# marionmari/pyGPs

Measured on AMD Instinct MI355X. Metric: GP fits/sec (nlZ+grad, RBF, N=8192 d=16), higher is better.
Workload: dtype f64; 1 GPU; GPR+RBF, N=8192 d=16 fp64 synthetic (SURVEY 8d recipe, seed 0), infExact nlZ + dnlZ (BASELINE configs[1]); x,y resident in HBM, hyp changes every step; outputs nlZ, dnlZ(4), alpha(N) to host per step; fits_per_rank=313, fit_streams_per_gpu=2, sched=1

## Files before the change

### pygps_amd/csrc/capi.hip

```cpp
#include <algorithm>
#include <atomic>
#include <cmath>
#include <cstdio>
#include <cstdlib>
#include <cstring>
#include <map>
#include <string>
#include <mutex>
#include <vector>

#include "ctx.h"

static thread_local char g_err[512] = "";
void pgp_set_last_hip_error(hipError_t e, const char* what, const char* file, int line) {
    snprintf(g_err, sizeof(g_err), "HIP error %d (%s) in %s at %s:%d", (int)e, hipGetErrorString(e), what, file, line);
    (void)hipGetLastError();
}

static void ctx_register(pgp_ctx* c);
static void ctx_unregister(pgp_ctx* c);

void prof_collect(pgp_ctx* c) {
    if (c->recs.empty()) return;
    (void)hipStreamSynchronize(c->st);
    for (auto& r : c->recs) {
        float ms = 0.f;
        (void)hipEventElapsedTime(&ms, r.e0, r.e1);
        c->pc_ms[r.cls] += ms; c->pc_flops[r.cls] += r.flops; c->pc_bytes[r.cls] += r.bytes; c->pc_launch[r.cls]++;
        if (r.shadow >= 0) { c->pc_ms[r.shadow] += ms; c->pc_flops[r.shadow] += r.flops; c->pc_launch[r.shadow]++; }
        if (getenv("PGP_PROF_DUMP"))
            fprintf(stderr, "prof %-34s %8.4f ms %10.3f GF %7.2f TF\n", kProfNames[r.cls], ms, r.flops * 1e-9,
                    ms > 0 ? r.flops / (ms * 1e-3) * 1e-12 : 0.0);
        c->ev_pool.push_back(r.e0); c->ev_pool.push_back(r.e1);
    }
    c->recs.clear();
}

DeviceGate& device_gate(int device) {
    static DeviceGate gates[64];
    return gates[(unsigned)device % 64u];
}
int& device_gate_depth(int device) {
    static thread_local int depth[64] = {0};
    return depth[(unsigned)device % 64u];
}

extern "C" {

const char* pgp_version(void) { return "pygps_amd 0.1 (gfx950)"; }
int pgp_device_count(void) {
    int n = 0;
    if (hipGetDeviceCount(&n) != hipSuccess) { (void)hipGetLastError(); return 0; }
    return n;
}

const char* pgp_strerror(int status) {
    if (status == 0) return "ok";
    if (status > 0) return "kernel matrix not positive definite";
    if (status <= PGP_ERR_HIP) return g_err[0] ? g_err : "HIP runtime failure";
    return "bad argument";
}

__global__ void pgp_noop_kernel() {}
static int alloc_result_buffer(pgp_ctx* c, long np);

static unsigned* yield_table(int device) {
    static std::mutex mu;
    static unsigned* tab[64] = {nullptr};
    std::lock_guard<std::mutex> lk(mu);
    if (device < 0 || device >= 64) return nullptr;
    if (!tab[device]) {
        if (hipMalloc((void**)&tab[device], 4096 * sizeof(unsigned)) != hipSuccess) { (void)hipGetLastError(); tab[device] = nullptr; return nullptr; }
        (void)hipMemset(tab[device], 0, 4096 * sizeof(unsigned));
    }
    return tab[device];
}

int pgp_init(int device, pgp_ctx** ctx_out) { GateShared device_gate_hold(device);
    if (!ctx_out) return -2;
    HIP_TRY(hipSetDevice(device));
    {
        static std::mutex mu;
        static bool primed[64] = {false};
        std::lock_guard<std::mutex> lk(mu);
        if (device >= 0 && device < 64 && !primed[device]) {
            hipLaunchKernelGGL(pgp_noop_kernel, dim3(1), dim3(64), 0, 0);
            HIP_TRY(hipDeviceSynchronize());
            primed[device] = true;
        }
    }
    pgp_ctx* c = new pgp_ctx();
    c->device = device;
    if (const char* e = getenv("PYGPS_AMD_PREDICT_INVERSE")) { const int v = atoi(e); if (v >= 0 && v <= 2) c->predict_inverse = v; }
    if (const char* e = getenv("PYGPS_AMD_KEEP_INVERSE")) c->keep_inverse = atoi(e) != 0;
    HIP_TRY(hipGetDeviceProperties(&c->prop, device));
    HIP_TRY(hipStreamCreateWithFlags(&c->st, hipStreamNonBlocking));
    {
        int lo = 0, hi = 0;
        (void)hipDeviceGetStreamPriorityRange(&lo, &hi);
        HIP_TRY(hipStreamCreateWithPriority(&c->st2, hipStreamNonBlocking, hi));
        if (lo == hi) c->ep_block = 0;
    }
    for (auto& e : c->ev) HIP_TRY(hipEventCreate(&e));
    memset(c->last_ms, 0, sizeof(c->last_ms));
    memset(c->pc_ms, 0, sizeof(c->pc_ms)); memset(c->pc_flops, 0, sizeof(c->pc_flops));
    memset(c->pc_bytes, 0, sizeof(c->pc_bytes)); memset(c->pc_launch, 0, sizeof(c->pc_launch));
    CHK(alloc_result_buffer(c, 0));
    c->yield_flags = yield_table(device);
    HIP_TRY(hipMalloc((void**)&c->Dk, (size_t)2048 * 1024 * sizeof(double)));
    HIP_TRY(hipMalloc((void**)&c->dpack, (size_t)8 * PACK_DOUBLES * sizeof(double)));
    HIP_TRY(hipMemset(c->Dk, 0, (size_t)2048 * 1024 * sizeof(double)));
    ctx_register(c);
    *ctx_out = c;
    return PGP_OK;
}

constexpr long RES_HEAD = 272, RES_INFO = 264;
static int alloc_result_buffer(pgp_ctx* c, long np) {
    const size_t bytes = (size_t)(RES_HEAD + np) * sizeof(double);
    if (c->res_dev) (void)hipFree(c->res_dev);
    if (c->res_host) (void)hipHostFree(c->res_host);
    c->res_dev = c->res_host = c->res_host_dev = nullptr; c->scal = c->alpha_dev = nullptr; c->info_dev = nullptr; c->res_cap = 0;
    HIP_TRY(hipMalloc((void**)&c->res_dev, bytes));
    HIP_TRY(hipMemset(c->res_dev, 0, bytes));
    HIP_TRY(hipHostMalloc((void**)&c->res_host, bytes, hipHostMallocMapped | hipHostMallocCoherent));
    c->res_host_dev = nullptr;
    if (hipHostGetDevicePointer((void**)&c->res_host_dev, c->res_host, 0) != hipSuccess) { (void)hipGetLastError(); c->res_host_dev = nullptr; }
    c->scal = c->res_dev; c->info_dev = (int*)(c->res_dev + RES_INFO); c->alpha_dev = c->res_dev + RES_HEAD;
    c->res_cap = bytes;
    return PGP_OK;
}

void pgp_destroy(pgp_ctx* c) { if (!c) return; GateShared device_gate_hold(c);
    if (!c) return;
    ctx_unregister(c);
    (void)hipSetDevice(c->device);
    (void)hipStreamSynchronize(c->st);
    if (c->st2) (void)hipStreamSynchronize(c->st2);
    for (auto& kv : c->pool) (void)hipFree(kv.second);
    for (auto& kv : c->spool) (void)hipFree(kv.second);
    for (auto& kv : c->orders) (void)hipFree(kv.second.first);
    void* bufs[] = {c->x_dev, c->y_dev, c->XsT, c->scale_dev, c->W, c->T, c->Binv, c->inv16, c->m_dev,
                    c->rvec, c->zvec, c->partial, c->Dk, c->dpack, c->Xs, c->res_dev, c->prep, c->pre2, c->pre1t, c->pre1s};
    for (void* b : bufs) if (b) (void)hipFree(b);
    if (c->res_host) (void)hipHostFree(c->res_host);
    if (c->in_host) (void)hipHostFree(c->in_host);
    if (c->pred_host) (void)hipHostFree(c->pred_host);
    if (c->gemm_trace) (void)hipFree(c->gemm_trace);
    for (auto& e : c->ev) (void)hipEventDestroy(e);
    for (auto& e : c->ev_pool) (void)hipEventDestroy(e);
    for (auto& r : c->recs) { (void)hipEventDestroy(r.e0); (void)hipEventDestroy(r.e1); }
    for (auto& e : c->la_ev) (void)hipEventDestroy(e);
    for (auto& e : c->tm_ev) (void)hipEventDestroy(e);
    for (auto& e : c->fill_ev) (void)hipEventDestroy(e);
    for (auto& e : c->ep_ev) (void)hipEventDestroy(e);
    (void)hipStreamDestroy(c->st);
    if (c->st2) (void)hipStreamDestroy(c->st2);
    delete c;
}

int pgp_device_info(pgp_ctx* c, int* n_cu, int* sclk_mhz, double* hbm_gib, char* name, int name_len) {
    if (!c) return -1;
    if (n_cu) *n_cu = c->prop.multiProcessorCount;
    if (sclk_mhz) *sclk_mhz = c->prop.clockRate / 1000;
    if (hbm_gib) *hbm_gib = (double)c->prop.totalGlobalMem / (1024.0 * 1024.0 * 1024.0);
    if (name && name_len > 0) { strncpy(name, c->prop.name, name_len - 1); name[name_len - 1] = 0; }
    return PGP_OK;
}

int pgp_set_option(pgp_ctx* c, const char* name, int value) {
    if (!c || !name) return -1;
    if (!strcmp(name, "nb_outer")) { if (value < 0) return -3; c->nb_outer = value; return PGP_OK; }
    if (!strcmp(name, "small_tile_below")) { c->small_tile_below = value; return PGP_OK; }
    if (!strcmp(name, "trtri_small_tile_below")) { c->trtri_small_tile_below = value; return PGP_OK; }
    if (!strcmp(name, "xcd_order")) { c->xcd_order = value; return PGP_OK; }
    if (!strcmp(name, "gemm_dbg")) { if (value & ~(64 | 256 | 512)) return -2; c->gemm_dbg = value; return PGP_OK; }
    if (!strcmp(name, "tile_ring")) { if (value < 0 || value > 1) return -2; c->tile_ring = value; return PGP_OK; }
    if (!strcmp(name, "lookahead")) { c->lookahead = value; return PGP_OK; }
    if (!strcmp(name, "leaf_first")) { c->leaf_first = value; return PGP_OK; }
    if (!strcmp(name, "leaf_pivot")) { if (value < 0 || value > 2) return -2; c->leaf_pivot = value; return PGP_OK; }
    if (!strcmp(name, "sched")) { if (value < -1 || value > 2) return -2; c->sched = value < 0 ? PGP_SCHED_DEFAULT : value; c->sched_explicit = value >= 0; return PGP_OK; }
    if (!strcmp(name, "concurrent_streams")) { c->concurrent_streams = value != 0; return PGP_OK; }
    if (!strcmp(name, "tud_tile")) { if (value != 64 && value != 128) return -2; c->tud_tile = value; return PGP_OK; }
    if (!strcmp(name, "tur_tile")) { if (value != 0 && value != 64 && value != 128 && value != 1264) return -2; c->tur_tile = value; return PGP_OK; }
    if (!strcmp(name, "s_pan")) { if (value < -1 || value > 2) return -2; c->s_pan = value; return PGP_OK; }
    if (!strcmp(name, "s_pan_direct")) { c->s_pan_direct = value != 0; return PGP_OK; }
    if (!strcmp(name, "s_pan_out")) { c->s_pan_out = value != 0; return PGP_OK; }
    if (!strcmp(name, "skip_zeros")) { c->skip_zeros = value != 0; return PGP_OK; }
    if (!strcmp(name, "tud_mark")) { c->tud_mark = value != 0; return PGP_OK; }
    if (!strcmp(name, "sched2_wide")) { c->sched2_wide = value != 0; return PGP_OK; }
    if (!strcmp(name, "gram_assembly")) { if (value < 0 || value > 2) return -2; c->gram_assembly = value; return PGP_OK; }
    if (!strcmp(name, "yield")) { c->yield = value; return PGP_OK; }
    if (!strcmp(name, "ep_fused")) { c->ep_fused = value; return PGP_OK; }
    if (!strcmp(name, "ep_tol_exp")) { if (value < 1 || value > 16) return -3; c->ep_tol_exp = value; return PGP_OK; }
    if (!strcmp(name, "ep_max_sweep")) { if (value < 2 || value > 1000) return -3; c->ep_max_sweep = value; return PGP_OK; }
    if (!strcmp(name, "laplace_tol_exp")) { if (value < 1 || value > 16) return -3; c->laplace_tol_exp = value; return PGP_OK; }
    if (!strcmp(name, "ep_r_direct")) { c->ep_r_direct = value; return PGP_OK; }
    if (!strcmp(name, "ep_alpha_direct")) { c->ep_alpha_direct = value; return PGP_OK; }
    if (!strcmp(name, "ep_sym")) { c->ep_sym = value; return PGP_OK; }
    if (!strcmp(name, "ep_wait_kernel")) { c->ep_wait_kernel = value; return PGP_OK; }
    if (!strcmp(name, "ep_sigma_under")) { c->ep_sigma_under = value; return PGP_OK; }
    if (!strcmp(name, "ep_recompute")) { c->ep_recompute = value; return PGP_OK; }
    if (!strcmp(name, "ep_final_rebuild")) { c->ep_final_rebuild = value; return PGP_OK; }
    if (!strcmp(name, "ep_block")) { c->ep_block = value; return PGP_OK; }
    if (!strcmp(name, "xcd_max_k")) { c->xcd_max_k = value; return PGP_OK; }
    if (!strcmp(name, "xcd_min_tiles")) { c->xcd_min_tiles = value; return PGP_OK; }
    if (!strcmp(name, "xcd_super")) { c->xcd_super = value; return PGP_OK; }
    if (!strcmp(name, "solve_outer")) { if (value < 1) return -2; c->solve_outer = value; return PGP_OK; }
    if (!strcmp(name, "keep_inverse")) { c->keep_inverse = value != 0; return PGP_OK; }
    if (!strcmp(name, "predict_inverse")) { if (value < 0 || value > 2) return -2; c->predict_inverse = value; return PGP_OK; }
    if (!strcmp(name, "predict_batch")) { if (value < 128 || value % 128) return -2; c->predict_batch = value; return PGP_OK; }
    if (!strcmp(name, "s_tile")) { if (value != 0 && value != 64 && value != 128) return -2; c->s_tile = value; return PGP_OK; }
    if (!strcmp(name, "eet_overlap")) { if (value != 0 && value != 2 && value != 3) return -2; c->eet_overlap = value; return PGP_OK; }
    if (!strcmp(name, "eet_max_panels")) { c->eet_max_panels = value; return PGP_OK; }
    if (!strcmp(name, "eet_first")) { if (value < -1) return -2; c->eet_first = value; return PGP_OK; }
    if (!strcmp(name, "eet_tile")) { if (value != 64 && value != 128) return -2; c->eet_tile = value; return PGP_OK; }
    if (!strcmp(name, "fused_inverse")) { c->fused_inverse = value; return PGP_OK; }
    if (!strcmp(name, "trsm_lean")) { if (value < 0 || value > 2) return -2; c->trsm_lean = value; return PGP_OK; }
    if (!strcmp(name, "ep_merge12")) { c->ep_merge12 = value != 0; return PGP_OK; }
    if (!strcmp(name, "publish")) { c->publish = value != 0; return PGP_OK; }
    if (!strcmp(name, "fused_value_max_np")) { c->fused_value_max_np = value; return PGP_OK; }
    if (!strcmp(name, "asm_grid")) { c->asm_grid = value; return PGP_OK; }
    if (!strcmp(name, "gram_fast")) { if (value < 0 || value > 2) return -2; c->gram_fast = value; return PGP_OK; }
    if (!strcmp(name, "gram_grid")) { if (value < 0) return -2; c->gram_grid = value; return PGP_OK; }
    if (!strcmp(name, "asm_nt")) { c->asm_nt = value; return PGP_OK; }
    if (!strcmp(name, "pair_launch")) { c->pair_launch = value != 0; return PGP_OK; }
    if (!strcmp(name, "gemm_trace")) {
        GateShared device_gate_hold(c);
        HIP_TRY(hipSetDevice(c->device));
        HIP_TRY(hipDeviceSynchronize());
        if (c->gemm_trace) { (void)hipFree(c->gemm_trace); c->gemm_trace = nullptr; }
        c->gemm_trace_cap = 0; c->gemm_trace_pos = 0;
        if (value > 0) {
            const long cap = (long)value * 1024;
            HIP_TRY(hipMalloc((void**)&c->gemm_trace, (size_t)cap * 64));
            HIP_TRY(hipMemset(c->gemm_trace, 0, (size_t)cap * 64));
            c->gemm_trace_cap = cap;
        }
        return PGP_OK;
    }
    if (!strcmp(name, "ard_grad_form")) { if (value < 0 || value > 2) return -3; c->ard_grad_form = value; return PGP_OK; }
    return -2;
}

int pgp_last_timings(pgp_ctx* c, double* ms_out) {
    if (!c || !ms_out) return -1;
    memcpy(ms_out, c->last_ms, sizeof(c->last_ms));
    return PGP_OK;
}
int pgp_set_profiling(pgp_ctx* c, int on) { if (!c) return -1; c->prof = on != 0; return PGP_OK; }
int pgp_profile_classes(void) { return PC_COUNT; }
const char* pgp_profile_class_name(int cls) { return (cls >= 0 && cls < PC_COUNT) ? kProfNames[cls] : "?"; }
int pgp_profile_read(pgp_ctx* c, int cls, int64_t* launches, double* ms, double* flops, double* bytes) {
    if (!c || cls < 0 || cls >= PC_COUNT) return -1;
    prof_collect(c);
    if (launches) *launches = c->pc_launch[cls];
    if (ms) *ms = c->pc_ms[cls];
    if (flops) *flops = c->pc_flops[cls];
    if (bytes) *bytes = c->pc_bytes[cls];
    return PGP_OK;
}
int pgp_profile_reset(pgp_ctx* c) {
    if (!c) return -1;
    prof_collect(c);
    memset(c->pc_ms, 0, sizeof(c->pc_ms)); memset(c->pc_flops, 0, sizeof(c->pc_flops));
    memset(c->pc_bytes, 0, sizeof(c->pc_bytes)); memset(c->pc_launch, 0, sizeof(c->pc_launch));
    return PGP_OK;
}

}


static int matern_d(int para) { return (para == 1 || para == 3 || para == 5 || para == 7) ? para : 3; }

static int leaf_nhyp(int kind, long d) {
    switch (kind) {
        case PGP_COV_RBF: case PGP_COV_MATERN: case PGP_COV_PIECEPOLY: case PGP_COV_GABOR: return 2;
        case PGP_COV_RBFARD: return (int)d + 1;
        case PGP_COV_RQARD: return (int)d + 2;
        case PGP_COV_RBFUNIT: case PGP_COV_NOISE: case PGP_COV_CONST: return 1;
        case PGP_COV_RQ: case PGP_COV_PERIODIC: return 3;
        case PGP_COV_PRE: return 0;
        default: return -1;
    }
}

static int make_leaf(int kind, const double* hyp, int nhyp, int para, int flags, long d, CovParams& cp, double& iso) {
    const int want = leaf_nhyp(kind, d);
    if (want < 0) return -2;
    if (nhyp != want) return -11;
    cp = CovParams{};
    cp.kind = kind; cp.der = -1; cp.md = matern_d(para); cp.D = (int)d; cp.train = 1;
    cp.ref_der = (flags & PGP_FLAG_MATERN_REFERENCE_DER) ? 1 : 0;
    cp.sf2 = 1.0; cp.alpha = 1.0; cp.ppv = 0; cp.ppj = 1.0; cp.ga = 0.0; cp.gb = 0.0;
    iso = 1.0;
    switch (kind) {
        case PGP_COV_RBF: iso = 1.0 / exp(hyp[0]); cp.sf2 = exp(2.0 * hyp[1]); break;
        case PGP_COV_RBFARD: cp.sf2 = exp(2.0 * hyp[d]); break;
        case PGP_COV_MATERN: iso = sqrt((double)cp.md) / exp(hyp[0]); cp.sf2 = exp(2.0 * hyp[1]); break;
        case PGP_COV_RBFUNIT: iso = 1.0 / exp(hyp[0]); break;
        case PGP_COV_RQ: iso = 1.0 / exp(hyp[0]); cp.sf2 = exp(2.0 * hyp[1]); cp.alpha = exp(hyp[2]); break;
        case PGP_COV_PIECEPOLY:
            if (para < 0 || para > 3) return -12;
            iso = 1.0 / exp(hyp[0]); cp.sf2 = exp(2.0 * hyp[1]);
            cp.ppv = para; cp.ppj = floor(0.5 * (double)d) + para + 1.0;
            break;
        case PGP_COV_RQARD: cp.sf2 = exp(2.0 * hyp[d]); cp.alpha = exp(hyp[d + 1]); cp.gb = 1.0; break;
        case PGP_COV_GABOR: {
            const double ell = exp(hyp[0]), p = exp(2.0 * hyp[1]);
            iso = 1.0 / ell; cp.ga = 2.0 * M_PI * ell / p;
            break;
        }
        case PGP_COV_PERIODIC:
            if (d != 1) return -12;
            cp.gb = 1.0 / exp(hyp[0]); cp.ga = M_PI / exp(hyp[1]); cp.sf2 = exp(2.0 * hyp[2]);
            break;
        case PGP_COV_NOISE: cp.sf2 = exp(2.0 * hyp[0]); break;
        case PGP_COV_CONST: cp.sf2 = exp(hyp[0]); break;
    }
    return PGP_OK;
}

static int bind_pre(pgp_ctx* c, CovSpec& cs) {
    if (cs.pg.pre_leaf < 0) return PGP_OK;
    if (!c || !c->pre2 || c->pre_n != c->n || c->n <= 0) return -14;
    cs.pre_train = c->pre2; cs.pre_ld = c->pre_ld; cs.pre_rows = c->pre_ld;
    return PGP_OK;
}

int make_spec(pgp_ctx* c, int kind, const double* hyp, int nhyp, int para, int flags, int der, long d, CovSpec& cs) {
    cs = CovSpec{};
    if (c) { cs.asm_grid = c->asm_grid; cs.asm_nt = c->asm_nt; cs.gram_fast = c->gram_fast; cs.gram_grid = c->gram_grid; }
    if (!hyp && nhyp > 0) return -10;
    if (kind == PGP_COV_SM) {
        const long Q = para;
        if (Q < 1) return -12;
        if (d > SM_MAXD || Q * (1 + 2 * d) > SM_MAXHYP) return -13;
        if ((long)nhyp != Q * (1 + 2 * d)) return -11;
        if (der >= nhyp) return -4;
        CovSM& P = cs.smp;
        P = CovSM{};
        P.Q = (int)Q; P.D = (int)d; P.dt = -1; P.dj = -1; P.dq = 0;
        const long double pi = 3.14159265358979323846264338327950288L;
        long double sw = 0.0L;
        for (long q = 0; q < Q; ++q) { P.h[q] = (double)expl((long double)hyp[q]); sw += expl((long double)hyp[q]); }
        for (long i = 0; i < d * Q; ++i) {
            P.h[Q + i] = (double)(2.0L * pi * expl((long double)hyp[Q + i]));
            P.h[Q + d * Q + i] = (double)(2.0L * pi * pi * expl(2.0L * (long double)hyp[Q + d * Q + i]));
        }
        cs.sm = true; cs.scale.assign(d, 1.0); cs.ncov = nhyp; cs.nder = nhyp;
        cs.cp = CovParams{};
        cs.cp.kind = kind; cs.cp.der = der; cs.cp.D = (int)d; cs.cp.train = 1; cs.cp.sf2 = (double)sw;
        return PGP_OK;
    }
    if (kind >= PGP_COV_GABOR && kind < PGP_COV_NKIND) {
        CovProgram& P = cs.pg;
        P = CovProgram{};
        double iso;
        CHK(make_leaf(kind, hyp, nhyp, para, flags, d, P.leaf[0], iso));
        if (der >= nhyp) return -4;
        P.nleaf = 1; P.nterm = 1; P.nscale = 0; P.is2[0] = iso * iso; P.hyp0[0] = 0; P.nh[0] = nhyp; P.ard_leaf = -1; P.ard_leaf2 = -1;
        P.pre_leaf = kind == PGP_COV_PRE ? 0 : -1;
        P.coef[0] = 1.0; P.tl[0] = 1u; P.ts[0] = 0u;
        P.der = der; P.der_leaf = der >= 0 ? 0 : -1; P.der_j = der; P.der_scale = -1;
        cs.prog = true; cs.scale.assign(d, 1.0); cs.ncov = nhyp; cs.nder = nhyp;
        return bind_pre(c, cs);
    }
    if (kind != PGP_COV_COMPOSITE) {
        double iso;
        CHK(make_leaf(kind, hyp, nhyp, para, flags, d, cs.cp, iso));
        cs.scale.assign(d, iso);
        if (kind == PGP_COV_RBFARD || kind == PGP_COV_RQARD) {
            for (long k = 0; k < d; ++k) cs.scale[k] = 1.0 / exp(hyp[k]);
            double bound = 0.0;
            if (c && (long)c->xdev2.size() == d)
                for (long k = 0; k < d; ++k) bound += cs.scale[k] * cs.scale[k] * c->xdev2[k];
            cs.ard_grad_diff = !(bound <= ARD_GRAM_GRAD_BOUND) || (c && c->ard_grad_form == 2);
            if (c && c->ard_grad_form == 1) cs.ard_grad_diff = false;
        }
        cs.ncov = nhyp;
        cs.nder = (kind == PGP_COV_MATERN || kind == PGP_COV_PIECEPOLY) ? 3 : nhyp;
        if (der >= cs.nder) return -4;
        cs.cp.der = der;
        cs.ell4 = (kind == PGP_COV_RQARD && cs.cp.ref_der && der >= 0 && der < d) ? exp(4.0 * hyp[der]) : 1.0;
        return PGP_OK;
    }
    const std::vector<int>& tok = c->composite;
    if (tok.empty()) return -2;
    struct Term { unsigned leaves, scales; };
    std::vector<std::vector<Term>> stack;
    CovProgram& P = cs.pg;
    P = CovProgram{};
    P.der = der; P.der_leaf = P.der_j = P.der_scale = -1;
    P.ard_leaf = -1; P.ard_leaf2 = -1; P.pre_leaf = -1;
    int used = 0;
    for (size_t i = 0; i < tok.size();) {
        const int op = tok[i];
        if (op == PGP_PROG_LEAF) {
            if (i + 5 > tok.size()) return -2;
            const int lk = tok[i + 1], lpara = tok[i + 2], lflags = tok[i + 3], h0 = tok[i + 4];
            i += 5;
            const bool ard = lk == PGP_COV_RBFARD || lk == PGP_COV_RQARD;
            if (ard && (P.ard_leaf2 >= 0 || d > CP_MAXARD)) return -13;
            const int nh = leaf_nhyp(lk, d);
            if (nh < 0) return -2;
            if (h0 < 0 || h0 + nh > nhyp) return -11;
            if (P.nleaf >= CP_MAXLEAF) return -13;
            if (lk == PGP_COV_PRE) {
                if (P.pre_leaf >= 0) return -13;
                P.pre_leaf = P.nleaf;
            }
            double iso;
            CHK(make_leaf(lk, hyp + h0, nh, lpara, lflags, d, P.leaf[P.nleaf], iso));
            P.is2[P.nleaf] = iso * iso; P.hyp0[P.nleaf] = h0; P.nh[P.nleaf] = nh;
            if (ard) {
                double* aw = P.ard_leaf < 0 ? P.ardw : P.ardw2;
                (P.ard_leaf < 0 ? P.ard_leaf : P.ard_leaf2) = P.nleaf;
                for (long k = 0; k < d; ++k) aw[k] = exp(-2.0 * hyp[h0 + k]);
                if (lk == PGP_COV_RQARD && P.leaf[P.nleaf].ref_der && der >= h0 && der < h0 + d) cs.ell4 = exp(4.0 * hyp[der]);
            }
            if (der >= h0 && der < h0 + nh) { P.der_leaf = P.nleaf; P.der_j = der - h0; }
            stack.push_back({Term{1u << P.nleaf, 0u}});
            ++P.nleaf; used += nh;
        } else if (op == PGP_PROG_SUM || op == PGP_PROG_PRODUCT) {
            ++i;
            if (stack.size() < 2) return -2;
            std::vector<Term> b = stack.back(); stack.pop_back();
            std::vector<Term> a = stack.back(); stack.pop_back();
            std::vector<Term> r;
            if (op == PGP_PROG_SUM) { r = a; r.insert(r.end(), b.begin(), b.end()); }
            else for (const Term& x : a) for (const Term& y : b) r.push_back(Term{x.leaves | y.leaves, x.scales | y.scales});
            if (r.size() > (size_t)CP_MAXTERM) return -13;
            stack.push_back(r);
        } else if (op == PGP_PROG_SCALE) {
            if (i + 1 >= tok.size()) return -2;
            const int h = tok[i + 1];
            i += 2;
            if (stack.empty()) return -2;
            if (h < 0 || h >= nhyp) return -11;
            if (P.nscale >= CP_MAXSCALE) return -13;
            for (Term& t : stack.back()) t.scales |= 1u << P.nscale;
            P.shyp[P.nscale] = h;
            if (der == h) P.der_scale = P.nscale;
            ++P.nscale; ++used;
        } else {
            return -2;
        }
    }
    if (stack.size() != 1 || used != nhyp) return -11;
    P.nterm = (int)stack[0].size();
    for (int t = 0; t < P.nterm; ++t) {
        P.tl[t] = stack[0][t].leaves; P.ts[t] = stack[0][t].scales;
        double cf = 1.0;
        for (int k = 0; k < P.nscale; ++k)
            if ((P.ts[t] >> k) & 1u) cf *= exp(hyp[P.shyp[k]]);
        P.coef[t] = cf;
    }
    if (der >= nhyp) return -4;
    cs.prog = true;
    cs.scale.assign(d, 1.0);
    cs.ncov = nhyp; cs.nder = nhyp;
    cs.cp = CovParams{};
    if (P.ard_leaf >= 0 && c && (long)c->xdev2.size() == d) {
        double b1 = 0.0, b2 = 0.0;
        for (long k = 0; k < d && k < CP_MAXARD; ++k) { b1 += P.ardw[k] * c->xdev2[k]; if (P.ard_leaf2 >= 0) b2 += P.ardw2[k] * c->xdev2[k]; }
        cs.ard_grad_diff = !(std::max(b1, b2) <= ARD_GRAM_GRAD_BOUND);
    }
    if (c && P.ard_leaf >= 0 && c->ard_grad_form) cs.ard_grad_diff = c->ard_grad_form == 2;
    return bind_pre(c, cs);
}

int cov_point_value(pgp_ctx* c, const CovSpec& cs, int train, double* out) {
    if (cs.has_pre()) { *out = 0.0; return PGP_OK; }
    if (!cs.prog && cs.cp.der < 0) {
        (void)train;
        *out = cs.cp.sf2;
        return PGP_OK;
    }
    double* dv = c->scal + 6;
    CHK(cov_self_launch(cs, train, dv, c->st));
    HIP_TRY(hipMemcpyAsync(out, dv, sizeof(double), hipMemcpyDeviceToHost, c->st));
    HIP_TRY(hipStreamSynchronize(c->st));
    return PGP_OK;
}

int upload_scaled(pgp_ctx* c, const double* x_dev, long n, long d, const std::vector<double>& sc, double* XsT,
                         long ldp, int dpad, double* scale_dev) {
    HIP_TRY(hipMemcpyAsync(scale_dev, sc.data(), d * sizeof(double), hipMemcpyHostToDevice, c->st));
    return scale_transpose_launch(x_dev, n, (int)d, scale_dev, XsT, ldp, dpad, c->st);
}

static int tile_order(pgp_ctx* c, int mt, int nt, int tri, int off_tiles, const int** out, int* n) {
    std::vector<int> key = {mt, nt, tri ? 1 : 0, off_tiles, c->xcd_super};
    auto it = c->orders.find(key);
    if (it != c->orders.end()) { *out = it->second.first; *n = it->second.second; return PGP_OK; }
    const int S = c->xcd_super > 0 ? c->xcd_super : 8;
    std::vector<std::vector<int>> sts;
    for (int SI = 0; SI * S < mt; ++SI)
        for (int SJ = 0; SJ * S < nt; ++SJ) {
            std::vector<int> st;
            for (int ti = SI * S; ti < std::min(mt, SI * S + S); ++ti)
                for (int tj = SJ * S; tj < std::min(nt, SJ * S + S); ++tj)
                    if (!tri || ti + off_tiles >= tj) { st.push_back(ti); st.push_back(tj); }
            if (!st.empty()) sts.push_back(std::move(st));
        }
    std::stable_sort(sts.begin(), sts.end(), [](const std::vector<int>& a, const std::vector<int>& b) { return a.size() > b.size(); });
    std::vector<std::vector<int>> seq(8);
    for (auto& st : sts) {
        int best = 0;
        for (int x = 1; x < 8; ++x) if (seq[x].size() < seq[best].size()) best = x;
        seq[best].insert(seq[best].end(), st.begin(), st.end());
    }
    for (;;) {
        int lo = 0, hi = 0;
        for (int x = 1; x < 8; ++x) { if (seq[x].size() < seq[lo].size()) lo = x; if (seq[x].size() > seq[hi].size()) hi = x; }
        if (seq[hi].size() < seq[lo].size() + 4) break;
        const int tj = seq[hi].back(); seq[hi].pop_back();
        const int ti = seq[hi].back(); seq[hi].pop_back();
        seq[lo].push_back(ti); seq[lo].push_back(tj);
    }
    size_t maxlen = 0;
    for (auto& q : seq) maxlen = std::max(maxlen, q.size() / 2);
    const int nb = (int)maxlen * 8;
    std::vector<int> ord(2 * (size_t)nb, -1);
    for (int b = 0; b < nb; ++b) {
        const int x = b % 8, idx = b / 8;
        if ((size_t)idx < seq[x].size() / 2) { ord[2 * b] = seq[x][2 * idx]; ord[2 * b + 1] = seq[x][2 * idx + 1]; }
    }
    int* dev = nullptr;
    HIP_TRY(hipMalloc((void**)&dev, ord.size() * sizeof(int)));
    HIP_TRY(hipMemcpyAsync(dev, ord.data(), ord.size() * sizeof(int), hipMemcpyHostToDevice, c->st));
    HIP_TRY(hipStreamSynchronize(c->st));
    c->orders[key] = {dev, nb};
    *out = dev; *n = nb;
    return PGP_OK;
}

static int tri_tile_list(pgp_ctx* c, int mt, int nt, int off_tiles, const int** out, int* n) {
    std::vector<int> key = {mt, nt, 2, off_tiles};
    auto it = c->orders.find(key);
    if (it != c->orders.end()) { *out = it->second.first; *n = it->second.second; return PGP_OK; }
    std::vector<int> ord;
    for (int tj = 0; tj < nt; ++tj)
        for (int ti = 0; ti < mt; ++ti)
            if (ti + off_tiles >= tj) { ord.push_back(ti); ord.push_back(tj); }
    int* dev = nullptr;
    HIP_TRY(hipMalloc((void**)&dev, ord.size() * sizeof(int)));
    HIP_TRY(hipMemcpyAsync(dev, ord.data(), ord.size() * sizeof(int), hipMemcpyHostToDevice, c->st));
    HIP_TRY(hipStreamSynchronize(c->st));
    c->orders[key] = {dev, (int)ord.size() / 2};
    *out = dev; *n = (int)ord.size() / 2;
    return PGP_OK;
}

int batch_tile_list(pgp_ctx* c, int mt0, int nt, int nb, int dmt, const int** out, int* n) {
    std::vector<int> key = {mt0, nt, nb, dmt, 7777};
    auto it = c->orders.find(key);
    if (it != c->orders.end()) { *out = it->second.first; *n = it->second.second; return PGP_OK; }
    std::vector<int> ord;
    for (int z = 0; z < nb; ++z)
        for (int tj = 0; tj < nt; ++tj)
            for (int ti = tj; ti < mt0 - z * dmt; ++ti) { ord.push_back(ti | (z << 16)); ord.push_back(tj); }
    if (ord.empty()) { ord.push_back(-1); ord.push_back(-1); }
    int* dev = nullptr;
    HIP_TRY(hipMalloc((void**)&dev, ord.size() * sizeof(int)));
    HIP_TRY(hipMemcpyAsync(dev, ord.data(), ord.size() * sizeof(int), hipMemcpyHostToDevice, c->st));
    HIP_TRY(hipStreamSynchronize(c->st));
    c->orders[key] = {dev, (int)ord.size() / 2};
    *out = dev; *n = (int)ord.size() / 2;
    return PGP_OK;
}

bool gram_assembly_applies(pgp_ctx* c, const CovSpec& cs) {
    if (!c->gram_assembly || !cov_gram_applies(cs, c->dpad) || (long)c->xdev2.size() != c->d || (long)cs.scale.size() < c->d) return false;
    if (c->gram_assembly == 2) return true;
    double bound = 0.0;
    for (long k = 0; k < c->d; ++k) bound += cs.scale[k] * cs.scale[k] * c->xdev2[k];
    return bound <= 64.0;
}

static int gemm_prepare(pgp_ctx* c, GemmArgs& g) {
    if (g.batch < 1) g.batch = 1;
    g.dbg |= c->gemm_dbg;
    bool xcd = false;
    if (c->xcd_order && !g.order && g.tile != 64 && g.tile != 1264 && g.batch == 1 && g.K <= c->xcd_max_k) {
        const long mt = g.M / 128, nt = g.N / 128;
        const long tiles = g.tri == 2 ? mt * (mt + 1) / 2 : (g.tri == 1 ? mt * nt - nt * (nt - 1) / 2 : mt * nt);
        xcd = tiles >= c->xcd_min_tiles;
    }
    if (g.tri == 1 && !g.order && !xcd) {
        const int T = g.tile == 64 ? 64 : 128;
        CHK(tri_tile_list(c, g.M / T, g.N / T, g.tri_off / T, &g.order, &g.norder));
    }
    if (xcd) CHK(tile_order(c, g.M / 128, g.N / 128, g.tri, g.tri ? g.tri_off / 128 : 0, &g.order, &g.norder));
    if (c->yield && c->yield_flags) {
        g.yield_flags = c->yield_flags;
        if (g.yield_role != 2) g.yield_role = gemm_f64_uses_dma(g) ? 1 : 0;
    } else g.yield_role = 0;
    g.ring = c->tile_ring && gemm_f64_uses_dma(g) ? 1 : 0;
    if (c->gemm_trace && gemm_f64_uses_dma128(g) && g.batch == 1) {
        const long mt = g.M / 128, nt = g.N / 128;
        const long nb = g.order ? g.norder : (g.tri == 2 ? mt * (mt + 1) / 2 : mt * nt);
        if (c->gemm_trace_pos + nb <= c->gemm_trace_cap) { g.trace = c->gemm_trace + 8 * c->gemm_trace_pos; c->gemm_trace_pos += nb; }
    }
    return PGP_OK;
}

int gemm_prof(pgp_ctx* c, int cls, GemmArgs g, hipStream_t st) {
    if (!st) st = c->st;
    CHK(gemm_prepare(c, g));
    ProfScope ps(c, cls, g.flops, 0.0, st, gemm_f64_uses_dma128(g) ? PC_KERNEL_DMA128 : -1);
    return gemm_f64_launch(g, st);
}

int gemm_prof_pair(pgp_ctx* c, int cls_a, GemmArgs a, int cls_b, GemmArgs b, hipStream_t st) {
    if (!st) st = c->st;
    CHK(gemm_prepare(c, a));
    CHK(gemm_prepare(c, b));
    if (c->pair_launch && gemm_f64_pair_ok(a, b)) {
        ProfScope ps(c, cls_a, a.flops + b.flops, 0.0, st, PC_KERNEL_DMA128);
        return gemm_f64_launch_pair(a, b, st);
    }
    { ProfScope ps(c, cls_a, a.flops, 0.0, st, gemm_f64_uses_dma128(a) ? PC_KERNEL_DMA128 : -1);
      CHK(gemm_f64_launch(a, st)); }
    ProfScope ps(c, cls_b, b.flops, 0.0, st, gemm_f64_uses_dma128(b) ? PC_KERNEL_DMA128 : -1);
    return gemm_f64_launch(b, st);
}

struct TriNode { int lo, mid, hi, depth; };
static void tri_nodes(int lo, int hi, int depth, std::vector<TriNode>& out) {
    if (hi - lo <= 1) return;
    int half = 1;
    while (half * 2 < hi - lo) half *= 2;
    const int mid = lo + half;
    out.push_back({lo, mid, hi, depth});
    tri_nodes(lo, mid, depth + 1, out);
    tri_nodes(mid, hi, depth + 1, out);
}

int trtri_lower(pgp_ctx* c, const double* L, long ldl, double* W, long ldw, double* T, long np) {
    const int nblk = (int)(np / 128);
    {
        ProfScope ps(c, PC_LEAFINV, (double)nblk * 128.0 * 128.0 * 128.0 / 3.0, 0.0);
        CHK(leaf_inv_launch(L, ldl, W, ldw, 128L * (1 + ldw), nblk, c->st));
    }
    std::vector<TriNode> nodes;
    tri_nodes(0, nblk, 0, nodes);
    int maxd = -1;
    for (auto& nd : nodes) maxd = std::max(maxd, nd.depth);
    for (int dep = maxd; dep >= 0; --dep) {
        std::vector<TriNode> lv;
        for (auto& nd : nodes) if (nd.depth == dep) lv.push_back(nd);
        if (lv.empty()) continue;
        std::sort(lv.begin(), lv.end(), [](const TriNode& a, const TriNode& b) { return a.lo < b.lo; });
        bool uniform = true;
        const int h1 = lv[0].mid - lv[0].lo, h2 = lv[0].hi - lv[0].mid;
        const int step = lv.size() > 1 ? lv[1].lo - lv[0].lo : 0;
        for (size_t i = 0; i < lv.size(); ++i)
            if (lv[i].mid - lv[i].lo != h1 || lv[i].hi - lv[i].mid != h2 || lv[i].lo != lv[0].lo + (int)i * step)
                uniform = false;
        const size_t ngroups = uniform ? 1 : lv.size();
        for (size_t gi = 0; gi < ngroups; ++gi) {
            const TriNode& nd = lv[gi];
            const int a1 = (nd.mid - nd.lo) * 128, a2 = (nd.hi - nd.mid) * 128;
            const long o1 = (long)nd.lo * 128, o2 = (long)nd.mid * 128;
            const int batch = uniform ? (int)lv.size() : 1;
            const long bstep = (long)step * 128;
            const long t128 = (long)(a2 / 128) * (a1 / 128) * batch;
            GemmArgs g{};
            g.A = L + o2 + o1 * ldl; g.lda = ldl; g.a_kc = 0;
            g.B = W + o1 + o1 * ldw; g.ldb = ldw; g.b_kc = 1;
            g.C = T; g.ldc = a2;
            g.M = a2; g.N = a1; g.K = a1; g.alpha = 1.0; g.beta = 0.0;
            g.kmode = KM_GE_J; g.koff = 0;
            g.batch = batch; g.sA = bstep * (1 + ldl); g.sB = bstep * (1 + ldw); g.sC = (long)a1 * a2;
            g.tile = t128 < c->trtri_small_tile_below ? 64 : 128;
            g.flops = (double)batch * (double)a2 * a1 * a1;
            CHK(gemm_prof(c, PC_GEMM_TRTRI, g));
            GemmArgs h{};
            h.A = W + o2 + o2 * ldw; h.lda = ldw; h.a_kc = 0;
            h.B = T; h.ldb = a2; h.b_kc = 1;
            h.C = W + o2 + o1 * ldw; h.ldc = ldw;
            h.M = a2; h.N = a1; h.K = a2; h.alpha = -1.0; h.beta = 0.0;
            h.kmode = KM_LT_I; h.koff = 0;
            h.batch = batch; h.sA = bstep * (1 + ldw); h.sB = (long)a1 * a2; h.sC = bstep * (1 + ldw);
            h.tile = g.tile;
            h.flops = (double)batch * (double)a2 * a2 * a1;
            CHK(gemm_prof(c, PC_GEMM_TRTRI, h));
        }
    }
    return PGP_OK;
}

int lauum_lower(pgp_ctx* c, const double* W, long ldw, double* Binv, long ldb, long np) {
    GemmArgs g{};
    g.A = W; g.lda = ldw; g.a_kc = 1;
    g.B = W; g.ldb = ldw; g.b_kc = 1;
    g.C = Binv; g.ldc = ldb;
    g.M = (int)np; g.N = (int)np; g.K = (int)np; g.alpha = 1.0; g.beta = 0.0;
    g.tri = 2; g.mask_diag = 1; g.kmode = KM_GE_I; g.koff = 0;
    const long t128 = (np / 128) * (np / 128 + 1) / 2;
    g.tile = t128 < c->small_tile_below ? 64 : 128;
    g.flops = (double)np * np * np / 3.0;
    return gemm_prof(c, PC_GEMM_LAUUM, g);
}

int eet_lower(pgp_ctx* c, const double* E, long lde, double* Binv, long ldb, long np) {
    GemmArgs g{};
    g.A = E; g.lda = lde; g.a_kc = 0;
    g.B = E; g.ldb = lde; g.b_kc = 0;
    g.C = Binv; g.ldc = ldb;
    g.M = (int)np; g.N = (int)np; g.K = (int)np; g.alpha = 1.0; g.beta = 0.0;
    g.tri = 2; g.mask_diag = 1; g.kmode = KM_GE_I; g.koff = 0;
    const long t128 = (np / 128) * (np / 128 + 1) / 2;
    g.tile = t128 < c->small_tile_below ? 64 : 128;
    g.flops = (double)np * np * np / 3.0;
    return gemm_prof(c, PC_GEMM_LAUUM, g);
}

int ensure_workspace(pgp_ctx* c, long np) {
    if (c->ws_np == np) return PGP_OK;
    (void)hipStreamSynchronize(c->st);
    void* olds[] = {c->W, c->T, c->Binv, c->inv16, c->m_dev, c->rvec, c->zvec, c->prep};
    for (void* b : olds) if (b) (void)hipFree(b);
    c->W = c->T = c->Binv = c->inv16 = c->m_dev = c->rvec = c->zvec = c->prep = nullptr;
    if (c->in_host) { (void)hipHostFree(c->in_host); c->in_host = nullptr; c->in_cap = 0; }
    c->ws_np = 0;
    c->dense_ready = false;
    const size_t nn = (size_t)np * np * sizeof(double);
    HIP_TRY(hipMalloc((void**)&c->W, nn));
    HIP_TRY(hipMemsetAsync(c->W, 0, nn, c->st));
    HIP_TRY(hipMalloc((void**)&c->Binv, nn));
    HIP_TRY(hipMemsetAsync(c->Binv, 0, nn, c->st));
    HIP_TRY(hipMalloc((void**)&c->T, std::max<size_t>(nn / 4, 128 * 128 * sizeof(double))));
    HIP_TRY(hipMalloc((void**)&c->inv16, (size_t)(np / 128) * PACK_DOUBLES * sizeof(double)));
    CHK(alloc_result_buffer(c, np));
    HIP_TRY(hipMalloc((void**)&c->m_dev, np * sizeof(double)));
    HIP_TRY(hipMalloc((void**)&c->rvec, np * sizeof(double)));
    HIP_TRY(hipMalloc((void**)&c->zvec, np * sizeof(double)));
    HIP_TRY(hipMalloc((void**)&c->prep, (size_t)hadamard_prep_count(np) * sizeof(double)));
    HIP_TRY(hipMemsetAsync(c->rvec, 0, np * sizeof(double), c->st));
    c->in_cap = (size_t)(np + 1024) * sizeof(double);
    HIP_TRY(hipHostMalloc((void**)&c->in_host, c->in_cap, hipHostMallocDefault));
    c->ws_np = np;
    return PGP_OK;
}

int alloc_factor_buffer(pgp_ctx* c, long np, long ldf, double** F) {
    const size_t bytes = (size_t)ldf * np * sizeof(double);
    bool fresh = false;
    CHK(pool_alloc(c, bytes, (void**)F, &fresh));
    if (fresh) HIP_TRY(hipMemsetAsync(*F, 0, bytes, c->st));
    return PGP_OK;
}

static std::mutex g_ctx_mu;
static std::vector<pgp_ctx*> g_ctxs;
int pgp_ctx_count_on_device(int device) {
    std::lock_guard<std::mutex> lk(g_ctx_mu);
    int n = 0;
    for (pgp_ctx* c : g_ctxs) n += c->device == device;
    return n;
}
void pgp_drop_idle_pools(int device) { GateShared device_gate_hold(device);
    std::lock_guard<std::mutex> lk(g_ctx_mu);
    for (pgp_ctx* c : g_ctxs) {
        if (c->device != device) continue;
        std::lock_guard<std::mutex> lp(c->pool_mu);
        for (auto& kv : c->pool) (void)hipFree(kv.second);
        for (auto& kv : c->spool) (void)hipFree(kv.second);
        c->pool.clear(); c->pool_bytes = 0;
        c->spool.clear(); c->spool_bytes = 0;
    }
}
static void ctx_register(pgp_ctx* c) { std::lock_guard<std::mutex> lk(g_ctx_mu); g_ctxs.push_back(c); }
static void ctx_unregister(pgp_ctx* c) {
    std::lock_guard<std::mutex> lk(g_ctx_mu);
    g_ctxs.erase(std::remove(g_ctxs.begin(), g_ctxs.end(), c), g_ctxs.end());
}

extern "C" {

int pgp_set_composite(pgp_ctx* c, const int32_t* prog, int nprog) { if (!c) return -1; GateShared device_gate_hold(c);
    if (!c) return -1;
    if (nprog < 0 || (nprog > 0 && !prog)) return -2;
    c->composite.assign(prog, prog + nprog);
    return PGP_OK;
}

int pgp_set_pre(pgp_ctx* c, const double* M2, int64_t n, const double* M1, int64_t ns) { if (!c) return -1; GateShared device_gate_hold(c);
    if (!c) return -1;
    if (n <= 0) return -3;
    if (M1 && ns <= 0) return -5;
    HIP_TRY(hipSetDevice(c->device));
    (void)hipStreamSynchronize(c->st);
    const long np = round_up(n, 128);
    if (M2) {
        if (c->pre2) (void)hipFree(c->pre2);
        c->pre2 = nullptr; c->pre_n = 0;
        if (c->pre1t) (void)hipFree(c->pre1t);
        if (c->pre1s) (void)hipFree(c->pre1s);
        c->pre1t = c->pre1s = nullptr; c->pre_ns = 0;
        HIP_TRY(hipMalloc((void**)&c->pre2, (size_t)np * np * sizeof(double)));
        HIP_TRY(hipMemsetAsync(c->pre2, 0, (size_t)np * np * sizeof(double), c->st));
        HIP_TRY(hipMemcpy2DAsync(c->pre2, np * sizeof(double), M2, n * sizeof(double), n * sizeof(double), n, hipMemcpyHostToDevice, c->st));
        HIP_TRY(hipStreamSynchronize(c->st));
        c->pre_n = n; c->pre_ld = np;
    }
    if (M1) {
        if (!c->pre2 || c->pre_n != n) return -2;
        if (c->pre1t) (void)hipFree(c->pre1t);
        if (c->pre1s) (void)hipFree(c->pre1s);
        c->pre1t = c->pre1s = nullptr; c->pre_ns = 0;
        const long nsp = round_up(ns, 128);
        HIP_TRY(hipMalloc((void**)&c->pre1t, (size_t)nsp * np * sizeof(double)));
        HIP_TRY(hipMalloc((void**)&c->pre1s, (size_t)nsp * sizeof(double)));
        HIP_TRY(hipMemsetAsync(c->pre1t, 0, (size_t)nsp * np * sizeof(double), c->st));
        HIP_TRY(hipMemsetAsync(c->pre1s, 0, (size_t)nsp * sizeof(double), c->st));
        std::vector<double> blk;
        for (int64_t a = 0; a < ns; a += 1024) {
            const int64_t nb = std::min<int64_t>(1024, ns - a);
            blk.resize((size_t)nb * n);
            for (int64_t i = 0; i < n; ++i)
                for (int64_t j = 0; j < nb; ++j) blk[(size_t)j * n + i] = M1[(size_t)i * ns + a + j];
            HIP_TRY(hipMemcpy2DAsync(c->pre1t + a * np, np * sizeof(double), blk.data(), n * sizeof(double), n * sizeof(double), nb,
                                     hipMemcpyHostToDevice, c->st));
            HIP_TRY(hipStreamSynchronize(c->st));
        }
        HIP_TRY(hipMemcpyAsync(c->pre1s, M1 + (size_t)n * ns, ns * sizeof(double), hipMemcpyHostToDevice, c->st));
        HIP_TRY(hipStreamSynchronize(c->st));
        c->pre_ns = ns; c->pre_nsp = nsp;
    }
    return PGP_OK;
}

int pgp_set_data(pgp_ctx* c, const double* x, int64_t n, int64_t d, const double* y) { if (!c) return -1; GateShared device_gate_hold(c);
    if (!c) return -1;
    if (!x) return -2;
    if (n <= 0) return -3;
    if (d <= 0) return -4;
    HIP_TRY(hipSetDevice(c->device));
    (void)hipStreamSynchronize(c->st);
    void* olds[] = {c->x_dev, c->y_dev, c->XsT, c->scale_dev};
    for (void* b : olds) if (b) (void)hipFree(b);
    c->x_dev = c->y_dev = c->XsT = c->scale_dev = nullptr;
    c->n = 0;
    const long np = round_up(n, 128);
    const int dpad = (int)round_up(d, SKC);
    HIP_TRY(hipMalloc((void**)&c->x_dev, n * d * sizeof(double)));
    HIP_TRY(hipMalloc((void**)&c->y_dev, np * sizeof(double)));
    HIP_TRY(hipMalloc((void**)&c->XsT, (size_t)dpad * np * sizeof(double)));
    HIP_TRY(hipMalloc((void**)&c->scale_dev, dpad * sizeof(double)));
    HIP_TRY(hipMemcpyAsync(c->x_dev, x, n * d * sizeof(double), hipMemcpyHostToDevice, c->st));
    HIP_TRY(hipMemsetAsync(c->y_dev, 0, np * sizeof(double), c->st));
    if (y) HIP_TRY(hipMemcpyAsync(c->y_dev, y, n * sizeof(double), hipMemcpyHostToDevice, c->st));
    HIP_TRY(hipStreamSynchronize(c->st));
    {
        std::vector<double> mean((size_t)d, 0.0);
        for (int64_t p = 0; p < n; ++p) for (int64_t k = 0; k < d; ++k) mean[k] += x[p * d + k];
        for (int64_t k = 0; k < d; ++k) mean[k] /= (double)n;
        c->xdev2.assign((size_t)d, 0.0);
        for (int64_t p = 0; p < n; ++p)
            for (int64_t k = 0; k < d; ++k) { const double v = x[p * d + k] - mean[k]; if (v * v > c->xdev2[k]) c->xdev2[k] = v * v; }
    }
    c->n = n; c->d = d; c->np = np; c->ldf = np + 128;
    c->dpad = dpad;
    return PGP_OK;
}

int pgp_exact_fit(pgp_ctx* c, int kind, const double* covhyp, int ncov, int para, int flags, double log_sn,
                  const double* mvec, const double* dm, int nmean, int want, double* alpha_out, double* nlZ_out,
                  double* dnlZ_out, pgp_factor** factor_out) {
    if (!c) return -1;
    GateShared device_gate_hold(c);
    if (!c) return -1;
    if (c->n <= 0) return -1;
    if (!covhyp) return -3;
    if (want < 1 || want > 3) return -11;
    if (ncov < 0 || 8 + ncov + 1 > RES_INFO) return -4;
    HIP_TRY(hipSetDevice(c->device));
    c->dense_ready = false;
    const long n = c->n, d = c->d, np = c->np;
    bool fused = c->fused_inverse != 0;
    if (want < 3 && fused && c->fused_value_max_np >= 0 && np > c->fused_value_max_np) fused = false;
    const long ldf = c->ldf;
    CovSpec cp;
    { const int rc = make_spec(c, kind, covhyp, ncov, para, flags, -1, d, cp); if (rc != PGP_OK) return rc == -11 ? -10 : rc; }
    const std::vector<double>& sc = cp.scale;
    CHK(ensure_workspace(c, np));
    double kss = 0.0;
    if (factor_out) CHK(cov_point_value(c, cp, 2, &kss));
    const long need = std::max(hadamard_partial_count(np, ncov), 32L * np);
    if ((want >= 3 || fused) && c->partial_cap < need) {
        if (c->partial) (void)hipFree(c->partial);
        c->partial = nullptr; c->partial_cap = 0;
        HIP_TRY(hipMalloc((void**)&c->partial, need * sizeof(double)));
        c->partial_cap = need;
    }
    const double sn2 = exp(2.0 * log_sn);
    double* F = nullptr;
    CHK(alloc_factor_buffer(c, np, ldf, &F));
    FactorGuard fguard(c, F, (size_t)ldf * np * sizeof(double), true);
    PoolScratch pscr(c);
    double* E = nullptr;
    const long lde = np;
    if (fused) {
        const int erc = pscr.alloc(&E, (size_t)np * np * sizeof(double));
        if (erc != PGP_OK) {
            if (want >= 3) return erc;
            (void)hipGetLastError(); fused = false; E = nullptr;
        }
    }
    hipStream_t st = c->st;
    HIP_TRY(hipMemsetAsync(c->info_dev, 0, sizeof(int), st));
    if (mvec) {
        memcpy(c->in_host, mvec, n * sizeof(double));
        HIP_TRY(hipMemcpyAsync(c->m_dev, c->in_host, n * sizeof(double), hipMemcpyHostToDevice, st));
    } else HIP_TRY(hipMemsetAsync(c->m_dev, 0, n * sizeof(double), st));

    HIP_TRY(hipEventRecord(c->ev[0], st));
    CHK(upload_scaled(c, c->x_dev, n, d, sc, c->XsT, np, c->dpad, c->scale_dev));
    const bool gram = gram_assembly_applies(c, cp);
    if (gram) CHK(hadamard_prepare_launch(c->XsT, np, n, np, c->dpad, cp, c->prep, st, true));
    {
        ProfScope ps(c, PC_ASSEMBLE, 0.0, 8.0 * (double)np * (np + 1) / 2.0 + 8.0 * (double)n * d);
        if (gram) CHK(cov_factor_gram_launch(c->XsT, np, n, np, c->dpad, cp, 1.0 / sn2, F, ldf, c->prep, st));
        else CHK(cov_factor_launch(c->XsT, np, n, np, c->dpad, cp, 1.0 / sn2, F, ldf, st));
    }
    CHK(aug_rhs_launch(c->y_dev, c->m_dev, n, F, ldf, np, c->rvec, st));
    HIP_TRY(hipEventRecord(c->ev[1], st));
    SweepJob job{F, ldf, np, np + 128, fused, E, lde};
    if (fused && want >= 3) { job.eet_out = c->Binv; job.eet_ld = np; }
    const int prc = potrf_blocked(c, job);
    if (prc != PGP_OK) (void)hipDeviceSynchronize();
    CHK(prc);
    HIP_TRY(hipEventRecord(c->ev[2], st));
    CHK(logdet_ztz_launch(F, ldf, n, F + np, ldf, c->scal, st));
    CHK(gather_strided_launch(F + np, ldf, np, c->zvec, st));
    if (fused) {
        HIP_TRY(hipEventRecord(c->ev[3], st));
        { ProfScope ps(c, PC_SMALL, 0.0, 4.0 * (double)np * np);
          CHK(upper_matvec_launch(E, lde, np, c->zvec, 1.0 / sn2, c->partial, c->alpha_dev, st)); }
    } else if (want >= 3) {
        CHK(trtri_lower(c, F, ldf, c->W, np, c->T, np));
        HIP_TRY(hipEventRecord(c->ev[3], st));
        { ProfScope ps(c, PC_SMALL, 0.0, 4.0 * (double)np * np);
          CHK(col_dot_launch(c->W, np, np, c->zvec, 1, 1.0 / sn2, c->alpha_dev, st)); }
    } else {
        { ProfScope ps(c, PC_LEAFINV, 0.0, 0.0);
          CHK(leaf_inv_launch(F, ldf, c->W, np, 128L * (1 + np), (int)(np / 128), st)); }
        HIP_TRY(hipEventRecord(c->ev[3], st));
        { ProfScope ps(c, PC_SMALL, 0.0, 4.0 * (double)np * np);
          CHK(trsv_bwd_launch(F, ldf, c->W, np, c->zvec, c->alpha_dev, (int)(np / 128), st)); }
    }
    HIP_TRY(hipEventRecord(c->ev[4], st));
    if (want >= 3) {
        if (fused && job.join) HIP_TRY(hipStreamWaitEvent(st, job.join, 0));
        else if (fused) CHK(eet_lower(c, E, lde, c->Binv, np, np));
        else CHK(lauum_lower(c, c->W, np, c->Binv, np, np));
        HIP_TRY(hipEventRecord(c->ev[5], st));
        { ProfScope ps(c, PC_HADAMARD, 0.0, 8.0 * (double)np * (np + 1) / 2.0 + 8.0 * (double)n * d);
          CHK(hadamard_reduce_launch(c->XsT, np, n, np, c->dpad, cp, ncov, sn2, c->Binv, np, c->alpha_dev, c->partial,
                                     c->scal + 8, st, nullptr, gram ? c->prep : nullptr)); }
    } else {
        HIP_TRY(hipEventRecord(c->ev[5], st));
    }
    HIP_TRY(hipEventRecord(c->ev[6], st));
    if (c->publish && c->res_host_dev) CHK(publish_launch(c->res_dev, c->res_host_dev, RES_HEAD + n, st));
    else HIP_TRY(hipMemcpyAsync(c->res_host, c->res_dev, (size_t)(RES_HEAD + n) * sizeof(double), hipMemcpyDeviceToHost, st));
    HIP_TRY(hipStreamSynchronize(st));
    const double* sc_host = c->res_host;
    double* alpha_h = c->res_host + RES_HEAD;
    int info = 0;
    memcpy(&info, c->res_host + RES_INFO, sizeof(int));
    if (want < 3 && !fused) for (long j = 0; j < n; ++j) alpha_h[j] /= sn2;
    {
        float ms;
        const int map[6][2] = {{0, 1}, {1, 2}, {3, 4}, {2, 3}, {4, 5}, {5, 6}};
        for (int i = 0; i < 6; ++i) { (void)hipEventElapsedTime(&ms, c->ev[map[i][0]], c->ev[map[i][1]]); c->last_ms[i] = ms; }
        (void)hipEventElapsedTime(&ms, c->ev[0], c->ev[6]); c->last_ms[PGP_STAGE_TOTAL] = ms;
    }
    if (c->prof) prof_collect(c);
    if (info != 0) return info > (int)n ? (int)n : info;
    if (alpha_out) memcpy(alpha_out, alpha_h, n * sizeof(double));
    if (want >= 2 && nlZ_out) {
        const double logdet = sc_host[0], ztz = sc_host[1];
        *nlZ_out = 0.5 * ztz / sn2 + logdet + 0.5 * (double)n * log(2.0 * M_PI * sn2);
    }
    if (want >= 3 && dnlZ_out) {
        for (int i = 0; i < nmean; ++i) {
            double s = 0.0;
            for (long j = 0; j < n; ++j) s += dm[(long)i * n + j] * alpha_h[j];
            dnlZ_out[i] = -s;
        }
        for (int h = 0; h < ncov; ++h) dnlZ_out[nmean + h] = 0.5 * sc_host[8 + h];
        dnlZ_out[nmean + ncov] = sc_host[8 + ncov];
    }
    if (factor_out) {
        FactorHandleGuard hg(c, new pgp_factor());
        pgp_factor* f = hg.f;
        f->n = n; f->np = np; f->ldf = ldf; f->F = fguard.release(); f->dpad = c->dpad; f->d = (int)d; f->cs = cp; f->kss = kss;
        f->sn2 = sn2; f->sw = 1.0 / sqrt(sn2); f->Wd = nullptr;
        CHK(spool_take(c, np * sizeof(double), (void**)&f->alpha));
        HIP_TRY(hipMemsetAsync(f->alpha, 0, np * sizeof(double), st));
        HIP_TRY(hipMemcpyAsync(f->alpha, alpha_h, n * sizeof(double), hipMemcpyHostToDevice, st));
        CHK(spool_take(c, (size_t)c->dpad * np * sizeof(double), (void**)&f->XsT));
        HIP_TRY(hipMemcpyAsync(f->XsT, c->XsT, (size_t)c->dpad * np * sizeof(double), hipMemcpyDeviceToDevice, st));
        HIP_TRY(hipStreamSynchronize(st));
        if (fused && E && c->keep_inverse && np <= 16384) {
            const size_t eb = pscr.release(E);
            if (eb) { f->Eraw = E; f->Eraw_bytes = eb; }
        }
        *factor_out = hg.release();
    }
    fguard.scrub = false;
    return PGP_OK;
}

int64_t pgp_factor_n(pgp_factor* f) { return f ? f->n : 0; }

int pgp_factor_to_host(pgp_ctx* c, pgp_factor* f, double* L_out) {
    if (!c) return -1;
    GateShared device_gate_hold(c);
    if (!c || !f) return -1;
    if (!L_out) return -3;
    HIP_TRY(hipSetDevice(c->device));
    HIP_TRY(hipMemcpy2DAsync(L_out, f->n * sizeof(double), f->F, f->ldf * sizeof(double), f->n * sizeof(double), f->n,
                             hipMemcpyDeviceToHost, c->st));
    HIP_TRY(hipStreamSynchronize(c->st));
    return PGP_OK;
}

void pgp_factor_free(pgp_ctx* c, pgp_factor* f) { GateShared device_gate_hold(c);
    if (!f) return;
    if (c) {
        (void)hipSetDevice(c->device);
        pool_free(c, (size_t)f->ldf * f->np * sizeof(double), f->F);
        if (f->Linv) pool_free(c, (size_t)f->ldf * f->np * sizeof(double), f->Linv);
    }
    spool_give(c, (size_t)f->np * sizeof(double), f->alpha);
    spool_give(c, (size_t)f->dpad * f->np * sizeof(double), f->XsT);
    spool_give(c, (size_t)128 * f->np * sizeof(double), f->Wd);
    spool_give(c, (size_t)f->np * sizeof(double), f->sWv);
    if (f->Eraw) spool_give(c, f->Eraw_bytes, f->Eraw);
    delete f;
}

int pgp_cov(pgp_ctx* c, int kind, int mode, int der, const double* x, int64_t n, const double* z, int64_t m,
            int64_t d, const double* hyp, int nhyp, int para, int flags, double* out) {
    if (!c) return -1;
    GateShared device_gate_hold(c);
    if (!c) return -1;
    if (mode < 0 || mode > 2) return -3;
    if (!hyp) return -10;
    if (!out) return -14;
    if (mode != PGP_MODE_SELF_TEST && !x) return -5;
    if (mode != PGP_MODE_TRAIN && !z) return -7;
    if (d <= 0) return -9;
    HIP_TRY(hipSetDevice(c->device));
    hipStream_t st = c->st;
    CovSpec cp;
    CHK(make_spec(c, kind, hyp, nhyp, para, flags, der, d, cp));
    if (cp.has_pre()) return -13;
    if (mode == PGP_MODE_SELF_TEST) {
        double val = 0.0;
        CHK(cov_point_value(c, cp, 2, &val));
        for (int64_t i = 0; i < m; ++i) out[i] = val;
        return PGP_OK;
    }
    const std::vector<double>& sc = cp.scale;
    const int dpad = (int)round_up(d, SKC);
    const long ldr = round_up(n, 128), ldc = (mode == PGP_MODE_CROSS) ? round_up(m, 128) : 0;
    const long mm = (mode == PGP_MODE_CROSS) ? m : n;
    PoolScratch tmp(c);
    double *xd = nullptr, *zd = nullptr, *XrT = nullptr, *XcT = nullptr, *scd = nullptr, *od = nullptr;
    CHK(tmp.alloc(&xd, n * d * sizeof(double)));
    CHK(tmp.alloc(&XrT, (size_t)dpad * ldr * sizeof(double)));
    CHK(tmp.alloc(&scd, dpad * sizeof(double)));
    CHK(tmp.alloc(&od, (size_t)n * mm * sizeof(double)));
    HIP_TRY(hipMemcpyAsync(xd, x, n * d * sizeof(double), hipMemcpyHostToDevice, st));
    CHK(upload_scaled(c, xd, n, d, sc, XrT, ldr, dpad, scd));
    if (mode == PGP_MODE_CROSS) {
        CHK(tmp.alloc(&zd, m * d * sizeof(double)));
        CHK(tmp.alloc(&XcT, (size_t)dpad * ldc * sizeof(double)));
        HIP_TRY(hipMemcpyAsync(zd, z, m * d * sizeof(double), hipMemcpyHostToDevice, st));
        CHK(scale_transpose_launch(zd, m, (int)d, scd, XcT, ldc, dpad, st));
    }
    {
        ProfScope ps(c, PC_ASSEMBLE, 0.0, 8.0 * (double)n * mm + 8.0 * (double)(n + (mode == PGP_MODE_CROSS ? m : 0)) * d);
        bool gram = false;
        if (mode == PGP_MODE_TRAIN && der < 0 && n >= 4096 && c->gram_assembly && cov_gram_applies(cp, dpad) && (long)sc.size() >= d) {
            gram = c->gram_assembly == 2;
            if (!gram) {
                double bound = 0.0;
                for (int64_t k = 0; k < d; ++k) {
                    double mean = 0.0, dev = 0.0;
                    for (int64_t p = 0; p < n; ++p) mean += x[p * d + k];
                    mean /= (double)n;
                    for (int64_t p = 0; p < n; ++p) dev = std::max(dev, fabs(x[p * d + k] - mean));
                    bound += sc[k] * sc[k] * dev * dev;
                }
                gram = bound <= 64.0;
            }
        }
        if (gram) {
            double* prep = nullptr;
            CHK(tmp.alloc(&prep, (size_t)hadamard_prep_count(ldr) * sizeof(double)));
            CHK(hadamard_prepare_launch(XrT, ldr, n, ldr, dpad, cp, prep, st, true));
            CHK(cov_sym_gram_launch(XrT, ldr, n, dpad, cp, od, n, prep, st));
        } else if (mode == PGP_MODE_TRAIN) CHK(cov_sym_launch(XrT, ldr, n, dpad, cp, od, st));
        else CHK(cov_rect_launch(XrT, ldr, n, XcT, ldc, m, dpad, cp, od, m, st));
    }
    HIP_TRY(hipMemcpyAsync(out, od, (size_t)n * mm * sizeof(double), hipMemcpyDeviceToHost, st));
    HIP_TRY(hipStreamSynchronize(st));
    if (c->prof) prof_collect(c);
    return PGP_OK;
}

int pgp_potrf(pgp_ctx* c, const double* A, int64_t n, double* L_out) {
    if (!c) return -1;
    GateShared device_gate_hold(c);
    if (!c) return -1;
    if (!A) return -2;
    if (n <= 0) return -3;
    if (!L_out) return -4;
    HIP_TRY(hipSetDevice(c->device));
    const long np = round_up(n, 128);
    hipStream_t st = c->st;
    PoolScratch tmp(c);
    double *F = nullptr, *pack = nullptr;
    CHK(tmp.alloc(&F, (size_t)np * np * sizeof(double)));
    CHK(tmp.alloc(&pack, (size_t)(np / 128) * PACK_DOUBLES * sizeof(double)));
    HIP_TRY(hipMemsetAsync(F, 0, (size_t)np * np * sizeof(double), st));
    HIP_TRY(hipMemcpy2DAsync(F, np * sizeof(double), A, n * sizeof(double), n * sizeof(double), n, hipMemcpyHostToDevice, st));
    std::vector<double> ones(np - n + 1, 1.0);
    if (np > n)
        HIP_TRY(hipMemcpy2DAsync(F + n + n * np, (np + 1) * sizeof(double), ones.data(), sizeof(double), sizeof(double),
                                 np - n, hipMemcpyHostToDevice, st));
    HIP_TRY(hipMemsetAsync(c->info_dev, 0, sizeof(int), st));
    double* pack_save = c->inv16;
    c->inv16 = pack;
    SweepJob job{F, np, np, np};
    const int rc = potrf_blocked(c, job);
    c->inv16 = pack_save;
    CHK(rc);
    int info = 0;
    HIP_TRY(hipMemcpyAsync(&info, c->info_dev, sizeof(int), hipMemcpyDeviceToHost, st));
    HIP_TRY(hipStreamSynchronize(st));
    if (c->prof) prof_collect(c);
    if (info != 0) return info > (int)n ? (int)n : info;
    std::vector<double> host((size_t)n * n);
    HIP_TRY(hipMemcpy2D(host.data(), n * sizeof(double), F, np * sizeof(double), n * sizeof(double), n,
                        hipMemcpyDeviceToHost));
    for (int64_t i = 0; i < n; ++i)
        for (int64_t j = 0; j < n; ++j) L_out[i * n + j] = (j <= i) ? host[(size_t)j * n + i] : 0.0;
    return PGP_OK;
}

}
```

### pygps_amd/csrc/common.h

```cpp
#pragma once
#include <hip/hip_runtime.h>
#include <cstdint>
#include <cstdio>

#define PGP_OK 0
#define PGP_ERR_HIP (-100)
#define PGP_ERR_ARG (-1)

#define HIP_TRY(expr)                                                                       \
    do {                                                                                    \
        hipError_t e__ = (expr);                                                            \
        if (e__ != hipSuccess) {                                                            \
            pgp_set_last_hip_error(e__, #expr, __FILE__, __LINE__);                         \
            return PGP_ERR_HIP;                                                             \
        }                                                                                   \
    } while (0)

void pgp_set_last_hip_error(hipError_t e, const char* what, const char* file, int line);

enum GemmKMode {
    KM_FULL = 0,
    KM_GE_I = 1,
    KM_GE_J = 2,
    KM_LT_I = 3,
    KM_LT_J = 4,
};

struct GemmArgs {
    const double* A; long lda; int a_kc;
    const double* B; long ldb; int b_kc;
    double* C; long ldc;
    int M, N, K;
    double alpha, beta;
    int tri;
    int tri_off;
    int mask_diag;
    int kmode; int koff;
    int batch; long sA, sB, sC;
    int tile;
    const int* order;
    int norder;
    int order_z;
    int dbg;
    int ring;
    double flops;
    const double* A2; long lda2; int a_split;
    double* C2; long ldc2; int c_split;
    const double* Cin; long ldcin; const double* Cin2; long ldcin2;
    int rev_cols;
    int rev_rows;
    int fold_rows;
    int zero_from;
    int zf_upper;
    int batch_dm;
    int batch_dk;
    int batch_dldc; long batch_sC2;
    unsigned* yield_flags; int yield_role;
    int skip_lo, skip_hi;
    unsigned* wait_flag; unsigned wait_target; unsigned* wait_err;
    long long* trace;
};

__device__ __forceinline__ unsigned pgp_cu_key() {
    const unsigned hw = __builtin_amdgcn_s_getreg((4 << 0) | (0 << 6) | (31 << 11));
    const unsigned xcc = __builtin_amdgcn_s_getreg((20 << 0) | (0 << 6) | (3 << 11)) & 15u;
    return (xcc << 8) | ((hw >> 8) & 0xffu);
}
__device__ __forceinline__ void pgp_yield_mark(unsigned* flags, int delta) {
    if (flags && threadIdx.x == 0) {
        if (delta > 0) __hip_atomic_fetch_add(flags + pgp_cu_key(), 1u, __ATOMIC_RELAXED, __HIP_MEMORY_SCOPE_AGENT);
        else __hip_atomic_fetch_sub(flags + pgp_cu_key(), 1u, __ATOMIC_RELAXED, __HIP_MEMORY_SCOPE_AGENT);
    }
}

int gemm_f64_launch(const GemmArgs& g, hipStream_t st);
bool gemm_f64_pair_ok(const GemmArgs& a, const GemmArgs& b);
int gemm_f64_launch_pair(const GemmArgs& a, const GemmArgs& b, hipStream_t st);
bool gemm_f64_uses_dma(const GemmArgs& g);
bool gemm_f64_uses_dma128(const GemmArgs& g);

void func_max_dynamic_lds(const void* fn, size_t bytes);
```

### pygps_amd/csrc/ctx.h

```cpp
#pragma once
#include <algorithm>
#include <chrono>
#include <condition_variable>
#include <cstdio>
#include <cstdlib>
#include <map>
#include <mutex>
#include <vector>

#include "../../include/pygps_amd.h"
#include "kernels.h"
#include "sqdist_tile.h"

enum ProfClass { PC_ASSEMBLE = 0, PC_GEMM_TRAIL, PC_GEMM_INNER, PC_LEAF, PC_TRSM, PC_LEAFINV, PC_GEMM_TRTRI,
                 PC_GEMM_LAUUM, PC_HADAMARD, PC_SMALL, PC_GEMM_SOLVE, PC_DIAG, PC_KERNEL_DMA128, PC_COUNT };
static const char* const kProfNames[PC_COUNT] = {
    "cov_tile_kernel(assemble)", "gemm_f64(potrf trailing syrk)", "gemm_f64(potrf inner update)",
    "leaf_potrf_kernel", "trsm_rows_kernel", "leaf_inv_kernel", "gemm_f64(trtri)", "gemm_f64(lauum W^T W)",
    "hadamard_reduce_kernel", "small/O(N) kernels", "gemm_f64(panel solve X E_D)", "diag_in/out staging",
    "kernel gemm_f64_kernel<128,128,false,false,true,*> + gemm_f64_pair_kernel (LDS-DMA 128-tile)"};

struct ProfRec { int cls; hipEvent_t e0, e1; double flops, bytes; int shadow; };

struct pgp_factor {
    long n, np, ldf;
    double* F;
    double* alpha;
    double* XsT;
    double* Wd;
    double* Linv = nullptr;
    double* Eraw = nullptr;
    size_t Eraw_bytes = 0;
    int dpad, d;
    CovSpec cs;
    double kss = 0.0;
    double sn2;
    double sw;
    double* sWv = nullptr;
};

constexpr int PGP_SCHED_DEFAULT = 2;

struct pgp_ctx {
    int device = 0;
    std::vector<int> composite;
    hipStream_t st = nullptr;
    hipStream_t st2 = nullptr;
    std::vector<hipEvent_t> fill_ev;
    std::vector<hipEvent_t> ep_ev;
    int eet_tile = 128;
    int eet_first = -1;
    int eet_overlap = 3;
    int eet_max_panels = 32;
    std::vector<hipEvent_t> la_ev;
    std::vector<hipEvent_t> tm_ev;
    int lookahead = 1;
    bool sched_explicit = false;
    bool concurrent_streams = false;
    int sched = PGP_SCHED_DEFAULT;
    int tur_tile = 0;
    int tud_tile = 64;
    int sched2_wide = 0;
    int s_pan = -1;
    int s_pan_direct = 1;
    int s_pan_out = 1;
    int skip_zeros = 1;
    int tud_mark = 1;
    int leaf_pivot = 2;
    int leaf_first = 0;
    int yield = 1;
    long long* gemm_trace = nullptr;
    long gemm_trace_cap = 0;
    long gemm_trace_pos = 0;
    unsigned* yield_flags = nullptr;
    int ep_fused = 2;
    int ep_r_direct = 1;
    int ep_alpha_direct = 1;
    int ep_recompute = 0;
    int ep_final_rebuild = 0;
    int ep_tol_exp = 4;
    int ep_max_sweep = 10;
    int laplace_tol_exp = 6;
    int ep_sigma_under = 1;
    int ep_wait_kernel = 1;
    int ep_sym = 1;
    int ep_block = 1;
    int fused_value_max_np = 12288;
    int fused_inverse = 1;
    hipDeviceProp_t prop;
    std::mutex pool_mu;
    std::multimap<size_t, void*> pool;
    size_t pool_bytes = 0;
    std::multimap<size_t, void*> spool;
    size_t spool_bytes = 0;
    long n = 0, d = 0, np = 0, ldf = 0;
    int dpad = 0;
    double *x_dev = nullptr, *y_dev = nullptr, *XsT = nullptr, *scale_dev = nullptr;
    double *pre2 = nullptr, *pre1t = nullptr, *pre1s = nullptr;
    long pre_n = 0, pre_ld = 0, pre_ns = 0, pre_nsp = 0;
    long ws_np = 0;
    double *W = nullptr, *T = nullptr, *Binv = nullptr, *inv16 = nullptr, *alpha_dev = nullptr, *m_dev = nullptr,
           *rvec = nullptr, *zvec = nullptr, *partial = nullptr, *scal = nullptr;
    long partial_cap = 0;
    double* prep = nullptr;
    int pair_launch = 1;
    int ard_grad_form = 0;
    std::vector<double> xdev2;
    int gram_assembly = 1;
    bool dense_ready = false;
    long dense_n = 0;
    int* info_dev = nullptr;
    double* res_dev = nullptr;
    double* res_host = nullptr;
    double* res_host_dev = nullptr;
    int ep_merge12 = 1;
    int trsm_lean = 0;
    int publish = 1;
    double* in_host = nullptr;
    double* pred_host = nullptr;
    size_t pred_cap = 0;
    size_t res_cap = 0, in_cap = 0;
    double *Dk = nullptr, *dpack = nullptr, *Xs = nullptr;
    int xcd_max_k = 512;
    int xcd_min_tiles = 256;
    int xcd_super = 8;
    int solve_outer = 8;
    int keep_inverse = 1;
    int predict_inverse = 1;
    int predict_batch = 65536;
    int s_tile = 0;
    int gram_fast = 2, gram_grid = 32768;
    int asm_grid = 4096, asm_nt = 0;
    size_t Xs_bytes = 0;
    hipEvent_t ev[PGP_NSTAGE + 2];
    double last_ms[PGP_NSTAGE];
    bool prof = false;
    std::vector<ProfRec> recs;
    std::vector<hipEvent_t> ev_pool;
    double pc_ms[PC_COUNT], pc_flops[PC_COUNT], pc_bytes[PC_COUNT];
    int64_t pc_launch[PC_COUNT];
    std::map<std::vector<int>, std::pair<int*, int>> orders;
    int gemm_dbg = 64 | 256 | 512;
    int tile_ring = 1;
    int xcd_order = 0;
    int nb_outer = 0;
    int trtri_small_tile_below = 2049;
    int small_tile_below = 200;
};

#define CHK(x)                      \
    do {                            \
        int rc__ = (x);             \
        if (rc__ != PGP_OK) return rc__; \
    } while (0)

int pgp_ctx_count_on_device(int device);
void pgp_drop_idle_pools(int device);

static inline bool pool_trace_on() { static const bool on = getenv("PGP_POOL_TRACE") != nullptr; return on; }
static inline hipError_t pool_hip_malloc(void** out, size_t bytes, const char* who) {
    if (!pool_trace_on()) return hipMalloc(out, bytes);
    const auto t0 = std::chrono::steady_clock::now();
    const hipError_t e = hipMalloc(out, bytes);
    fprintf(stderr, "[pool] hipMalloc %8.1f MiB  %8.3f ms  (%s)%s\n", bytes / 1048576.0,
            std::chrono::duration<double, std::milli>(std::chrono::steady_clock::now() - t0).count(), who, e == hipSuccess ? "" : " FAILED");
    return e;
}
static inline void pool_hip_free(void* p, size_t bytes, const char* who) {
    if (!pool_trace_on()) { (void)hipFree(p); return; }
    const auto t0 = std::chrono::steady_clock::now();
    (void)hipFree(p);
    fprintf(stderr, "[pool] hipFree   %8.1f MiB  %8.3f ms  (%s)\n", bytes / 1048576.0,
            std::chrono::duration<double, std::milli>(std::chrono::steady_clock::now() - t0).count(), who);
}

static inline size_t pool_idle_cap(pgp_ctx* c) {
    return (size_t)c->prop.totalGlobalMem / 3 / (size_t)std::max(1, pgp_ctx_count_on_device(c->device));
}

static inline int pool_alloc(pgp_ctx* c, size_t bytes, void** out, bool* fresh = nullptr) {
    if (fresh) *fresh = false;
    {
        std::lock_guard<std::mutex> lk(c->pool_mu);
        auto it = c->pool.find(bytes);
        if (it != c->pool.end()) {
            *out = it->second;
            c->pool.erase(it);
            c->pool_bytes -= bytes;
            return PGP_OK;
        }
    }
    if (fresh) *fresh = true;
    if (pool_hip_malloc(out, bytes, "factor pool") != hipSuccess) {
        (void)hipGetLastError();
        pgp_drop_idle_pools(c->device);
        HIP_TRY(pool_hip_malloc(out, bytes, "factor pool, retry"));
    }
    return PGP_OK;
}
static inline void pool_free(pgp_ctx* c, size_t bytes, void* p) {
    if (!p) return;
    const size_t cap = pool_idle_cap(c);
    std::lock_guard<std::mutex> lk(c->pool_mu);
    if (c->pool_bytes + bytes > cap) { pool_hip_free(p, bytes, "factor pool over its cap"); return; }
    c->pool.insert({bytes, p});
    c->pool_bytes += bytes;
}

static inline int spool_take(pgp_ctx* c, size_t bytes, void** out) {
    {
        std::lock_guard<std::mutex> lk(c->pool_mu);
        auto it = c->spool.find(bytes);
        if (it != c->spool.end()) {
            *out = it->second;
            c->spool.erase(it);
            c->spool_bytes -= bytes;
            return PGP_OK;
        }
    }
    hipError_t e = pool_hip_malloc(out, bytes ? bytes : 8, "handle buffer");
    if (e != hipSuccess) { pgp_set_last_hip_error(e, "hipMalloc(handle buffer)", __FILE__, __LINE__); return PGP_ERR_HIP; }
    return PGP_OK;
}
static inline void spool_give(pgp_ctx* c, size_t bytes, void* p) {
    if (!p) return;
    if (!c) { (void)hipFree(p); return; }
    const size_t cap = pool_idle_cap(c);
    std::lock_guard<std::mutex> lk(c->pool_mu);
    if (c->spool_bytes + bytes > cap) { pool_hip_free(p, bytes, "scratch pool over its cap (handle buffer)"); return; }
    c->spool.insert({bytes, p});
    c->spool_bytes += bytes;
}

struct ProfScope {
    pgp_ctx* c; int cls; double flops, bytes; hipEvent_t e0 = nullptr, e1 = nullptr; hipStream_t s; int shadow;
    ProfScope(pgp_ctx* c_, int cls_, double f, double b, hipStream_t s_ = nullptr, int shadow_ = -1)
        : c(c_), cls(cls_), flops(f), bytes(b), s(s_ ? s_ : c_->st), shadow(shadow_) {
        if (!c->prof) return;
        auto get = [&]() {
            hipEvent_t e;
            if (!c->ev_pool.empty()) { e = c->ev_pool.back(); c->ev_pool.pop_back(); }
            else (void)hipEventCreate(&e);
            return e;
        };
        e0 = get(); e1 = get();
        (void)hipEventRecord(e0, s);
    }
    ~ProfScope() {
        if (!c->prof) return;
        (void)hipEventRecord(e1, s);
        c->recs.push_back({cls, e0, e1, flops, bytes, shadow});
    }
};


struct DevScratch {
    std::vector<void*> ptrs;
    ~DevScratch() { for (void* p : ptrs) if (p) (void)hipFree(p); }
    template <typename T>
    int alloc(T** out, size_t bytes) {
        void* p = nullptr;
        hipError_t e = hipMalloc(&p, bytes ? bytes : 8);
        if (e != hipSuccess) { pgp_set_last_hip_error(e, "hipMalloc(scratch)", __FILE__, __LINE__); return PGP_ERR_HIP; }
        ptrs.push_back(p);
        *out = (T*)p;
        return PGP_OK;
    }
};

struct PoolScratch {
    pgp_ctx* c;
    std::vector<std::pair<size_t, void*>> held;
    explicit PoolScratch(pgp_ctx* c_) : c(c_) {}
    ~PoolScratch() {
        const size_t cap = pool_idle_cap(c);
        std::lock_guard<std::mutex> lk(c->pool_mu);
        for (auto& h : held) {
            if (c->spool_bytes + h.first > cap) { pool_hip_free(h.second, h.first, "scratch pool over its cap"); continue; }
            c->spool.insert({h.first, h.second});
            c->spool_bytes += h.first;
        }
    }
    template <typename T>
    int alloc(T** out, size_t bytes) {
        void* p = nullptr;
        if (!bytes) bytes = 8;
        {
            std::lock_guard<std::mutex> lk(c->pool_mu);
            auto it = c->spool.find(bytes);
            if (it != c->spool.end()) { p = it->second; c->spool.erase(it); c->spool_bytes -= bytes; }
        }
        if (!p && pool_hip_malloc(&p, bytes, "scratch pool") != hipSuccess) {
            (void)hipGetLastError();
            pgp_drop_idle_pools(c->device);
            hipError_t e = pool_hip_malloc(&p, bytes, "scratch pool, retry");
            if (e != hipSuccess) { pgp_set_last_hip_error(e, "hipMalloc(pool scratch)", __FILE__, __LINE__); return PGP_ERR_HIP; }
        }
        held.push_back({bytes, p});
        *out = (T*)p;
        return PGP_OK;
    }
    size_t release(void* p) {
        for (size_t i = 0; i < held.size(); ++i)
            if (held[i].second == p) { const size_t b = held[i].first; held.erase(held.begin() + (long)i); return b; }
        return 0;
    }
};

struct FactorGuard {
    pgp_ctx* c; double* F; size_t bytes; bool scrub;
    FactorGuard(pgp_ctx* c_, double* F_, size_t b, bool scrub_ = false) : c(c_), F(F_), bytes(b), scrub(scrub_) {}
    ~FactorGuard() {
        if (!F) return;
        if (scrub) { (void)hipMemsetAsync(F, 0, bytes, c->st); (void)hipStreamSynchronize(c->st); }
        pool_free(c, bytes, F);
    }
    double* release() { double* p = F; F = nullptr; return p; }
};

struct FactorHandleGuard {
    pgp_ctx* c; pgp_factor* f;
    FactorHandleGuard(pgp_ctx* c_, pgp_factor* f_) : c(c_), f(f_) {}
    ~FactorHandleGuard() { if (f) pgp_factor_free(c, f); }
    pgp_factor* release() { pgp_factor* p = f; f = nullptr; return p; }
};

void prof_collect(pgp_ctx* c);
static inline long round_up(long v, long m) { return (v + m - 1) / m * m; }
int make_spec(pgp_ctx* c, int kind, const double* hyp, int nhyp, int para, int flags, int der, long d, CovSpec& cs);
int cov_point_value(pgp_ctx* c, const CovSpec& cs, int train, double* out);
struct SweepJob {
    double* F; long ldf, np, mrows;
    bool inverse = false;
    double* E = nullptr; long lde = 0;
    double* R = nullptr; long ldr = 0, nrhs2 = 0;
    double* eet_out = nullptr; long eet_ld = 0;
    double* rhs_C = nullptr;  long rhs_ld = 0;
    hipEvent_t join = nullptr;
};
int potrf_blocked(pgp_ctx* c, SweepJob& job);
static inline int ensure_events(std::vector<hipEvent_t>& ev, size_t n) {
    for (hipEvent_t e; ev.size() < n; ev.push_back(e)) HIP_TRY(hipEventCreateWithFlags(&e, hipEventDisableTiming));
    return PGP_OK;
}
int gemm_prof(pgp_ctx* c, int cls, GemmArgs g, hipStream_t st = nullptr);
int gemm_prof_pair(pgp_ctx* c, int cls_a, GemmArgs a, int cls_b, GemmArgs b, hipStream_t st = nullptr);
int batch_tile_list(pgp_ctx* c, int mt0, int nt, int nb, int dmt, const int** out, int* n);
inline long predict_batch_points(int option, long ns, long np) {
    const long cap = std::max<long>(16384, ((long)1 << 34) / (8 * std::max<long>(np, 1)) / 128 * 128);
    const long want = std::min<long>(option, (ns + 127) / 128 * 128);
    return std::max<long>(128, std::min<long>(want, cap));
}
struct DeviceGate {
    std::mutex m;
    std::condition_variable cv;
    int readers = 0, writers_waiting = 0;
    bool writer = false;
    void lock_shared() { std::unique_lock<std::mutex> l(m); cv.wait(l, [&] { return !writer && writers_waiting == 0; }); ++readers; }
    void unlock_shared() { std::lock_guard<std::mutex> l(m); if (--readers == 0) cv.notify_all(); }
    void lock() { std::unique_lock<std::mutex> l(m); ++writers_waiting; cv.wait(l, [&] { return !writer && readers == 0; }); --writers_waiting; writer = true; }
    void unlock() { std::lock_guard<std::mutex> l(m); writer = false; cv.notify_all(); }
};
DeviceGate& device_gate(int device);
int& device_gate_depth(int device);
struct GateShared {
    DeviceGate& g; int& depth; int state = 1;
    explicit GateShared(pgp_ctx* c) : GateShared(c ? c->device : 0) {}
    explicit GateShared(int device) : g(device_gate(device)), depth(device_gate_depth(device)) {
        if (depth++ > 0) state = 0; else g.lock_shared();
    }
    void exclusive() { if (state == 1) { g.unlock_shared(); g.lock(); state = 2; } }
    void shared_again() { if (state == 2) { g.unlock(); g.lock_shared(); state = 1; } }
    ~GateShared() { --depth; if (state == 1) g.unlock_shared(); else if (state == 2) g.unlock(); }
    GateShared(const GateShared&) = delete;
    GateShared& operator=(const GateShared&) = delete;
};
constexpr double ARD_GRAM_GRAD_BOUND = 1.0e6;
bool gram_assembly_applies(pgp_ctx* c, const CovSpec& cs);
int diag_block_factor(pgp_ctx* c, const double* src, long lds, int w, double* Fd, long ldf, double* Ed, long lde,
                      int info_base, hipStream_t st, hipEvent_t staged = nullptr);
int trtri_lower(pgp_ctx* c, const double* L, long ldl, double* W, long ldw, double* T, long np);
int lauum_lower(pgp_ctx* c, const double* W, long ldw, double* Binv, long ldb, long np);
int upload_scaled(pgp_ctx* c, const double* x_dev, long n, long d, const std::vector<double>& sc, double* XsT, long ldp,
                  int dpad, double* scale_dev);
int alloc_factor_buffer(pgp_ctx* c, long np, long ldf, double** F);
int ensure_workspace(pgp_ctx* c, long np);
int solve_lower_multi(pgp_ctx* c, const double* L, long ldl, const double* Wd, double* Y, long ldy, long np, int nrhs,
                      bool trans);
int eet_lower(pgp_ctx* c, const double* E, long lde, double* Binv, long ldb, long np);

struct GatherSrc {
    long n = 0;
    long n_pos = 0;
    const double* K_all = nullptr;
    long ld = 0;
    const int* idx = nullptr;
    const double* m_all = nullptr;
    double* y = nullptr;
    double* m = nullptr;
};
int gather_sym_launch(const GatherSrc& g, double* Kd, long np, hipStream_t st);
int ep_fit_gathered(pgp_ctx* c, const GatherSrc& g, double* nlZ_out, int* sweeps_out, pgp_factor** factor_out);
int laplace_fit_gathered(pgp_ctx* c, const GatherSrc& g, double* nlZ_out, int* steps_out, pgp_factor** factor_out);
int predict_dense_block(pgp_ctx* c, pgp_factor* f, double* Ks, long nb, int nrhs, const double* msd, double* o1, double* o2);
```

### pygps_amd/csrc/gemm_f64.hip

```cpp
#include <algorithm>
#include <atomic>

#include "gemm_tile.h"

void func_max_dynamic_lds(const void* fn, size_t bytes) {
    constexpr int MAXF = 64, MAXD = 16;
    static std::atomic<const void*> fns[MAXF];
    static std::atomic<size_t> done[MAXF][MAXD];
    int dev = 0;
    if (hipGetDevice(&dev) != hipSuccess || dev < 0 || dev >= MAXD) { (void)hipFuncSetAttribute(fn, hipFuncAttributeMaxDynamicSharedMemorySize, (int)bytes); return; }
    int slot = -1;
    for (int i = 0; i < MAXF; ++i) {
        const void* cur = fns[i].load(std::memory_order_acquire);
        if (cur == fn) { slot = i; break; }
        if (cur == nullptr) {
            const void* expect = nullptr;
            if (fns[i].compare_exchange_strong(expect, fn, std::memory_order_acq_rel) || expect == fn) { slot = i; break; }
        }
    }
    if (slot < 0) { (void)hipFuncSetAttribute(fn, hipFuncAttributeMaxDynamicSharedMemorySize, (int)bytes); return; }
    if (done[slot][dev].load(std::memory_order_acquire) >= bytes) return;
    (void)hipFuncSetAttribute(fn, hipFuncAttributeMaxDynamicSharedMemorySize, (int)bytes);
    size_t prev = done[slot][dev].load(std::memory_order_relaxed);
    while (prev < bytes && !done[slot][dev].compare_exchange_weak(prev, bytes, std::memory_order_release)) {}
}


namespace {

using gemm_tile_ns::BK;

__device__ __forceinline__ bool decode_tile(const GemmArgs& g, int b, int T, int TNc, int& ti, int& tj) {
    if (g.order) {
        ti = g.order[2 * b];
        tj = g.order[2 * b + 1];
        return ti >= 0;
    }
    if (g.tri == 2) {
        int r = (int)((sqrt(8.0 * (double)b + 1.0) - 1.0) * 0.5);
        while ((long)(r + 1) * (r + 2) / 2 <= b) ++r;
        while ((long)r * (r + 1) / 2 > b) --r;
        ti = r;
        tj = b - r * (r + 1) / 2;
        return true;
    }
    const int mt = g.M / T;
    ti = b % mt;
    tj = b / mt;
    if (g.rev_cols) tj = g.N / TNc - 1 - tj;
    if (g.rev_rows) ti = mt - 1 - ti;
    return true;
}

template <int TM, int TN, bool AKC, bool BKC, bool DMA = false, bool YIELD = false, bool RING = false>
__global__ __launch_bounds__(256, 2) void gemm_f64_kernel(GemmArgs g) {
    extern __shared__ __attribute__((aligned(16))) double smem[];
    if (g.trace) {
        long long* tr0 = g.trace + 8L * (blockIdx.x + (long)gridDim.x * blockIdx.z);
        tr0[0] = (long long)wall_clock64();
        tr0[6] = (long long)__builtin_readcyclecounter();
    }
    int ti, tj;
    if (!decode_tile(g, (int)blockIdx.x, TM, TN, ti, tj)) return;
    long bz = blockIdx.z;
    if (g.order_z) { bz = ti >> 16; ti &= 0xffff; }
    if (g.wait_flag) {
        if (threadIdx.x == 0) {
            for (unsigned it = 0; (int)(__hip_atomic_load(g.wait_flag, __ATOMIC_ACQUIRE, __HIP_MEMORY_SCOPE_AGENT) - g.wait_target) < 0; ++it) {
                if (it > (1u << 22) || ((it & 1023u) == 1023u && __hip_atomic_load(g.wait_err, __ATOMIC_RELAXED, __HIP_MEMORY_SCOPE_AGENT))) {
                    __hip_atomic_store(g.wait_err, 1u, __ATOMIC_RELAXED, __HIP_MEMORY_SCOPE_AGENT);
                    break;
                }
                __builtin_amdgcn_s_sleep(8);
            }
        }
        __syncthreads();
    }
    if (!YIELD && g.yield_role == 2) {
        pgp_yield_mark(g.yield_flags, +1);
        gemm_tile_ns::gemm_tile<TM, TN, AKC, BKC, DMA, false, RING>(g, ti, tj, bz, smem, (int)(blockIdx.x + gridDim.x * blockIdx.z));
        __syncthreads();
        pgp_yield_mark(g.yield_flags, -1);
        return;
    }
    gemm_tile_ns::gemm_tile<TM, TN, AKC, BKC, DMA, YIELD, RING>(g, ti, tj, bz, smem, (int)(blockIdx.x + gridDim.x * blockIdx.z));
}

template <bool YIELD, bool RING = false>
__global__ __launch_bounds__(256, 2) void gemm_f64_pair_kernel(GemmArgs a, GemmArgs b, int na) {
    extern __shared__ __attribute__((aligned(16))) double smem[];
    auto run = [&](const GemmArgs& g, int bid) {
        if (g.trace) {
            long long* tr0 = g.trace + 8L * bid;
            tr0[0] = (long long)wall_clock64();
            tr0[6] = (long long)__builtin_readcyclecounter();
        }
        int ti, tj;
        if (!decode_tile(g, bid, 128, 128, ti, tj)) return;
        gemm_tile_ns::gemm_tile<128, 128, false, false, true, YIELD, RING>(g, ti, tj, 0, smem, bid);
    };
    if ((int)blockIdx.x < na) run(a, (int)blockIdx.x);
    else run(b, (int)blockIdx.x - na);
}

template <bool YIELD, bool RING = false>
__global__ __launch_bounds__(256, 2) void gemm_f64_fold_kernel(GemmArgs g) {
    extern __shared__ __attribute__((aligned(16))) double smem[];
    const int mt = g.M / 128, half = (mt + 1) / 2;
    const int r = (int)blockIdx.x % half, tj = (int)blockIdx.x / half;
    const int hi = mt - 1 - r;
    const long bz = blockIdx.z;
    gemm_tile_ns::gemm_tile<128, 128, false, false, true, YIELD, RING>(g, hi, tj, bz, smem, 0);
    if (hi != r) {
        __syncthreads();
        gemm_tile_ns::gemm_tile<128, 128, false, false, true, YIELD, RING>(g, r, tj, bz, smem, 0);
    }
}

constexpr size_t DMA_SPARE = 16;

template <int T, bool AKC, bool BKC, bool DMA = false, bool YIELD = false, bool RING = false>
int launch_t(const GemmArgs& g, hipStream_t st) {
    constexpr int SK = BK + 2;
    constexpr int ASZ = AKC ? T * SK : BK * (T + 16);
    constexpr int BSZ = BKC ? T * SK : BK * (T + 16);
    const size_t shm = 2 * (ASZ + BSZ) * sizeof(double) + (DMA ? DMA_SPARE : 0);
    const int mt = g.M / T, nt = g.N / T;
    unsigned nblk = (g.tri == 2) ? (unsigned)((long)mt * (mt + 1) / 2) : (unsigned)(mt * nt);
    if (g.order) nblk = (unsigned)g.norder;
    dim3 grid(nblk, 1, (g.batch > 0 && !g.order_z) ? g.batch : 1);
    func_max_dynamic_lds((const void*)gemm_f64_kernel<T, T, AKC, BKC, DMA, YIELD, RING>, shm);
    hipLaunchKernelGGL((gemm_f64_kernel<T, T, AKC, BKC, DMA, YIELD, RING>), grid, dim3(256), shm, st, g);
    return hipGetLastError() == hipSuccess ? PGP_OK : PGP_ERR_HIP;
}

static bool dma_ok(const GemmArgs& g);
static bool dma1264_ok(const GemmArgs& g) {
    return g.tile == 1264 && dma_ok(g) && !g.tri && !g.order && g.batch <= 1 && !g.order_z && (g.N % 64) == 0 && (g.M % 128) == 0 && g.kmode == KM_FULL;
}
template <bool YIELD, bool RING>
int launch_1264(const GemmArgs& g, hipStream_t st) {
    constexpr int SA_ = 128 + 16;
    const size_t shm = 2 * (BK * SA_ + (BK / 2) * SA_) * sizeof(double) + DMA_SPARE;
    dim3 grid((unsigned)((g.M / 128) * (g.N / 64)), 1, 1);
    func_max_dynamic_lds((const void*)gemm_f64_kernel<128, 64, false, false, true, YIELD, RING>, shm);
    hipLaunchKernelGGL((gemm_f64_kernel<128, 64, false, false, true, YIELD, RING>), grid, dim3(256), shm, st, g);
    return hipGetLastError() == hipSuccess ? PGP_OK : PGP_ERR_HIP;
}

static bool dma_ok(const GemmArgs& g) {
    return g.tile != 64 && (g.dbg & 64) && !g.a_kc && !g.b_kc && (g.K % 16) == 0 && (g.koff % 16) == 0 && (g.batch_dk % 16) == 0;
}

template <int T>
int launch_l(const GemmArgs& g, hipStream_t st) {
    if (!g.a_kc && !g.b_kc) return launch_t<T, false, false>(g, st);
    if (!g.a_kc && g.b_kc) return launch_t<T, false, true>(g, st);
    if (g.a_kc && !g.b_kc) return launch_t<T, true, false>(g, st);
    return launch_t<T, true, true>(g, st);
}

}

bool gemm_f64_uses_dma128(const GemmArgs& g) { return dma_ok(g) && !dma1264_ok(g); }
bool gemm_f64_uses_dma(const GemmArgs& g) { return dma_ok(g); }

static unsigned launch_blocks(const GemmArgs& g) {
    const int mt = g.M / 128, nt = g.N / 128;
    if (g.order) return (unsigned)g.norder;
    return (g.tri == 2) ? (unsigned)((long)mt * (mt + 1) / 2) : (unsigned)(mt * nt);
}
bool gemm_f64_pair_ok(const GemmArgs& a, const GemmArgs& b) {
    auto plain = [](const GemmArgs& g) {
        return g.M > 0 && g.N > 0 && g.tile != 64 && dma_ok(g) && g.batch <= 1 && !g.order_z && !g.wait_flag && g.yield_role != 2;
    };
    return plain(a) && plain(b) && (a.yield_role == 1 && a.yield_flags) == (b.yield_role == 1 && b.yield_flags) && !a.ring == !b.ring;
}
int gemm_f64_launch_pair(const GemmArgs& a, const GemmArgs& b, hipStream_t st) {
    if (!gemm_f64_pair_ok(a, b)) return -2;
    constexpr int SA_ = 128 + 16;
    const size_t shm = 2 * (2 * BK * SA_) * sizeof(double) + DMA_SPARE;
    const unsigned na = launch_blocks(a), nb = launch_blocks(b);
    const bool yield = a.yield_role == 1 && a.yield_flags;
    auto go = [&](auto kern) {
        func_max_dynamic_lds((const void*)kern, shm);
        hipLaunchKernelGGL(kern, dim3(na + nb), dim3(256), shm, st, a, b, (int)na);
    };
    if (a.ring) { if (yield) go(gemm_f64_pair_kernel<true, true>); else go(gemm_f64_pair_kernel<false, true>); }
    else { if (yield) go(gemm_f64_pair_kernel<true, false>); else go(gemm_f64_pair_kernel<false, false>); }
    return hipGetLastError() == hipSuccess ? PGP_OK : PGP_ERR_HIP;
}

static int launch_fold(const GemmArgs& g, hipStream_t st) {
    constexpr int SA_ = 128 + 16;
    const size_t shm = 2 * (2 * BK * SA_) * sizeof(double) + DMA_SPARE;
    const int mt = g.M / 128, nt = g.N / 128;
    dim3 grid((unsigned)(((mt + 1) / 2) * nt), 1, g.batch > 0 ? g.batch : 1);
    const bool yield = g.yield_role == 1 && g.yield_flags;
    auto go = [&](auto kern) {
        func_max_dynamic_lds((const void*)kern, shm);
        hipLaunchKernelGGL(kern, grid, dim3(256), shm, st, g);
    };
    if (g.ring) { if (yield) go(gemm_f64_fold_kernel<true, true>); else go(gemm_f64_fold_kernel<false, true>); }
    else { if (yield) go(gemm_f64_fold_kernel<true, false>); else go(gemm_f64_fold_kernel<false, false>); }
    return hipGetLastError() == hipSuccess ? PGP_OK : PGP_ERR_HIP;
}

int gemm_f64_launch(const GemmArgs& g, hipStream_t st) {
    if (g.M <= 0 || g.N <= 0) return PGP_OK;
    if (g.tile == 64) return launch_l<64>(g, st);
    if (g.fold_rows && g.tile == 128 && dma_ok(g) && !g.tri && !g.order && !g.order_z && !g.wait_flag && g.yield_role != 2 && !g.trace)
        return launch_fold(g, st);
    const bool yield = g.yield_role == 1 && g.yield_flags;
    if (dma1264_ok(g)) {
        if (g.ring) return yield ? launch_1264<true, true>(g, st) : launch_1264<false, true>(g, st);
        return yield ? launch_1264<true, false>(g, st) : launch_1264<false, false>(g, st);
    }
    if (dma_ok(g)) {
        if (g.ring) return yield ? launch_t<128, false, false, true, true, true>(g, st) : launch_t<128, false, false, true, false, true>(g, st);
        return yield ? launch_t<128, false, false, true, true>(g, st) : launch_t<128, false, false, true>(g, st);
    }
    return launch_l<128>(g, st);
}
```

### pygps_amd/csrc/gemm_tile.h

```cpp
#pragma once
#include "common.h"

typedef double double4_t __attribute__((ext_vector_type(4)));
typedef double double2_t __attribute__((ext_vector_type(2)));

namespace gemm_tile_ns {

constexpr int BK = 16;

template <int LDS_OFF>
__device__ __forceinline__ void lds_dma_1k_s(unsigned voff, const double* sbase, unsigned lds_wave_base) {
    asm volatile("s_add_u32 m0, %2, %3\n\ts_nop 0\n\tglobal_load_lds_dwordx4 %0, %1"
                 :: "v"(voff), "s"(sbase), "s"(lds_wave_base), "n"(LDS_OFF) : "memory", "scc");
}
__device__ __forceinline__ const double* uniform_ptr(const double* p) {
    const unsigned long a = (unsigned long)p;
    const unsigned lo = __builtin_amdgcn_readfirstlane((unsigned)a), hi = __builtin_amdgcn_readfirstlane((unsigned)(a >> 32));
    return (const double*)(((unsigned long)hi << 32) | lo);
}
template <int V> struct IC { static constexpr int value = V; };

template <int N>
__device__ __forceinline__ void ring_wait() { asm volatile("s_waitcnt vmcnt(%0)" :: "n"(N) : "memory"); }
template <int N>
__device__ __forceinline__ void ring_wait_barrier() {
    asm volatile("s_waitcnt vmcnt(%0) lgkmcnt(0)" :: "n"(N) : "memory");
    __builtin_amdgcn_s_barrier();
    asm volatile("" ::: "memory");
}
__device__ __forceinline__ void ring_load_f64(double& d, const double* p) {
    asm volatile("global_load_dwordx2 %0, %1, off" : "=v"(d) : "v"(p) : "memory");
}
__device__ __forceinline__ void ring_landed(double& d) { asm volatile("" : "+v"(d)); }
__device__ __forceinline__ void ring_landed(unsigned& d) { asm volatile("" : "+v"(d)); }

__device__ __forceinline__ double swap_adjacent(double v) {
    const int lo = __builtin_amdgcn_update_dpp(0, __double2loint(v), 0xB1, 0xF, 0xF, false);
    const int hi = __builtin_amdgcn_update_dpp(0, __double2hiint(v), 0xB1, 0xF, 0xF, false);
    return __hiloint2double(hi, lo);
}

__device__ __noinline__ void gemm_yield_wait(const unsigned* yf) {
    for (int i = 0; i < 400; ++i) {
        __builtin_amdgcn_s_sleep(32);
        if (__hip_atomic_load(yf, __ATOMIC_RELAXED, __HIP_MEMORY_SCOPE_AGENT) == 0u) break;
    }
}

template <int TM, int TN, bool AKC, bool BKC, bool DMA = false, bool YIELD = false, bool RING = false>
__device__ __forceinline__ void gemm_tile(const GemmArgs& g, int ti, int tj, long bz, double* __restrict__ smem, int wg = 0) {
    static_assert(!RING || DMA, "the staging ring is an LDS-DMA loop");
    static_assert(!DMA || (!AKC && !BKC && TM == 128 && (TN == 128 || TN == 64)), "LDS-DMA staging: M-contiguous operands, 128 x 128 or 128 x 64 tiles");
    constexpr bool BH = DMA && TN == 64;
    constexpr int SA = TM + 16, SB = BH ? TM + 16 : TN + 16, SK = BK + 2;
    constexpr int ASZ = AKC ? TM * SK : BK * SA;
    constexpr int BSZ = BKC ? TN * SK : (BH ? (BK / 2) * SB : BK * SB);
    constexpr int STAGE = ASZ + BSZ;
    constexpr int FM = TM / 32, FN = TN / 32;
    constexpr int AV = TM * BK / 2 / 256;
    constexpr int BV = TN * BK / 2 / 256;

    const int i0 = ti * TM, j0 = tj * TN;
    if (g.batch_dm && i0 >= g.M - (int)bz * g.batch_dm) return;
    const int zero_from = g.zero_from > 0 ? g.zero_from - (int)bz * g.batch_dm : 0;
    if (i0 < g.skip_hi && j0 < g.skip_hi && i0 >= g.skip_lo && j0 >= g.skip_lo) return;
    bool diag = false;
    if (g.tri) {
        if (i0 + g.tri_off < j0) return;
        diag = g.mask_diag && (i0 + g.tri_off == j0);
    }
    int k0 = 0, k1 = g.K;
    const int koff = g.koff + (int)bz * g.batch_dk;
    if (g.kmode == KM_GE_I) k0 = i0 + koff;
    else if (g.kmode == KM_GE_J) k0 = j0 + koff;
    else if (g.kmode == KM_LT_I) k1 = i0 + TM + koff;
    else if (g.kmode == KM_LT_J) k1 = j0 + TN + koff;
    if (g.zf_upper && zero_from > 0 && i0 >= zero_from && i0 - zero_from > k0) k0 = i0 - zero_from;
    if (k0 < 0) k0 = 0;
    if (k1 > g.K) k1 = g.K;
    k0 &= ~(BK - 1);

    const bool a_hi = g.a_split && i0 >= g.a_split;
    const bool c_hi = g.c_split && i0 >= g.c_split;
    const double* __restrict__ A = (a_hi ? g.A2 - g.a_split : g.A) + bz * g.sA;
    const long lda = a_hi ? g.lda2 : g.lda;
    const double* __restrict__ B = g.B + bz * g.sB;
    double* __restrict__ C = (c_hi ? g.C2 - g.c_split : g.C) + bz * g.sC - (bz * (bz - 1) / 2) * g.batch_sC2;
    const long ldc = (c_hi ? g.ldc2 : g.ldc) - bz * g.batch_dldc;
    const double* __restrict__ Cin = g.Cin ? (c_hi ? g.Cin2 - g.c_split : g.Cin) : C;
    const long ldcin = g.Cin ? (c_hi ? g.ldcin2 : g.ldcin) : ldc;

    const int t = threadIdx.x;
    const int lane = t & 63, wave = t >> 6;
    const int wm = (wave & 1) * (TM / 2), wn = (wave >> 1) * (TN / 2);
    const int l15 = lane & 15, l4 = lane >> 4;

    double4_t acc[FM][FN];
    const double ab = g.beta / g.alpha;
    const bool wantc = g.beta != 0.0 && !(zero_from > 0 && i0 >= zero_from);
    constexpr int LZ = 16;
    const bool lazyc = DMA && wantc && (g.dbg & 256) && (k1 - k0) >= (LZ + 2) * BK;
    const bool preload = wantc && !lazyc;
#pragma unroll
    for (int im = 0; im < FM; ++im)
#pragma unroll
        for (int in = 0; in < FN; ++in) {
            if (preload) {
                const double* cp = Cin + (long)(i0 + wm + im * 16 + l15) + (long)(j0 + wn + in * 16 + l4) * ldcin;
#pragma unroll
                for (int r = 0; r < 4; ++r) acc[im][in][r] = ab * cp[(long)(4 * r) * ldcin];
            } else {
#pragma unroll
                for (int r = 0; r < 4; ++r) acc[im][in][r] = 0.0;
            }
        }

    double2_t ra[AV], rb[BV];
    const double* pa[AV];
    const double* pb[BV];
    long astep, bstep;
    if (!AKC) {
        constexpr int VPR = TM / 2, RPP = 256 / VPR;
#pragma unroll
        for (int p = 0; p < AV; ++p) pa[p] = A + (long)(i0 + 2 * (t % VPR)) + (long)(k0 + t / VPR + p * RPP) * lda;
        astep = (long)BK * lda;
    } else {
#pragma unroll
        for (int p = 0; p < AV; ++p) pa[p] = A + (long)(k0 + 2 * (t & 7)) + (long)(i0 + (t >> 3) + p * 32) * lda;
        astep = BK;
    }
    if (!BKC) {
        constexpr int VPR = TN / 2, RPP = 256 / VPR;
#pragma unroll
        for (int p = 0; p < BV; ++p) pb[p] = B + (long)(j0 + 2 * (t % VPR)) + (long)(k0 + t / VPR + p * RPP) * g.ldb;
        bstep = (long)BK * g.ldb;
    } else {
#pragma unroll
        for (int p = 0; p < BV; ++p) pb[p] = B + (long)(k0 + 2 * (t & 7)) + (long)(j0 + (t >> 3) + p * 32) * g.ldb;
        bstep = BK;
    }
    const double* da[4];
    const double* db[4];
    unsigned lds_w = 0;
    const unsigned dvoff = (unsigned)lane * 16u;
    unsigned dvoff_b = dvoff;
    if constexpr (BH) dvoff_b = (unsigned)(lane & 31) * 16u + (unsigned)(lane >> 5) * (unsigned)(4L * g.ldb * 8L);
    const unsigned smem_lds = (unsigned)(unsigned long)(__attribute__((address_space(3))) void*)smem;
    if constexpr (DMA) {
        static_assert(SA == SB, "one LDS row stride for both operands");
#pragma unroll
        for (int p = 0; p < 4; ++p) {
            da[p] = uniform_ptr(A + (long)i0 + (long)(k0 + wave + 4 * p) * lda);
            db[p] = uniform_ptr(B + (long)j0 + (long)(k0 + wave + (BH ? 8 * (p & 1) : 4 * p)) * g.ldb);
        }
        lds_w = __builtin_amdgcn_readfirstlane(smem_lds + (unsigned)wave * (unsigned)(SA * 8));
    }
    const long dstep_a = (long)BK * lda, dstep_b = (long)BK * g.ldb;
    auto dma_stage = [&](auto bufc) {
        constexpr int O = decltype(bufc)::value * STAGE * 8;
        if constexpr (DMA && BH) {
            lds_dma_1k_s<O + 0 * SA * 8>(dvoff, da[0], lds_w);
            lds_dma_1k_s<O + ASZ * 8 + 0 * SB * 8>(dvoff_b, db[0], lds_w);
            lds_dma_1k_s<O + 4 * SA * 8>(dvoff, da[1], lds_w);
            lds_dma_1k_s<O + 8 * SA * 8>(dvoff, da[2], lds_w);
            lds_dma_1k_s<O + ASZ * 8 + 4 * SB * 8>(dvoff_b, db[1], lds_w);
            lds_dma_1k_s<O + 12 * SA * 8>(dvoff, da[3], lds_w);
#pragma unroll
            for (int p = 0; p < 4; ++p) da[p] += dstep_a;
            db[0] += dstep_b; db[1] += dstep_b;
        } else if constexpr (DMA) {
            lds_dma_1k_s<O + 0 * SA * 8>(dvoff, da[0], lds_w);
            lds_dma_1k_s<O + ASZ * 8 + 0 * SB * 8>(dvoff, db[0], lds_w);
            lds_dma_1k_s<O + 4 * SA * 8>(dvoff, da[1], lds_w);
            lds_dma_1k_s<O + ASZ * 8 + 4 * SB * 8>(dvoff, db[1], lds_w);
            lds_dma_1k_s<O + 8 * SA * 8>(dvoff, da[2], lds_w);
            lds_dma_1k_s<O + ASZ * 8 + 8 * SB * 8>(dvoff, db[2], lds_w);
            lds_dma_1k_s<O + 12 * SA * 8>(dvoff, da[3], lds_w);
            lds_dma_1k_s<O + ASZ * 8 + 12 * SB * 8>(dvoff, db[3], lds_w);
#pragma unroll
            for (int p = 0; p < 4; ++p) { da[p] += dstep_a; db[p] += dstep_b; }
        }
    };
    constexpr int P = BH ? 3 : 4;
    auto ring_piece = [&](auto bufc, auto halfc, auto jc) __attribute__((always_inline)) {
        constexpr int O = decltype(bufc)::value * STAGE * 8, hf = decltype(halfc)::value, j = decltype(jc)::value;
        if constexpr (DMA && BH) {
            if constexpr (j == 0) { lds_dma_1k_s<O + (8 * hf) * SA * 8>(dvoff, da[2 * hf], lds_w); da[2 * hf] += dstep_a; }
            if constexpr (j == 1) { lds_dma_1k_s<O + ASZ * 8 + (4 * hf) * SB * 8>(dvoff_b, db[hf], lds_w); db[hf] += dstep_b; }
            if constexpr (j == 2) { lds_dma_1k_s<O + (8 * hf + 4) * SA * 8>(dvoff, da[2 * hf + 1], lds_w); da[2 * hf + 1] += dstep_a; }
        } else if constexpr (DMA) {
            if constexpr (j == 0) { lds_dma_1k_s<O + (8 * hf) * SA * 8>(dvoff, da[2 * hf], lds_w); da[2 * hf] += dstep_a; }
            if constexpr (j == 1) { lds_dma_1k_s<O + ASZ * 8 + (8 * hf) * SB * 8>(dvoff, db[2 * hf], lds_w); db[2 * hf] += dstep_b; }
            if constexpr (j == 2) { lds_dma_1k_s<O + (8 * hf + 4) * SA * 8>(dvoff, da[2 * hf + 1], lds_w); da[2 * hf + 1] += dstep_a; }
            if constexpr (j == 3) { lds_dma_1k_s<O + ASZ * 8 + (8 * hf + 4) * SB * 8>(dvoff, db[2 * hf + 1], lds_w); db[2 * hf + 1] += dstep_b; }
        }
    };
    auto ring_issue = [&](auto bufc, auto halfc) __attribute__((always_inline)) {
        ring_piece(bufc, halfc, IC<0>{}); ring_piece(bufc, halfc, IC<1>{}); ring_piece(bufc, halfc, IC<2>{});
        if constexpr (P == 4) ring_piece(bufc, halfc, IC<3>{});
    };
    auto gload = [&](int) {
#pragma unroll
        for (int p = 0; p < AV; ++p) { ra[p] = *(const double2_t*)pa[p]; pa[p] += astep; }
#pragma unroll
        for (int p = 0; p < BV; ++p) { rb[p] = *(const double2_t*)pb[p]; pb[p] += bstep; }
    };
    auto sstore = [&](int buf) {
        double* sa = smem + buf * STAGE;
        double* sb = sa + ASZ;
        if (!AKC) {
            constexpr int VPR = TM / 2;
            constexpr int RPP = 256 / VPR;
#pragma unroll
            for (int p = 0; p < AV; ++p) {
                const int mv = t % VPR, kr = t / VPR + p * RPP;
                *(double2_t*)(sa + kr * SA + 2 * mv) = ra[p];
            }
        } else {
#pragma unroll
            for (int p = 0; p < AV; ++p) {
                const int kp = t & 7, m = (t >> 3) + p * 32;
                *(double2_t*)(sa + m * SK + 2 * kp) = ra[p];
            }
        }
        if (!BKC) {
            constexpr int VPR = TN / 2;
            constexpr int RPP = 256 / VPR;
#pragma unroll
            for (int p = 0; p < BV; ++p) {
                const int nv = t % VPR, kr = t / VPR + p * RPP;
                *(double2_t*)(sb + kr * SB + 2 * nv) = rb[p];
            }
        } else {
#pragma unroll
            for (int p = 0; p < BV; ++p) {
                const int kp = t & 7, n = (t >> 3) + p * 32;
                *(double2_t*)(sb + n * SK + 2 * kp) = rb[p];
            }
        }
    };

    double cr[8];
    const int ring_half = __builtin_amdgcn_readfirstlane(wave >> 1);
    auto ring_cact = [&](int fold_step) __attribute__((always_inline)) { return !BH || ring_half == (fold_step >> 3); };
    auto ring_cload = [&](int chunk) __attribute__((always_inline)) {
        const int in = chunk / (FM / 2), hf = chunk % (FM / 2);
#pragma unroll
        for (int q = 0; q < 2; ++q) {
            const double* cp = Cin + (long)(i0 + wm + (2 * hf + q) * 16 + l15) + (long)(j0 + wn + in * 16 + l4) * ldcin;
#pragma unroll
            for (int r = 0; r < 4; ++r) ring_load_f64(cr[4 * q + r], cp + (long)(4 * r) * ldcin);
        }
    };
    if (k0 < k1) {
        if constexpr (RING) {
            ring_issue(IC<0>{}, IC<0>{});
            ring_issue(IC<0>{}, IC<1>{});
            if (k0 + BK < k1) {
                ring_issue(IC<1>{}, IC<0>{});
                if (lazyc && ring_cact(1)) { ring_cload(0); ring_wait_barrier<2 * P + 8>(); }
                else ring_wait_barrier<2 * P>();
            } else ring_wait_barrier<P>();
        } else {
        if constexpr (DMA) {
            dma_stage(IC<0>{});
            asm volatile("s_waitcnt vmcnt(0)" ::: "memory");
        } else {
            gload(k0);
            sstore(0);
        }
        __syncthreads();
        }
        double fa[2][FM], fb[2][FN];
        auto ldfrag = [&](int b, int ks, int slot) {
            const double* sa = smem + b * STAGE;
            const double* sb = sa + ASZ;
            const int k = ks * 4 + l4;
#pragma unroll
            for (int im = 0; im < FM; ++im) {
                const int m = wm + im * 16 + l15;
                fa[slot][im] = AKC ? sa[m * SK + k] : sa[k * SA + m];
            }
#pragma unroll
            for (int in = 0; in < FN; ++in) {
                const int n = wn + in * 16 + l15;
                if constexpr (BH) fb[slot][in] = sb[(l4 + 4 * (ks >> 1)) * SB + (ks & 1) * 64 + n];
                else fb[slot][in] = BKC ? sb[n * SK + k] : sb[k * SB + n];
            }
        };
        auto mfmas = [&](int slot) {
#pragma unroll
            for (int in = 0; in < FN; ++in)
#pragma unroll
                for (int im = 0; im < FM; ++im)
                    acc[im][in] = __builtin_amdgcn_mfma_f64_16x16x4f64(fb[slot][in], fa[slot][im], acc[im][in], 0, 0, 0);
        };
        constexpr int NS = BK / 4;
        ldfrag(0, 0, 0);
        const unsigned* yf = nullptr;
        if constexpr (YIELD) yf = g.yield_flags + pgp_cu_key();
        auto kstep = [&](int kt, auto bufc, auto pollc) {
            constexpr int buf = decltype(bufc)::value;
            constexpr bool POLL = YIELD && decltype(pollc)::value != 0;
            const bool more = kt + BK < k1;
            if constexpr (DMA) { if (more) dma_stage(IC<(buf ^ 1)>{}); }
            else if (more) gload(kt + BK);
            unsigned yv = 0u;
            if constexpr (POLL) yv = __hip_atomic_load(yf, __ATOMIC_RELAXED, __HIP_MEMORY_SCOPE_AGENT);
#pragma unroll
            for (int ks = 0; ks + 1 < NS; ++ks) {
                ldfrag(buf, ks + 1, (ks + 1) & 1);
                mfmas(ks & 1);
            }
            if constexpr (DMA) asm volatile("s_waitcnt vmcnt(0)" ::: "memory");
            else if (more) sstore(buf ^ 1);
            __syncthreads();
            if constexpr (POLL) { if (__builtin_amdgcn_readfirstlane(yv) != 0u) gemm_yield_wait(yf); }
            if (more) ldfrag(buf ^ 1, 0, NS & 1);
            __builtin_amdgcn_sched_barrier(0);
            mfmas((NS - 1) & 1);
        };
        auto mfma1 = [&](int slot, auto ic) __attribute__((always_inline)) {
            constexpr int i = decltype(ic)::value, in = i / FM, im = i % FM;
            acc[im][in] = __builtin_amdgcn_mfma_f64_16x16x4f64(fb[slot][in], fa[slot][im], acc[im][in], 0, 0, 0);
        };
        auto mfmas_p = [&](int slot, bool go, auto bufc, auto halfc) __attribute__((always_inline)) {
            auto one = [&](auto ic) __attribute__((always_inline)) {
                constexpr int i = decltype(ic)::value;
                mfma1(slot, ic);
                if constexpr (i % 2 == 1 && i / 2 < P) {
                    __builtin_amdgcn_sched_barrier(0);
                    if (go) ring_piece(bufc, halfc, IC<i / 2>{});
                    __builtin_amdgcn_sched_barrier(0);
                }
            };
            one(IC<0>{}); one(IC<1>{}); one(IC<2>{}); one(IC<3>{}); one(IC<4>{}); one(IC<5>{}); one(IC<6>{}); one(IC<7>{});
            if constexpr (FM * FN == 16) {
                one(IC<8>{}); one(IC<9>{}); one(IC<10>{}); one(IC<11>{}); one(IC<12>{}); one(IC<13>{}); one(IC<14>{}); one(IC<15>{});
            }
        };
        auto rstep = [&](int kt, auto bufc, auto pollc, int cp, int cmchunk, bool cmact) __attribute__((always_inline)) {
            constexpr int buf = decltype(bufc)::value;
            constexpr bool POLL = YIELD && decltype(pollc)::value != 0;
            constexpr int Y = POLL ? 1 : 0;
            const bool more = kt + BK < k1, more2 = kt + 2 * BK < k1;
            unsigned yv = 0u;
            if constexpr (POLL) asm volatile("global_load_dword %0, %1, %2 sc1" : "=v"(yv) : "v"(0u), "s"(yf) : "memory");
            ldfrag(buf, 1, 1);
            mfmas_p(0, more, IC<(buf ^ 1)>{}, IC<1>{});
            if (more) {
                if (cp != 0) ring_wait_barrier<2 * P + Y + 8>();
                else ring_wait_barrier<2 * P + Y>();
            } else ring_wait_barrier<0>();
            const bool cm = cmchunk >= 0 && cmact;
            if (cm) ring_cload(cmchunk);
            ldfrag(buf, 2, 0);
            __builtin_amdgcn_sched_barrier(0);
            mfmas_p(1, more2, IC<buf>{}, IC<0>{});
            ldfrag(buf, 3, 1);
            mfmas(0);
            if (more2) {
                if (cm) ring_wait_barrier<2 * P + 8>();
                else ring_wait_barrier<2 * P>();
            } else if (more) ring_wait_barrier<P>();
            else ring_wait_barrier<0>();
            if constexpr (POLL) { ring_landed(yv); if (__builtin_amdgcn_readfirstlane(yv) != 0u) gemm_yield_wait(yf); }
            if (more) ldfrag(buf ^ 1, 0, 0);
            __builtin_amdgcn_sched_barrier(0);
            mfmas(1);
        };
        int kt = k0;
        if constexpr (RING) {
            if (lazyc) {
                static_assert(FM == 4 && (FN == 4 || FN == 2), "lazy C: 64-row wave tiles, 64 or 32 columns");
                auto lzstep = [&](auto stc) __attribute__((always_inline)) {
                    constexpr int st = decltype(stc)::value;
                    constexpr int chunk = (BH ? (st & 7) : st) >> 1, in = chunk / (FM / 2), hf = chunk % (FM / 2);
                    if constexpr ((st & 1) != 0) {
                        if (ring_cact(st)) {
#pragma unroll
                            for (int i = 0; i < 8; ++i) ring_landed(cr[i]);
#pragma unroll
                            for (int q = 0; q < 2; ++q)
#pragma unroll
                                for (int r = 0; r < 4; ++r) acc[2 * hf + q][in][r] = fma(ab, cr[4 * q + r], acc[2 * hf + q][in][r]);
                        }
                        rstep(kt, IC<1>{}, IC<0>{}, 0, st + 2 < LZ ? (BH ? ((st + 2) & 7) : (st + 2)) >> 1 : -1, ring_cact(st + 2));
                    } else {
                        const int cp = ring_cact(st + 1) ? 8 : 0;
                        if constexpr ((st & 3) == 0) rstep(kt, IC<0>{}, IC<1>{}, cp, -1, false);
                        else rstep(kt, IC<0>{}, IC<0>{}, cp, -1, false);
                    }
                    kt += BK;
                };
                static_assert(LZ == 16, "the prologue is written out");
                lzstep(IC<0>{}); lzstep(IC<1>{}); lzstep(IC<2>{}); lzstep(IC<3>{}); lzstep(IC<4>{}); lzstep(IC<5>{}); lzstep(IC<6>{}); lzstep(IC<7>{});
                lzstep(IC<8>{}); lzstep(IC<9>{}); lzstep(IC<10>{}); lzstep(IC<11>{}); lzstep(IC<12>{}); lzstep(IC<13>{}); lzstep(IC<14>{}); lzstep(IC<15>{});
                if (g.trace) smem[2 * STAGE] = __longlong_as_double((long long)wall_clock64());
            }
            while (kt < k1) {
                rstep(kt, IC<0>{}, IC<1>{}, 0, -1, false);
                kt += BK;
                if (kt >= k1) break;
                rstep(kt, IC<1>{}, IC<0>{}, 0, -1, false);
                kt += BK;
                if constexpr (YIELD) {
                    if (kt >= k1) break;
                    rstep(kt, IC<0>{}, IC<0>{}, 0, -1, false);
                    kt += BK;
                    if (kt >= k1) break;
                    rstep(kt, IC<1>{}, IC<0>{}, 0, -1, false);
                    kt += BK;
                }
            }
        } else {
        if constexpr (DMA) {
            if (lazyc) {
                double4_t creg[2];
                static_assert(FM == 4 && (FN == 4 || FN == 2), "lazy C: 64-row wave tiles, 64 or 32 columns");
                const int my_half = __builtin_amdgcn_readfirstlane(wave >> 1);
#pragma unroll
                for (int st = 0; st < LZ; ++st) {
                    const int chunk = (BH ? (st & 7) : st) >> 1, in = chunk / (FM / 2), hf = chunk % (FM / 2);
                    const bool act = !BH || my_half == (st >> 3);
                    if (!(st & 1)) {
                        if (act) {
#pragma unroll
                        for (int q = 0; q < 2; ++q) {
                            const double* cp = Cin + (long)(i0 + wm + (2 * hf + q) * 16 + l15) + (long)(j0 + wn + in * 16 + l4) * ldcin;
#pragma unroll
                            for (int r = 0; r < 4; ++r) creg[q][r] = cp[(long)(4 * r) * ldcin];
                        }
                        }
                    } else if (act) {
#pragma unroll
                        for (int q = 0; q < 2; ++q)
#pragma unroll
                            for (int r = 0; r < 4; ++r) acc[2 * hf + q][in][r] = fma(ab, creg[q][r], acc[2 * hf + q][in][r]);
                    }
                    if (st & 1) kstep(kt, IC<1>{}, IC<0>{});
                    else if ((st & 3) == 0) kstep(kt, IC<0>{}, IC<1>{});
                    else kstep(kt, IC<0>{}, IC<0>{});
                    kt += BK;
                }
                if (g.trace) smem[2 * STAGE] = __longlong_as_double((long long)wall_clock64());
            }
        }
        while (kt < k1) {
            kstep(kt, IC<0>{}, IC<1>{});
            kt += BK;
            if (kt >= k1) break;
            kstep(kt, IC<1>{}, IC<0>{});
            kt += BK;
            if constexpr (YIELD) {
                if (kt >= k1) break;
                kstep(kt, IC<0>{}, IC<0>{});
                kt += BK;
                if (kt >= k1) break;
                kstep(kt, IC<1>{}, IC<0>{});
                kt += BK;
            }
        }
        }
    }

    long long* const trc = g.trace ? g.trace + 8L * wg : nullptr;
    if (trc) {
        trc[2] = (long long)wall_clock64();
        if constexpr (DMA) trc[1] = lazyc ? __double_as_longlong(smem[2 * STAGE]) : 0ll;
    }
    if (!diag && (g.dbg & 512) && !(ldc & 1) && !((unsigned long)C & 15ul)) {
        const bool odd = l15 & 1;
#pragma unroll
        for (int im = 0; im < FM; ++im)
#pragma unroll
            for (int in = 0; in < FN; ++in) {
                const int m = wm + im * 16 + l15;
                const int nb = wn + in * 16 + l4;
#pragma unroll
                for (int r = 0; r < 4; r += 2) {
                    const double x = g.alpha * acc[im][in][r], yv = g.alpha * acc[im][in][r + 1];
                    const double nx = swap_adjacent(x), ny = swap_adjacent(yv);
                    const double2_t val = odd ? double2_t{ny, yv} : double2_t{x, nx};
                    double* cp = C + (long)(i0 + (odd ? m - 1 : m)) + (long)(j0 + nb + 4 * (odd ? r + 1 : r)) * ldc;
                    *(double2_t*)cp = val;
                }
            }
    } else {
#pragma unroll
    for (int im = 0; im < FM; ++im)
#pragma unroll
        for (int in = 0; in < FN; ++in) {
            const int m = wm + im * 16 + l15;
            const int nb = wn + in * 16 + l4;
            double* cp = C + (long)(i0 + m) + (long)(j0 + nb) * ldc;
#pragma unroll
            for (int r = 0; r < 4; ++r) {
                const int n = nb + 4 * r;
                if (!diag || m >= n) cp[(long)(4 * r) * ldc] = g.alpha * acc[im][in][r];
            }
        }
    }
    if (trc) {
        trc[3] = (long long)wall_clock64();
        asm volatile("s_waitcnt vmcnt(0)" ::: "memory");
        __syncthreads();
        trc[4] = (long long)wall_clock64(); trc[5] = (long long)pgp_cu_key(); trc[7] = (long long)__builtin_readcyclecounter();
    }
}

}
```

### pygps_amd/csrc/testhooks.hip

```cpp
#include <time.h>
#include <cstdlib>
#include <cmath>
#include <vector>

#include "ctx.h"
#include <chrono>
#include <thread>

#include "testhooks.h"
#include "erf_lik.h"
#include "laplace_lik.h"

typedef double double4_t __attribute__((ext_vector_type(4)));

namespace {
__global__ __launch_bounds__(256) void mfma_peak_kernel(double* out, int iters, double a0, double b0) {
    double4_t acc[8];
#pragma unroll
    for (int i = 0; i < 8; ++i) acc[i] = double4_t{0.0, 0.0, 0.0, 0.0};
    double a = a0 + threadIdx.x * 1e-9, b = b0;
    for (int it = 0; it < iters; ++it) {
#pragma unroll
        for (int i = 0; i < 8; ++i) acc[i] = __builtin_amdgcn_mfma_f64_16x16x4f64(a, b, acc[i], 0, 0, 0);
    }
    double s = 0.0;
#pragma unroll
    for (int i = 0; i < 8; ++i) s += acc[i][0] + acc[i][1] + acc[i][2] + acc[i][3];
    if (s == 123.456) out[0] = s;
}
template <int NACC, bool VACC>
__global__ __launch_bounds__(256) void mfma_cycles_kernel(long long* out, int iters, double a0) {
    double4_t acc[NACC];
#pragma unroll
    for (int i = 0; i < NACC; ++i) acc[i] = double4_t{0.0, 0.0, 0.0, 0.0};
    double a = a0 + threadIdx.x * 1e-9, b = 1.0;
    const long long t0 = __builtin_readcyclecounter();
    const long long w0 = wall_clock64();
    for (int it = 0; it < iters; ++it) {
#pragma unroll
        for (int i = 0; i < NACC; ++i) {
            if (VACC) asm volatile("v_mfma_f64_16x16x4_f64 %0, %1, %2, %0" : "+v"(acc[i]) : "v"(a), "v"(b));
            else acc[i] = __builtin_amdgcn_mfma_f64_16x16x4f64(a, b, acc[i], 0, 0, 0);
        }
    }
    double s = 0.0;
#pragma unroll
    for (int i = 0; i < NACC; ++i) s += acc[i][0] + acc[i][1] + acc[i][2] + acc[i][3];
    const long long t1 = __builtin_readcyclecounter();
    const long long w1 = wall_clock64();
    if (blockIdx.x == 0 && threadIdx.x == 0) { out[0] = t1 - t0; out[1] = w1 - w0; }
    if (s == 123.456) out[2] = (long long)s;
}
}

extern "C" {

int pgp_test_mfma_cycles(pgp_ctx* c, int iters, int nacc, int waves_per_simd, double* out3) {
    if (!c || !out3) return -1;
    HIP_TRY(hipSetDevice(c->device));
    long long* d = nullptr;
    HIP_TRY(hipMalloc((void**)&d, 32));
    hipEvent_t e0, e1;
    HIP_TRY(hipEventCreate(&e0)); HIP_TRY(hipEventCreate(&e1));
    const int blocks = waves_per_simd > 0 ? c->prop.multiProcessorCount * waves_per_simd : -waves_per_simd;
    for (int rep = 0; rep < 2; ++rep) {
        HIP_TRY(hipEventRecord(e0, c->st));
        if (nacc == 1) hipLaunchKernelGGL((mfma_cycles_kernel<1, false>), dim3(blocks), dim3(256), 0, c->st, d, iters, 1.0);
        else if (nacc == 4) hipLaunchKernelGGL((mfma_cycles_kernel<4, false>), dim3(blocks), dim3(256), 0, c->st, d, iters, 1.0);
        else if (nacc == 8) hipLaunchKernelGGL((mfma_cycles_kernel<8, false>), dim3(blocks), dim3(256), 0, c->st, d, iters, 1.0);
        else if (nacc == -4) hipLaunchKernelGGL((mfma_cycles_kernel<4, true>), dim3(blocks), dim3(256), 0, c->st, d, iters, 1.0);
        else hipLaunchKernelGGL((mfma_cycles_kernel<8, true>), dim3(blocks), dim3(256), 0, c->st, d, iters, 1.0);
        HIP_TRY(hipEventRecord(e1, c->st));
        HIP_TRY(hipStreamSynchronize(c->st));
    }
    float ms = 0.f;
    HIP_TRY(hipEventElapsedTime(&ms, e0, e1));
    long long h[2];
    HIP_TRY(hipMemcpy(h, d, 16, hipMemcpyDeviceToHost));
    out3[0] = (double)h[0]; out3[1] = (double)h[1]; out3[2] = ms;
    (void)hipEventDestroy(e0); (void)hipEventDestroy(e1); (void)hipFree(d);
    return PGP_OK;
}

__global__ __launch_bounds__(256) void valu_peak_kernel(double* out, int iters, double a0, double b0) {
    double s[16], a[4], b[4];
    for (int i = 0; i < 16; ++i) s[i] = 0.0;
    for (int i = 0; i < 4; ++i) { a[i] = a0 + threadIdx.x * 1e-3 + i; b[i] = b0 + i * 0.5; }
    for (int it = 0; it < iters; ++it) {
#pragma unroll
        for (int i = 0; i < 4; ++i)
#pragma unroll
            for (int j = 0; j < 4; ++j) {
                const double d = a[i] - b[j];
                s[4 * i + j] = fma(d, d, s[4 * i + j]);
            }
#pragma unroll
        for (int i = 0; i < 4; ++i) { a[i] += 1e-9; }
    }
    double t = 0.0;
    for (int i = 0; i < 16; ++i) t += s[i];
    if (t == 12345.678) out[0] = t;
}

int pgp_test_valu_peak(pgp_ctx* c, int iters, int waves_per_simd, double* out2) {
    if (!c || !out2) return -1;
    HIP_TRY(hipSetDevice(c->device));
    double* out = nullptr;
    HIP_TRY(hipMalloc((void**)&out, 8));
    hipEvent_t e0, e1;
    HIP_TRY(hipEventCreate(&e0)); HIP_TRY(hipEventCreate(&e1));
    const int blocks = c->prop.multiProcessorCount * waves_per_simd;
    hipLaunchKernelGGL(valu_peak_kernel, dim3(blocks), dim3(256), 0, c->st, out, 64, 1.0, 1.0);
    HIP_TRY(hipEventRecord(e0, c->st));
    hipLaunchKernelGGL(valu_peak_kernel, dim3(blocks), dim3(256), 0, c->st, out, iters, 1.0, 1.0);
    HIP_TRY(hipEventRecord(e1, c->st));
    HIP_TRY(hipStreamSynchronize(c->st));
    float ms = 0.f;
    HIP_TRY(hipEventElapsedTime(&ms, e0, e1));
    const double winstr = (double)blocks * 4.0 * (double)iters * 36.0;
    const double per_simd = (double)waves_per_simd * (double)iters * 36.0;
    out2[0] = winstr / (ms * 1e6);
    out2[1] = (ms * 1e-3) * 2.4e9 / per_simd;
    (void)hipEventDestroy(e0); (void)hipEventDestroy(e1); (void)hipFree(out);
    return PGP_OK;
}

int pgp_test_mfma_peak(pgp_ctx* ctx, int iters, double* tflops_out) {
    if (!ctx || !tflops_out) return -1;
    pgp_ctx* c = ctx;
    HIP_TRY(hipSetDevice(c->device));
    hipDeviceProp_t prop;
    HIP_TRY(hipGetDeviceProperties(&prop, c->device));
    double* out = nullptr;
    HIP_TRY(hipMalloc((void**)&out, 8));
    hipEvent_t e0, e1;
    HIP_TRY(hipEventCreate(&e0)); HIP_TRY(hipEventCreate(&e1));
    const int blocks = prop.multiProcessorCount * 2;
    hipLaunchKernelGGL(mfma_peak_kernel, dim3(blocks), dim3(256), 0, c->st, out, 16, 1.0, 1.0);
    HIP_TRY(hipEventRecord(e0, c->st));
    hipLaunchKernelGGL(mfma_peak_kernel, dim3(blocks), dim3(256), 0, c->st, out, iters, 1.0, 1.0);
    HIP_TRY(hipEventRecord(e1, c->st));
    HIP_TRY(hipStreamSynchronize(c->st));
    float ms = 0.f;
    HIP_TRY(hipEventElapsedTime(&ms, e0, e1));
    const double flops = (double)blocks * 4.0 * (double)iters * 8.0 * 2048.0;
    *tflops_out = flops / (ms * 1e-3) / 1e12;
    (void)hipEventDestroy(e0); (void)hipEventDestroy(e1); (void)hipFree(out);
    return PGP_OK;
}

int pgp_test_leaf_ticks(pgp_ctx* c, double* ticks_out) {
    if (!c || !ticks_out) return -1;
    HIP_TRY(hipSetDevice(c->device));
    std::vector<double> A(128 * 128, 0.0);
    for (int i = 0; i < 128; ++i)
        for (int j = 0; j < 128; ++j) A[i + j * 128] = (i == j ? 3.0 : 0.0) + 1.0 / (1.0 + (i > j ? i - j : j - i));
    double *Ad, *pk; int* info; long long* tk;
    HIP_TRY(hipMalloc((void**)&Ad, A.size() * 8)); HIP_TRY(hipMalloc((void**)&pk, PACK_DOUBLES * 8));
    HIP_TRY(hipMalloc((void**)&info, 4)); HIP_TRY(hipMalloc((void**)&tk, 24 * 8));
    HIP_TRY(hipMemset(info, 0, 4)); HIP_TRY(hipMemset(tk, 0, 24 * 8));
    for (int rep = 0; rep < 3; ++rep) {
        HIP_TRY(hipMemcpy(Ad, A.data(), A.size() * 8, hipMemcpyHostToDevice));
        int rc = leaf_potrf_launch(Ad, 128, pk, info, 0, c->st, tk, nullptr, c->leaf_pivot);
        if (rc) return rc;
        HIP_TRY(hipStreamSynchronize(c->st));
    }
    long long h[24];
    HIP_TRY(hipMemcpy(h, tk, sizeof(h), hipMemcpyDeviceToHost));
    for (int i = 0; i < 24; ++i) ticks_out[i] = (double)h[i];
    (void)hipFree(Ad); (void)hipFree(pk); (void)hipFree(info); (void)hipFree(tk);
    return PGP_OK;
}

namespace {
__global__ __launch_bounds__(256) void wave_costs_kernel(double* __restrict__ out, double seed) {
    __shared__ double lds[512];
    __shared__ int nxt[256];
    const int t = threadIdx.x;
    lds[t] = seed + t; lds[t + 256] = seed - t; nxt[t] = (t * 7 + 1) & 255;
    __syncthreads();
    long long a, b, ra, rb;
    double x = seed, acc = 0.0;
    a = __builtin_amdgcn_s_memtime(); ra = __builtin_amdgcn_s_memrealtime();
#pragma unroll 16
    for (int i = 0; i < 2048; ++i) x = fma(x, 0.999999, 1e-9);
    acc += x;
    asm volatile("" :: "v"(x));
    b = __builtin_amdgcn_s_memtime(); rb = __builtin_amdgcn_s_memrealtime();
    if (t == 0) { out[0] = (double)(b - a) / 2048.0; out[1] = (double)(rb - ra); out[9] = (double)(b - a); }
    double y[8];
#pragma unroll
    for (int q = 0; q < 8; ++q) y[q] = seed + q;
    a = __builtin_amdgcn_s_memtime();
    for (int i = 0; i < 256; ++i) {
#pragma unroll
        for (int q = 0; q < 8; ++q) y[q] = fma(y[q], 0.999999, 1e-9);
    }
#pragma unroll
    for (int q = 0; q < 8; ++q) acc += y[q];
    asm volatile("" :: "v"(acc));
    b = __builtin_amdgcn_s_memtime();
    if (t == 0) out[2] = (double)(b - a) / 2048.0;
    int idx = t;
    a = __builtin_amdgcn_s_memtime();
    for (int i = 0; i < 512; ++i) idx = nxt[idx];
    asm volatile("" :: "v"(idx));
    b = __builtin_amdgcn_s_memtime();
    if (t == 0) out[3] = (double)(b - a) / 512.0;
    acc += idx;
    a = __builtin_amdgcn_s_memtime();
    for (int i = 0; i < 512; ++i) {
        double sum = 0.0;
        const int o = (i & 1) * 256;
#pragma unroll
        for (int q = 0; q < 20; ++q) sum += lds[o + ((t >> 4) + 16 * q) % 256];
        acc = fma(sum, 1e-9, acc);
        asm volatile("" :: "v"(acc));
    }
    b = __builtin_amdgcn_s_memtime();
    if (t == 0) out[4] = (double)(b - a) / 512.0;
    a = __builtin_amdgcn_s_memtime();
    for (int i = 0; i < 512; ++i) __syncthreads();
    b = __builtin_amdgcn_s_memtime();
    if (t == 0) out[5] = (double)(b - a) / 512.0;
    a = __builtin_amdgcn_s_memtime();
    for (int i = 0; i < 512; ++i) {
        if ((t & 15) == (i & 15)) lds[(i & 1) * 256 + (t >> 4)] = acc + i;
        __syncthreads();
        acc += lds[(i & 1) * 256 + (i & 15)];
        asm volatile("" :: "v"(acc));
    }
    b = __builtin_amdgcn_s_memtime();
    if (t == 0) out[6] = (double)(b - a) / 512.0;
    x = seed + 2.0;
    a = __builtin_amdgcn_s_memtime();
#pragma unroll 16
    for (int i = 0; i < 512; ++i) x = __builtin_amdgcn_rcp(x) + 1.5;
    asm volatile("" :: "v"(x));
    b = __builtin_amdgcn_s_memtime();
    if (t == 0) out[7] = (double)(b - a) / 512.0;
    acc += x;
    x = seed + 2.0;
    a = __builtin_amdgcn_s_memtime();
#pragma unroll 16
    for (int i = 0; i < 512; ++i) x = __builtin_amdgcn_rsq(x) + 1.5;
    asm volatile("" :: "v"(x));
    b = __builtin_amdgcn_s_memtime();
    if (t == 0) out[8] = (double)(b - a) / 512.0;
    acc += x;
    if (acc == 12345.678 && t == 0) out[15] = acc;
}
}
int pgp_test_wave_costs(pgp_ctx* c, double* out16) {
    if (!c || !out16) return -1;
    HIP_TRY(hipSetDevice(c->device));
    double* od;
    HIP_TRY(hipMalloc((void**)&od, 16 * 8));
    HIP_TRY(hipMemset(od, 0, 16 * 8));
    for (int rep = 0; rep < 3; ++rep) hipLaunchKernelGGL(wave_costs_kernel, dim3(1), dim3(256), 0, c->st, od, 1.0 + 1e-3 * rep);
    HIP_TRY(hipStreamSynchronize(c->st));
    HIP_TRY(hipMemcpy(out16, od, 16 * 8, hipMemcpyDeviceToHost));
    (void)hipFree(od);
    return PGP_OK;
}

int pgp_test_assemble(pgp_ctx* c, int kind, int mode, int64_t n, int64_t d, int iters, double* ms_out) {
    if (!c || !ms_out) return -1;
    HIP_TRY(hipSetDevice(c->device));
    const long np = round_up(n, 128);
    const int dpad = (int)round_up(d, SKC);
    std::vector<double> x((size_t)n * d);
    unsigned long long s = 88172645463325252ULL;
    for (auto& v : x) { s ^= s << 13; s ^= s >> 7; s ^= s << 17; v = ((double)(s >> 11) / 9007199254740992.0 - 0.5) * 3.4; }
    std::vector<double> hyp(kind == PGP_COV_RBFARD ? d + 1 : 2, 0.0);
    for (size_t i = 0; i + 1 < hyp.size(); ++i) hyp[i] = 0.5 * log((double)d);
    CovSpec cp;
    CHK(make_spec(c, kind, hyp.data(), (int)hyp.size(), 3, 0, -1, d, cp));
    const std::vector<double>& sc = cp.scale;
    double *xd, *XT, *scd, *out;
    const long ldo = mode == 2 ? np + 128 : n;
    HIP_TRY(hipMalloc((void**)&xd, x.size() * 8)); HIP_TRY(hipMalloc((void**)&XT, (size_t)dpad * np * 8));
    HIP_TRY(hipMalloc((void**)&scd, dpad * 8)); HIP_TRY(hipMalloc((void**)&out, (size_t)ldo * np * 8));
    HIP_TRY(hipMemcpy(xd, x.data(), x.size() * 8, hipMemcpyHostToDevice));
    HIP_TRY(hipMemcpy(scd, sc.data(), d * 8, hipMemcpyHostToDevice));
    CHK(scale_transpose_launch(xd, n, (int)d, scd, XT, np, dpad, c->st));
    const bool gram = c->gram_assembly && cov_gram_applies(cp, dpad);
    double* prep = nullptr;
    if (gram) HIP_TRY(hipMalloc((void**)&prep, (size_t)hadamard_prep_count(np) * 8));
    hipEvent_t e0, e1;
    HIP_TRY(hipEventCreate(&e0)); HIP_TRY(hipEventCreate(&e1));
    int rc = PGP_OK;
    for (int it = -std::max(100, iters); it < iters && rc == PGP_OK; ++it) {
        if (it == 0) HIP_TRY(hipEventRecord(e0, c->st));
        if (gram) {
            rc = hadamard_prepare_launch(XT, np, n, np, dpad, cp, prep, c->st, true);
            if (rc == PGP_OK) rc = mode == 2 ? cov_factor_gram_launch(XT, np, n, np, dpad, cp, 100.0, out, ldo, prep, c->st)
                                             : cov_sym_gram_launch(XT, np, n, dpad, cp, out, 0, prep, c->st);
        } else
        rc = mode == 2 ? cov_factor_launch(XT, np, n, np, dpad, cp, 100.0, out, ldo, c->st)
                       : cov_sym_launch(XT, np, n, dpad, cp, out, c->st, 0);
    }
    HIP_TRY(hipEventRecord(e1, c->st));
    HIP_TRY(hipStreamSynchronize(c->st));
    float ms = 0.f;
    HIP_TRY(hipEventElapsedTime(&ms, e0, e1));
    *ms_out = ms / iters;
    (void)hipEventDestroy(e0); (void)hipEventDestroy(e1);
    (void)hipFree(xd); (void)hipFree(XT); (void)hipFree(scd); (void)hipFree(out);
    if (prep) (void)hipFree(prep);
    return rc;
}

namespace {
__global__ __launch_bounds__(256) void store_only_sym_kernel(double* out, long n, const int2* tab, long ntiles, double v) {
    const int t = threadIdx.x;
    for (long ti = blockIdx.x; ti < ntiles; ti += gridDim.x) {
        const int2 ij = tab[ti];
        double* base = out + (long)ij.x * 64 * n + (long)ij.y * 64;
        double* mir = out + (long)ij.y * 64 * n + (long)ij.x * 64;
#pragma unroll
        for (int p = 0; p < 8; ++p) {
            const int e = t + 256 * p, r = e >> 5, cpair = e & 31;
            *(double2_t*)(base + (long)r * n + 2 * cpair) = double2_t{v, v + 1.0};
        }
        if (ij.x != ij.y) {
#pragma unroll
            for (int p = 0; p < 8; ++p) {
                const int e = t + 256 * p, r = e >> 5, cpair = e & 31;
                *(double2_t*)(mir + (long)r * n + 2 * cpair) = double2_t{v, v + 1.0};
            }
        }
    }
}
__global__ __launch_bounds__(256) void store_only_linear_kernel(double* out, long n2, double v) {
    const long i = ((long)blockIdx.x * 256 + threadIdx.x) * 2;
    if (i + 1 < n2) *(double2_t*)(out + i) = double2_t{v, v + 1.0};
}
}

int pgp_test_store_roof(pgp_ctx* c, int64_t n, int grid, int iters, double* out3) {
    if (!c || !out3 || n <= 0 || n % 64 || iters <= 0) return -1;
    HIP_TRY(hipSetDevice(c->device));
    const long nt = n / 64, S = 8, nst = (nt + S - 1) / S;
    std::vector<int2> h;
    for (long SI = 0; SI < nst; ++SI)
        for (long SJ = SI; SJ < nst; ++SJ)
            for (long i = SI * S; i < std::min(nt, SI * S + S); ++i)
                for (long j = std::max(i, SJ * S); j < std::min(nt, SJ * S + S); ++j) h.push_back(make_int2((int)i, (int)j));
    int2* tab; double* out;
    HIP_TRY(hipMalloc((void**)&tab, h.size() * sizeof(int2)));
    HIP_TRY(hipMalloc((void**)&out, (size_t)n * n * 8));
    HIP_TRY(hipMemcpy(tab, h.data(), h.size() * sizeof(int2), hipMemcpyHostToDevice));
    hipEvent_t e0, e1;
    HIP_TRY(hipEventCreate(&e0)); HIP_TRY(hipEventCreate(&e1));
    const long ntl = (long)h.size(), n2 = (long)n * n;
    const unsigned g = (unsigned)std::min<long>(ntl, grid > 0 ? grid : 4096);
    for (int which = 0; which < 3; ++which) {
        for (int it = -std::max(50, iters / 2); it < iters; ++it) {
            if (it == 0) HIP_TRY(hipEventRecord(e0, c->st));
            if (which == 0) hipLaunchKernelGGL(store_only_sym_kernel, dim3(g), dim3(256), 0, c->st, out, (long)n, tab, ntl, 1.0);
            else if (which == 1) HIP_TRY(hipMemsetAsync(out, 0, (size_t)n2 * 8, c->st));
            else hipLaunchKernelGGL(store_only_linear_kernel, dim3((unsigned)((n2 / 2 + 255) / 256)), dim3(256), 0, c->st, out, n2, 1.0);
        }
        HIP_TRY(hipEventRecord(e1, c->st));
        HIP_TRY(hipStreamSynchronize(c->st));
        float ms = 0.f;
        HIP_TRY(hipEventElapsedTime(&ms, e0, e1));
        out3[which] = ms / iters;
    }
    (void)hipEventDestroy(e0); (void)hipEventDestroy(e1);
    (void)hipFree(tab); (void)hipFree(out);
    return hipGetLastError() == hipSuccess ? PGP_OK : PGP_ERR_HIP;
}

int pgp_test_gemm(pgp_ctx* ctx, int tile, int a_kc, int b_kc, int tri, int mask_diag, int kmode, int koff,
                  double alpha, double beta, const double* A, int64_t lda, const double* B, int64_t ldb, double* C,
                  int64_t ldc, int M, int N, int K, int iters, double* ms_out) {
    if (!ctx) return -1;
    pgp_ctx* c = ctx;
    const bool poll = getenv("PGP_TEST_GEMM_YIELD") != nullptr;
    if (poll && !c->yield_flags) return -2;
    HIP_TRY(hipSetDevice(c->device));
    const size_t an = (size_t)lda * (a_kc ? M : K), bn = (size_t)ldb * (b_kc ? N : K), cn = (size_t)ldc * N;
    double *Ad, *Bd, *Cd;
    HIP_TRY(hipMalloc((void**)&Ad, an * 8)); HIP_TRY(hipMalloc((void**)&Bd, bn * 8)); HIP_TRY(hipMalloc((void**)&Cd, cn * 8));
    HIP_TRY(hipMemcpy(Ad, A, an * 8, hipMemcpyHostToDevice));
    HIP_TRY(hipMemcpy(Bd, B, bn * 8, hipMemcpyHostToDevice));
    HIP_TRY(hipMemcpy(Cd, C, cn * 8, hipMemcpyHostToDevice));
    GemmArgs g{};
    g.A = Ad; g.lda = lda; g.a_kc = a_kc; g.B = Bd; g.ldb = ldb; g.b_kc = b_kc; g.C = Cd; g.ldc = ldc;
    g.M = M; g.N = N; g.K = K; g.alpha = alpha; g.beta = beta; g.tri = tri; g.tri_off = 0; g.mask_diag = mask_diag;
    g.kmode = kmode; g.koff = koff; g.batch = 1; g.tile = tile; g.dbg = c->gemm_dbg; g.ring = c->tile_ring != 0;
    if (getenv("PGP_TEST_GEMM_FOLD")) g.fold_rows = 1;
    if (poll && gemm_f64_uses_dma(g)) { g.yield_flags = c->yield_flags; g.yield_role = 1; }
    hipStream_t ts = c->st;
    int rc = gemm_f64_launch(g, ts);
    HIP_TRY(hipStreamSynchronize(ts));
    if (rc == PGP_OK) HIP_TRY(hipMemcpy(C, Cd, cn * 8, hipMemcpyDeviceToHost));
    if (rc == PGP_OK && iters > 0 && ms_out) {
        hipEvent_t e0, e1;
        HIP_TRY(hipEventCreate(&e0)); HIP_TRY(hipEventCreate(&e1));
        {
            HIP_TRY(hipEventRecord(e0, ts));
            rc = gemm_f64_launch(g, ts);
            HIP_TRY(hipEventRecord(e1, ts));
            HIP_TRY(hipStreamSynchronize(ts));
            float m1 = 0.f;
            HIP_TRY(hipEventElapsedTime(&m1, e0, e1));
            const int nwarm = (int)std::min(4000.0, std::max(1.0, 80.0 / std::max(1e-3, (double)m1)));
            for (int i = 0; i < nwarm && rc == PGP_OK; ++i) rc = gemm_f64_launch(g, ts);
        }
        HIP_TRY(hipEventRecord(e0, ts));
        for (int i = 0; i < iters; ++i) rc = gemm_f64_launch(g, ts);
        HIP_TRY(hipEventRecord(e1, ts));
        HIP_TRY(hipStreamSynchronize(ts));
        float ms = 0.f;
        HIP_TRY(hipEventElapsedTime(&ms, e0, e1));
        *ms_out = ms / iters;
        (void)hipEventDestroy(e0); (void)hipEventDestroy(e1);
    }
    (void)hipFree(Ad); (void)hipFree(Bd); (void)hipFree(Cd);
    return rc;
}

int pgp_test_gemm_trace(pgp_ctx* c, int M, int K, int tri, int warm, int conc, long long* out, int64_t out_words, int64_t* nblk_out) {
    if (!c || !out || !nblk_out || M % 128 || K % 16) return -1;
    HIP_TRY(hipSetDevice(c->device));
    const long mt = M / 128;
    const long nblk = tri ? mt * (mt + 1) / 2 : mt * mt;
    if (out_words < 8 * nblk) return -2;
    double *A, *Cd, *C2; long long* tr;
    HIP_TRY(hipMalloc((void**)&A, (size_t)M * K * 8)); HIP_TRY(hipMalloc((void**)&Cd, (size_t)M * M * 8));
    HIP_TRY(hipMalloc((void**)&C2, (size_t)M * M * 8)); HIP_TRY(hipMalloc((void**)&tr, (size_t)nblk * 64));
    HIP_TRY(hipMemset(tr, 0, (size_t)nblk * 64));
    std::vector<double> h((size_t)M * K);
    unsigned long long s = 88172645463325252ULL;
    for (auto& v : h) { s ^= s << 13; s ^= s >> 7; s ^= s << 17; v = ((double)(s >> 11) / 9007199254740992.0 - 0.5) * 0.01; }
    HIP_TRY(hipMemcpy(A, h.data(), h.size() * 8, hipMemcpyHostToDevice));
    HIP_TRY(hipMemset(Cd, 0, (size_t)M * M * 8)); HIP_TRY(hipMemset(C2, 0, (size_t)M * M * 8));
    GemmArgs g{};
    g.A = A; g.lda = M; g.B = A; g.ldb = M; g.C = Cd; g.ldc = M; g.M = M; g.N = M; g.K = K; g.alpha = -1.0; g.beta = 1.0;
    g.tri = tri ? 2 : 0; g.mask_diag = tri ? 1 : 0; g.batch = 1; g.tile = 128; g.dbg = c->gemm_dbg; g.ring = c->tile_ring != 0;
    int rc = PGP_OK;
    for (int i = 0; i < warm && rc == PGP_OK; ++i) rc = gemm_f64_launch(g, c->st);
    HIP_TRY(hipStreamSynchronize(c->st));
    GemmArgs g2 = g; g2.C = C2;
    if (conc > 0 && rc == PGP_OK) rc = gemm_f64_launch(g2, c->st2);
    g.trace = tr;
    if (rc == PGP_OK) rc = gemm_f64_launch(g, c->st);
    HIP_TRY(hipStreamSynchronize(c->st)); HIP_TRY(hipStreamSynchronize(c->st2));
    HIP_TRY(hipMemcpy(out, tr, (size_t)nblk * 64, hipMemcpyDeviceToHost));
    *nblk_out = nblk;
    (void)hipFree(A); (void)hipFree(Cd); (void)hipFree(C2); (void)hipFree(tr);
    return rc;
}

int pgp_test_read_gemm_trace(pgp_ctx* c, long long* out, int64_t words, int64_t* nwg) {
    if (!c || !out || !nwg || !c->gemm_trace) return -1;
    HIP_TRY(hipSetDevice(c->device));
    HIP_TRY(hipDeviceSynchronize());
    const long n = std::min<long>(c->gemm_trace_pos, words / 8);
    HIP_TRY(hipMemcpy(out, c->gemm_trace, (size_t)n * 64, hipMemcpyDeviceToHost));
    HIP_TRY(hipMemset(c->gemm_trace, 0, (size_t)c->gemm_trace_cap * 64));
    c->gemm_trace_pos = 0;
    *nwg = n;
    return PGP_OK;
}

int pgp_test_gemm_skip_wait(pgp_ctx* ctx, int tile, const double* A, const double* B, double* C, int n, int K, int skip_lo,
                            int skip_hi, int wait_ms, int* timed_out) {
    if (!ctx) return -1;
    pgp_ctx* c = ctx;
    HIP_TRY(hipSetDevice(c->device));
    DevScratch scr;
    double *Ad = nullptr, *Bd = nullptr, *Cd = nullptr;
    unsigned* fl = nullptr;
    const size_t an = (size_t)n * K * 8, cn = (size_t)n * n * 8;
    CHK(scr.alloc(&Ad, an)); CHK(scr.alloc(&Bd, an)); CHK(scr.alloc(&Cd, cn));
    CHK(scr.alloc(&fl, 16));
    HIP_TRY(hipMemcpy(Ad, A, an, hipMemcpyHostToDevice));
    HIP_TRY(hipMemcpy(Bd, B, an, hipMemcpyHostToDevice));
    HIP_TRY(hipMemcpy(Cd, C, cn, hipMemcpyHostToDevice));
    HIP_TRY(hipMemset(fl, 0, 16));
    GemmArgs g{};
    g.A = Ad; g.lda = n; g.B = Bd; g.ldb = n; g.C = Cd; g.ldc = n; g.M = n; g.N = n; g.K = K; g.alpha = -1.0; g.beta = 1.0;
    g.tri = 2; g.mask_diag = 1; g.batch = 1; g.tile = tile; g.dbg = c->gemm_dbg; g.ring = c->tile_ring != 0; g.skip_lo = skip_lo; g.skip_hi = skip_hi;
    if (wait_ms > 0) { g.wait_flag = fl; g.wait_target = 7u; g.wait_err = fl + 1; }
    int rc = gemm_f64_launch(g, c->st);
    if (rc == PGP_OK && wait_ms > 0) {
        std::this_thread::sleep_for(std::chrono::milliseconds(wait_ms));
        const unsigned seven = 7u;
        HIP_TRY(hipMemcpyAsync(fl, &seven, sizeof(seven), hipMemcpyHostToDevice, c->st2));
        HIP_TRY(hipStreamSynchronize(c->st2));
    }
    HIP_TRY(hipStreamSynchronize(c->st));
    unsigned flh[2] = {0u, 0u};
    HIP_TRY(hipMemcpy(flh, fl, sizeof(flh), hipMemcpyDeviceToHost));
    if (timed_out) *timed_out = (int)flh[1];
    if (rc == PGP_OK) HIP_TRY(hipMemcpy(C, Cd, cn, hipMemcpyDeviceToHost));
    return rc;
}

int pgp_test_gemm_shrink(pgp_ctx* ctx, const double* Y, int64_t ldy, int M, int K, int w, int nb, int dm, int zero_from,
                         double* C, int64_t ldc, int64_t sC) {
    if (!ctx) return -1;
    pgp_ctx* c = ctx;
    if (!Y || !C || M <= 0 || M % 128 || w % 128 || K % 16 || dm % 128 || nb < 1) return -2;
    HIP_TRY(hipSetDevice(c->device));
    DevScratch scr;
    double *yd, *cd;
    const size_t cbytes = (size_t)((nb - 1) * sC + ldc * w) * 8;
    CHK(scr.alloc(&yd, (size_t)ldy * K * 8)); CHK(scr.alloc(&cd, cbytes));
    HIP_TRY(hipMemcpy(yd, Y, (size_t)ldy * K * 8, hipMemcpyHostToDevice));
    HIP_TRY(hipMemcpy(cd, C, cbytes, hipMemcpyHostToDevice));
    GemmArgs g{};
    g.A = yd; g.lda = ldy; g.B = yd; g.ldb = ldy; g.C = cd; g.ldc = ldc; g.M = M; g.N = w; g.K = K;
    g.alpha = -1.0; g.beta = 1.0; g.tri = 1; g.mask_diag = 1; g.kmode = KM_FULL; g.tile = 128;
    g.batch = nb; g.sA = dm; g.sB = dm; g.sC = sC; g.batch_dm = dm; g.zero_from = zero_from;
    CHK(gemm_prof(c, PC_GEMM_TRAIL, g, c->st));
    HIP_TRY(hipStreamSynchronize(c->st));
    HIP_TRY(hipMemcpy(C, cd, cbytes, hipMemcpyDeviceToHost));
    return PGP_OK;
}

int pgp_test_gemm_zskip(pgp_ctx* ctx, int tile, int tri, int mask_diag, int zero_from, int zf_upper, double alpha, double beta,
                        const double* A, int64_t lda, const double* B, int64_t ldb, const double* Cin, double* C, int64_t ldc,
                        int M, int N, int K) {
    if (!ctx) return -1;
    pgp_ctx* c = ctx;
    if (!A || !B || !C || M <= 0 || N <= 0 || M % 128 || N % 128 || K % 16 || lda < M || ldb < N || ldc < M) return -2;
    if ((tile != 64 && tile != 128) || zero_from < 0 || zero_from % 128) return -2;
    HIP_TRY(hipSetDevice(c->device));
    DevScratch scr;
    double *Ad = nullptr, *Bd = nullptr, *Cd = nullptr, *Ci = nullptr;
    const size_t an = (size_t)lda * K * 8, bn = (size_t)ldb * K * 8, cn = (size_t)ldc * N * 8;
    CHK(scr.alloc(&Ad, an)); CHK(scr.alloc(&Bd, bn)); CHK(scr.alloc(&Cd, cn));
    HIP_TRY(hipMemcpy(Ad, A, an, hipMemcpyHostToDevice));
    HIP_TRY(hipMemcpy(Bd, B, bn, hipMemcpyHostToDevice));
    HIP_TRY(hipMemcpy(Cd, C, cn, hipMemcpyHostToDevice));
    if (Cin) { CHK(scr.alloc(&Ci, cn)); HIP_TRY(hipMemcpy(Ci, Cin, cn, hipMemcpyHostToDevice)); }
    GemmArgs g{};
    g.A = Ad; g.lda = lda; g.B = Bd; g.ldb = ldb; g.C = Cd; g.ldc = ldc; g.M = M; g.N = N; g.K = K; g.alpha = alpha; g.beta = beta;
    if (Ci) { g.Cin = Ci; g.ldcin = ldc; }
    g.tri = tri; g.mask_diag = mask_diag; g.kmode = KM_FULL; g.batch = 1; g.tile = tile; g.dbg = c->gemm_dbg; g.ring = c->tile_ring != 0;
    g.zero_from = zero_from; g.zf_upper = zf_upper;
    const int rc = gemm_f64_launch(g, c->st);
    HIP_TRY(hipStreamSynchronize(c->st));
    if (rc == PGP_OK) HIP_TRY(hipMemcpy(C, Cd, cn, hipMemcpyDeviceToHost));
    return rc;
}

int pgp_test_gemm_pair(pgp_ctx* ctx, double alpha, double beta, const double* A, int64_t lda, const double* B, int64_t ldb, double* Ca,
                       double* Cb, int64_t ldc, int M, int N, int Ka, int Kb) {
    if (!ctx) return -1;
    pgp_ctx* c = ctx;
    const int K = std::max(Ka, Kb);
    if (!A || !B || !Ca || !Cb || M <= 0 || N <= 0 || M % 128 || N % 128 || Ka <= 0 || Kb <= 0 || Ka % 16 || Kb % 16 || lda < M || ldb < N || ldc < M) return -2;
    HIP_TRY(hipSetDevice(c->device));
    DevScratch scr;
    double *Ad = nullptr, *Bd = nullptr, *Cad = nullptr, *Cbd = nullptr;
    const size_t an = (size_t)lda * K * 8, bn = (size_t)ldb * K * 8, cn = (size_t)ldc * N * 8;
    CHK(scr.alloc(&Ad, an)); CHK(scr.alloc(&Bd, bn)); CHK(scr.alloc(&Cad, cn)); CHK(scr.alloc(&Cbd, cn));
    HIP_TRY(hipMemcpy(Ad, A, an, hipMemcpyHostToDevice));
    HIP_TRY(hipMemcpy(Bd, B, bn, hipMemcpyHostToDevice));
    HIP_TRY(hipMemcpy(Cad, Ca, cn, hipMemcpyHostToDevice));
    HIP_TRY(hipMemcpy(Cbd, Cb, cn, hipMemcpyHostToDevice));
    GemmArgs g{};
    g.A = Ad; g.lda = lda; g.B = Bd; g.ldb = ldb; g.C = Cad; g.ldc = ldc; g.M = M; g.N = N; g.K = Ka; g.alpha = alpha; g.beta = beta;
    g.kmode = KM_FULL; g.batch = 1; g.tile = 128; g.dbg = c->gemm_dbg; g.ring = c->tile_ring != 0;
    GemmArgs h = g;
    h.C = Cbd; h.K = Kb;
    const int rc = gemm_f64_launch_pair(g, h, c->st);
    HIP_TRY(hipStreamSynchronize(c->st));
    if (rc == PGP_OK) { HIP_TRY(hipMemcpy(Ca, Cad, cn, hipMemcpyDeviceToHost)); HIP_TRY(hipMemcpy(Cb, Cbd, cn, hipMemcpyDeviceToHost)); }
    return rc;
}

}

namespace {
__device__ unsigned g_probe_claim[16];
__device__ unsigned g_probe_cnt[4];
__device__ long long g_probe_t[4];
__device__ unsigned g_probe_log[4 * 2048];
__global__ void holder_kernel(long long hold_ticks, int reserve) {
    extern __shared__ double hs[];
    __shared__ int leave;
    if (threadIdx.x == 0) {
        int mine = 0;
        if (reserve > 0) {
            const unsigned hw = __builtin_amdgcn_s_getreg((4 << 0) | (0 << 6) | (31 << 11));
            const unsigned xcc = __builtin_amdgcn_s_getreg((20 << 0) | (0 << 6) | (3 << 11)) & 15u;
            const unsigned key = 1u + ((hw >> 8) & 0xffu);
            const unsigned prev = atomicCAS(&g_probe_claim[xcc], 0u, key);
            mine = prev == 0u || prev == key;
        }
        leave = mine;
        atomicAdd(&g_probe_cnt[mine ? 1 : 0], 1u);
        if (blockIdx.x < 2048) {
            const unsigned hw = __builtin_amdgcn_s_getreg((4 << 0) | (0 << 6) | (31 << 11));
            const unsigned xcc = __builtin_amdgcn_s_getreg((20 << 0) | (0 << 6) | (3 << 11));
            g_probe_log[4 * blockIdx.x] = hw; g_probe_log[4 * blockIdx.x + 1] = xcc; g_probe_log[4 * blockIdx.x + 2] = mine;
            g_probe_log[4 * blockIdx.x + 3] = (unsigned)(wall_clock64() & 0xffffffffu);
        }
        if (blockIdx.x == 0) g_probe_t[0] = wall_clock64();
    }
    __syncthreads();
    if (leave) return;
    hs[threadIdx.x] = 1.0;
    const long long t0 = wall_clock64();
    while (wall_clock64() - t0 < hold_ticks) __builtin_amdgcn_s_sleep(20);
}
__global__ void probe_kernel() {
    extern __shared__ double ps[];
    if (threadIdx.x == 0) { g_probe_t[1] = wall_clock64(); ps[0] = 1.0; }
}
__global__ void probe_mark_kernel() { if (threadIdx.x == 0) g_probe_t[2] = wall_clock64(); }
}

extern "C" int pgp_test_slot_probe(pgp_ctx* c, int nwg, int lds_kb, int hold_us, int reserve, int probe_lds_kb, int delay_us,
                                   double* out4) {
    if (!c || !out4) return -1;
    HIP_TRY(hipSetDevice(c->device));
    unsigned zero16[16] = {0}; unsigned zero4[4] = {0}; long long zt[4] = {0, 0, 0, 0};
    HIP_TRY(hipMemcpyToSymbol(HIP_SYMBOL(g_probe_claim), zero16, sizeof(zero16)));
    HIP_TRY(hipMemcpyToSymbol(HIP_SYMBOL(g_probe_cnt), zero4, sizeof(zero4)));
    HIP_TRY(hipMemcpyToSymbol(HIP_SYMBOL(g_probe_t), zt, sizeof(zt)));
    (void)hipFuncSetAttribute((const void*)holder_kernel, hipFuncAttributeMaxDynamicSharedMemorySize, 160 * 1024);
    (void)hipFuncSetAttribute((const void*)probe_kernel, hipFuncAttributeMaxDynamicSharedMemorySize, 160 * 1024);
    HIP_TRY(hipDeviceSynchronize());
    hipLaunchKernelGGL(holder_kernel, dim3(nwg), dim3(256), (size_t)lds_kb * 1024, c->st, (long long)hold_us * 100, reserve);
    struct timespec ts = {0, (long)delay_us * 1000};
    nanosleep(&ts, nullptr);
    hipLaunchKernelGGL(probe_mark_kernel, dim3(1), dim3(64), 0, c->st2);
    hipLaunchKernelGGL(probe_kernel, dim3(1), dim3(256), (size_t)probe_lds_kb * 1024, c->st2);
    HIP_TRY(hipDeviceSynchronize());
    unsigned cnt[4]; long long t[4];
    HIP_TRY(hipMemcpyFromSymbol(cnt, HIP_SYMBOL(g_probe_cnt), sizeof(cnt)));
    HIP_TRY(hipMemcpyFromSymbol(t, HIP_SYMBOL(g_probe_t), sizeof(t)));
    out4[0] = (double)(t[1] - t[2]) / 100.0; out4[1] = cnt[0]; out4[2] = cnt[1]; out4[3] = (double)(t[1] - t[0]) / 100.0;
    if (getenv("PGP_PROBE_DUMP")) {
        static unsigned lg[4 * 2048];
        HIP_TRY(hipMemcpyFromSymbol(lg, HIP_SYMBOL(g_probe_log), sizeof(lg)));
        for (int i = 0; i < nwg && i < 2048; ++i)
            fprintf(stderr, "wg %4d hw %08x cu %2u sh %u se %u xcc %08x leave %u t %u\n", i, lg[4 * i], (lg[4 * i] >> 8) & 15u, (lg[4 * i] >> 12) & 1u,
                    (lg[4 * i] >> 13) & 7u, lg[4 * i + 1], lg[4 * i + 2], lg[4 * i + 3] - lg[3]);
    }
    return PGP_OK;
}

extern "C" int pgp_test_cumask_gemm(pgp_ctx* c, int M, int K, int reserve_per_xcd, int stride, int iters, double* out2) {
    if (!c || !out2) return -1;
    HIP_TRY(hipSetDevice(c->device));
    const int ncu = c->prop.multiProcessorCount;
    std::vector<uint32_t> mask((ncu + 31) / 32, 0u);
    int kept = 0;
    for (int i = 0; i < ncu; ++i) {
        const int within = stride == 8 ? i / 8 : i % (ncu / 8);
        const bool keep = within >= reserve_per_xcd;
        if (keep) { mask[i / 32] |= 1u << (i % 32); ++kept; }
    }
    hipStream_t ms = nullptr;
    HIP_TRY(hipExtStreamCreateWithCUMask(&ms, (uint32_t)mask.size(), mask.data()));
    DevScratch scr;
    double *A, *Cm;
    CHK(scr.alloc(&A, (size_t)M * K * 8)); CHK(scr.alloc(&Cm, (size_t)M * M * 8));
    HIP_TRY(hipMemset(A, 0, (size_t)M * K * 8)); HIP_TRY(hipMemset(Cm, 0, (size_t)M * M * 8));
    GemmArgs g{};
    g.A = A; g.lda = M; g.B = A; g.ldb = M; g.C = Cm; g.ldc = M; g.M = M; g.N = M; g.K = K;
    g.alpha = -1.0; g.beta = 1.0; g.tile = 128; g.batch = 1; g.dbg = c->gemm_dbg; g.ring = c->tile_ring != 0;
    hipEvent_t e0, e1;
    HIP_TRY(hipEventCreate(&e0)); HIP_TRY(hipEventCreate(&e1));
    hipStream_t sts[2] = {ms, c->st};
    for (int s = 0; s < 2; ++s) {
        for (int i = 0; i < 3; ++i) CHK(gemm_f64_launch(g, sts[s]));
        HIP_TRY(hipStreamSynchronize(sts[s]));
        HIP_TRY(hipEventRecord(e0, sts[s]));
        for (int i = 0; i < iters; ++i) CHK(gemm_f64_launch(g, sts[s]));
        HIP_TRY(hipEventRecord(e1, sts[s]));
        HIP_TRY(hipStreamSynchronize(sts[s]));
        float t = 0.f;
        HIP_TRY(hipEventElapsedTime(&t, e0, e1));
        out2[s] = t / iters;
    }
    (void)hipEventDestroy(e0); (void)hipEventDestroy(e1);
    (void)hipStreamDestroy(ms);
    return kept;
}

__global__ void pgp_probe_spin_kernel(unsigned* flag, long long wait_ticks, long long* out) {
    const long long t0 = (long long)wall_clock64();
    long long t = t0;
    unsigned seen = 0u;
    while ((t = (long long)wall_clock64()) - t0 < wait_ticks) {
        if (__hip_atomic_load(flag, __ATOMIC_RELAXED, __HIP_MEMORY_SCOPE_AGENT)) { seen = 1u; break; }
        __builtin_amdgcn_s_sleep(16);
    }
    if (threadIdx.x == 0) { out[0] = (long long)seen; out[1] = t - t0; }
}
__global__ void pgp_probe_set_kernel(unsigned* flag) { __hip_atomic_store(flag, 1u, __ATOMIC_RELAXED, __HIP_MEMORY_SCOPE_AGENT); }
extern "C" int pgp_test_stream_concurrency(pgp_ctx* c, int wait_us, double* out2) {
    if (!c || !out2) return -1;
    HIP_TRY(hipSetDevice(c->device));
    DevScratch scr;
    double* buf;
    CHK(scr.alloc(&buf, 64));
    HIP_TRY(hipMemset(buf, 0, 64));
    unsigned* flag = (unsigned*)buf;
    long long* res = (long long*)(buf + 2);
    hipLaunchKernelGGL(pgp_probe_spin_kernel, dim3(1), dim3(64), 0, c->st2, flag, (long long)wait_us * 100LL, res);
    hipLaunchKernelGGL(pgp_probe_set_kernel, dim3(1), dim3(1), 0, c->st, flag);
    HIP_TRY(hipStreamSynchronize(c->st2));
    HIP_TRY(hipStreamSynchronize(c->st));
    long long h[2] = {0, 0};
    HIP_TRY(hipMemcpy(h, res, sizeof(h), hipMemcpyDeviceToHost));
    out2[0] = (double)h[0]; out2[1] = (double)h[1] / 100.0;
    return PGP_OK;
}

namespace {
__global__ void laplace_lik_test_kernel(int lik, double sn2, const double* __restrict__ y, const double* __restrict__ f,
                                        double* __restrict__ out, int n) {
    const int i = blockIdx.x * blockDim.x + threadIdx.x;
    if (i >= n) return;
    double lp, d1, d2, d3;
    if (lik == PGP_LIK_GAUSS) gauss_laplace_derivs(y[i], f[i], sn2, &lp, &d1, &d2, &d3);
    else erf_laplace_derivs(y[i], f[i], &lp, &d1, &d2, &d3);
    out[i] = lp; out[n + i] = d1; out[2L * n + i] = d2; out[3L * n + i] = d3;
}
}

extern "C" int pgp_test_laplace_lik(pgp_ctx* c, int lik, double log_sn, const double* y, const double* f, int n, double* out) {
    if (!c || !y || !f || !out || n <= 0) return -1;
    if (lik != PGP_LIK_ERF && lik != PGP_LIK_GAUSS) return -2;
    HIP_TRY(hipSetDevice(c->device));
    DevScratch scr;
    double *yd, *fd, *od;
    CHK(scr.alloc(&yd, (size_t)n * 8)); CHK(scr.alloc(&fd, (size_t)n * 8)); CHK(scr.alloc(&od, (size_t)4 * n * 8));
    HIP_TRY(hipMemcpy(yd, y, (size_t)n * 8, hipMemcpyHostToDevice));
    HIP_TRY(hipMemcpy(fd, f, (size_t)n * 8, hipMemcpyHostToDevice));
    hipLaunchKernelGGL(laplace_lik_test_kernel, dim3((unsigned)((n + 255) / 256)), dim3(256), 0, c->st, lik, exp(2.0 * log_sn), yd, fd, od, n);
    HIP_TRY(hipStreamSynchronize(c->st));
    HIP_TRY(hipMemcpy(out, od, (size_t)4 * n * 8, hipMemcpyDeviceToHost));
    return PGP_OK;
}

namespace {
__global__ void laplace_ep_lik_test_kernel(const double* __restrict__ in, double* __restrict__ out, int n) {
    const int i = blockIdx.x * blockDim.x + threadIdx.x;
    if (i >= n) return;
    const double y = in[i], mu = in[n + i], s2 = in[2L * n + i], sn = in[3L * n + i];
    double lZ, dlZ, d2lZ;
    laplace_ep_moments(y, mu, s2, sn, &lZ, &dlZ, &d2lZ);
    out[i] = lZ; out[n + i] = dlZ; out[2L * n + i] = d2lZ; out[3L * n + i] = laplace_ep_dlZhyp(y, mu, s2, sn);
}
}

extern "C" int pgp_test_laplace_ep_lik(pgp_ctx* c, const double* y, const double* mu, const double* s2, const double* sn, int n,
                                       double* out) {
    if (!c || !y || !mu || !s2 || !sn || !out || n <= 0) return -1;
    HIP_TRY(hipSetDevice(c->device));
    DevScratch scr;
    double *id, *od;
    CHK(scr.alloc(&id, (size_t)4 * n * 8)); CHK(scr.alloc(&od, (size_t)4 * n * 8));
    const double* src[4] = {y, mu, s2, sn};
    for (int q = 0; q < 4; ++q) HIP_TRY(hipMemcpy(id + (size_t)q * n, src[q], (size_t)n * 8, hipMemcpyHostToDevice));
    hipLaunchKernelGGL(laplace_ep_lik_test_kernel, dim3((unsigned)((n + 255) / 256)), dim3(256), 0, c->st, id, od, n);
    HIP_TRY(hipGetLastError());
    HIP_TRY(hipStreamSynchronize(c->st));
    HIP_TRY(hipMemcpy(out, od, (size_t)4 * n * 8, hipMemcpyDeviceToHost));
    return PGP_OK;
}

extern "C" int pgp_test_hadamard(pgp_ctx* c, int kind, const double* hyp, int ncov, int para, int flags, const double* Binv,
                                 const double* alpha, const double* wv, double sn2, double* out) {
    if (!c) return -1;
    GateShared device_gate_hold(c);
    if (c->n <= 0) return -1;
    if (!hyp || !Binv || !alpha || !out) return -2;
    HIP_TRY(hipSetDevice(c->device));
    const long n = c->n, d = c->d, np = c->np;
    CovSpec cp;
    CHK(make_spec(c, kind, hyp, ncov, para, flags, -1, d, cp));
    if (cp.ncov != ncov) return -11;
    hipStream_t st = c->st;
    const double nan = std::nan("");
    std::vector<double> hB((size_t)np * np, nan), ha(np, nan), hw(np, nan);
    for (long r = 0; r < n; ++r)
        for (long q = r; q < n; ++q) hB[(size_t)r * np + q] = Binv[(size_t)r * n + q];
    for (long r = 0; r < n; ++r) { ha[r] = alpha[r]; if (wv) hw[r] = wv[r]; }
    PoolScratch tmp(c);
    double *XsT = nullptr, *scd = nullptr, *Bd = nullptr, *ad = nullptr, *wd = nullptr, *partial = nullptr, *prep = nullptr,
           *od = nullptr;
    CHK(tmp.alloc(&XsT, (size_t)c->dpad * np * sizeof(double)));
    CHK(tmp.alloc(&scd, (size_t)c->dpad * sizeof(double)));
    CHK(tmp.alloc(&Bd, (size_t)np * np * sizeof(double)));
    CHK(tmp.alloc(&ad, (size_t)np * sizeof(double)));
    if (wv) CHK(tmp.alloc(&wd, (size_t)np * sizeof(double)));
    CHK(tmp.alloc(&partial, (size_t)hadamard_partial_count(np, ncov) * sizeof(double)));
    CHK(tmp.alloc(&prep, (size_t)hadamard_prep_count(np) * sizeof(double)));
    CHK(tmp.alloc(&od, (size_t)(ncov + 1) * sizeof(double)));
    HIP_TRY(hipMemcpyAsync(Bd, hB.data(), hB.size() * sizeof(double), hipMemcpyHostToDevice, st));
    HIP_TRY(hipMemcpyAsync(ad, ha.data(), np * sizeof(double), hipMemcpyHostToDevice, st));
    if (wv) HIP_TRY(hipMemcpyAsync(wd, hw.data(), np * sizeof(double), hipMemcpyHostToDevice, st));
    CHK(upload_scaled(c, c->x_dev, n, d, cp.scale, XsT, np, c->dpad, scd));
    const bool gram = gram_assembly_applies(c, cp);
    if (gram) CHK(hadamard_prepare_launch(XsT, np, n, np, c->dpad, cp, prep, st, true));
    CHK(hadamard_reduce_launch(XsT, np, n, np, c->dpad, cp, ncov, sn2, Bd, np, ad, partial, od, st, wd, gram ? prep : nullptr));
    HIP_TRY(hipMemcpyAsync(out, od, (size_t)(ncov + 1) * sizeof(double), hipMemcpyDeviceToHost, st));
    HIP_TRY(hipStreamSynchronize(st));
    return PGP_OK;
}

extern "C" int pgp_test_yield_table(pgp_ctx* c, uint32_t* out4096) {
    if (!c || !out4096) return -1;
    if (!c->yield_flags) return -2;
    GateShared device_gate_hold(c);
    HIP_TRY(hipSetDevice(c->device));
    HIP_TRY(hipStreamSynchronize(c->st));
    if (c->st2) HIP_TRY(hipStreamSynchronize(c->st2));
    HIP_TRY(hipMemcpy(out4096, c->yield_flags, 4096 * sizeof(uint32_t), hipMemcpyDeviceToHost));
    return PGP_OK;
}
```

Baseline: 111.4 fits/s.

## Add lean DMA GEMM path with wide C loads/stores and early stage issue

Measured after the change: 111.1 fits/s. About the same (-0.3%).

```diff
diff --git a/pygps_amd/csrc/capi.hip b/pygps_amd/csrc/capi.hip
--- a/pygps_amd/csrc/capi.hip
+++ b/pygps_amd/csrc/capi.hip
@@ -176,6 +176,7 @@
     if (!strcmp(name, "xcd_order")) { c->xcd_order = value; return PGP_OK; }
     if (!strcmp(name, "gemm_dbg")) { if (value & ~(64 | 256 | 512)) return -2; c->gemm_dbg = value; return PGP_OK; }
     if (!strcmp(name, "tile_ring")) { if (value < 0 || value > 1) return -2; c->tile_ring = value; return PGP_OK; }
+    if (!strcmp(name, "tile_lean")) { if (value < 0 || value > 7) return -2; c->tile_lean = value; return PGP_OK; }
     if (!strcmp(name, "lookahead")) { c->lookahead = value; return PGP_OK; }
     if (!strcmp(name, "leaf_first")) { c->leaf_first = value; return PGP_OK; }
     if (!strcmp(name, "leaf_pivot")) { if (value < 0 || value > 2) return -2; c->leaf_pivot = value; return PGP_OK; }
@@ -598,6 +599,7 @@
         if (g.yield_role != 2) g.yield_role = gemm_f64_uses_dma(g) ? 1 : 0;
     } else g.yield_role = 0;
     g.ring = c->tile_ring && gemm_f64_uses_dma(g) ? 1 : 0;
+    g.lean = gemm_f64_uses_dma(g) ? c->tile_lean : 0;
     if (c->gemm_trace && gemm_f64_uses_dma128(g) && g.batch == 1) {
         const long mt = g.M / 128, nt = g.N / 128;
         const long nb = g.order ? g.norder : (g.tri == 2 ? mt * (mt + 1) / 2 : mt * nt);
diff --git a/pygps_amd/csrc/common.h b/pygps_amd/csrc/common.h
--- a/pygps_amd/csrc/common.h
+++ b/pygps_amd/csrc/common.h
@@ -43,6 +43,7 @@
     int order_z;
     int dbg;
     int ring;
+    int lean;
     double flops;
     const double* A2; long lda2; int a_split;
     double* C2; long ldc2; int c_split;
diff --git a/pygps_amd/csrc/ctx.h b/pygps_amd/csrc/ctx.h
--- a/pygps_amd/csrc/ctx.h
+++ b/pygps_amd/csrc/ctx.h
@@ -142,6 +142,7 @@
     std::map<std::vector<int>, std::pair<int*, int>> orders;
     int gemm_dbg = 64 | 256 | 512;
     int tile_ring = 1;
+    int tile_lean = 7;
     int xcd_order = 0;
     int nb_outer = 0;
     int trtri_small_tile_below = 2049;
diff --git a/pygps_amd/csrc/gemm_f64.hip b/pygps_amd/csrc/gemm_f64.hip
--- a/pygps_amd/csrc/gemm_f64.hip
+++ b/pygps_amd/csrc/gemm_f64.hip
@@ -37,7 +37,8 @@
         return ti >= 0;
     }
     if (g.tri == 2) {
-        int r = (int)((sqrt(8.0 * (double)b + 1.0) - 1.0) * 0.5);
+        int r = (g.lean & 4) ? (int)((__builtin_sqrtf(8.0f * (float)b + 1.0f) - 1.0f) * 0.5f) : (int)((sqrt(8.0 * (double)b + 1.0) - 1.0) * 0.5);
+        if (r < 0) r = 0;
         while ((long)(r + 1) * (r + 2) / 2 <= b) ++r;
         while ((long)r * (r + 1) / 2 > b) --r;
         ti = r;
@@ -174,7 +175,7 @@
     auto plain = [](const GemmArgs& g) {
         return g.M > 0 && g.N > 0 && g.tile != 64 && dma_ok(g) && g.batch <= 1 && !g.order_z && !g.wait_flag && g.yield_role != 2;
     };
-    return plain(a) && plain(b) && (a.yield_role == 1 && a.yield_flags) == (b.yield_role == 1 && b.yield_flags) && !a.ring == !b.ring;
+    return plain(a) && plain(b) && (a.yield_role == 1 && a.yield_flags) == (b.yield_role == 1 && b.yield_flags) && !a.ring == !b.ring && a.lean == b.lean;
 }
 int gemm_f64_launch_pair(const GemmArgs& a, const GemmArgs& b, hipStream_t st) {
     if (!gemm_f64_pair_ok(a, b)) return -2;
diff --git a/pygps_amd/csrc/gemm_tile.h b/pygps_amd/csrc/gemm_tile.h
--- a/pygps_amd/csrc/gemm_tile.h
+++ b/pygps_amd/csrc/gemm_tile.h
@@ -15,7 +15,8 @@
 }
 __device__ __forceinline__ const double* uniform_ptr(const double* p) {
     const unsigned long a = (unsigned long)p;
-    const unsigned lo = __builtin_amdgcn_readfirstlane((unsigned)a), hi = __builtin_amdgcn_readfirstlane((unsigned)(a >> 32));
+    unsigned lo = __builtin_amdgcn_readfirstlane((unsigned)a), hi = __builtin_amdgcn_readfirstlane((unsigned)(a >> 32));
+    asm volatile("s_nop 4" : "+s"(lo), "+s"(hi));
     return (const double*)(((unsigned long)hi << 32) | lo);
 }
 template <int V> struct IC { static constexpr int value = V; };
@@ -33,6 +34,15 @@
 }
 __device__ __forceinline__ void ring_landed(double& d) { asm volatile("" : "+v"(d)); }
 __device__ __forceinline__ void ring_landed(unsigned& d) { asm volatile("" : "+v"(d)); }
+template <int OFF>
+__device__ __forceinline__ void ring_load_2f64(double2_t& d, unsigned voff, const double* sbase) {
+    asm volatile("global_load_dwordx4 %0, %1, %2 offset:%3" : "=v"(d) : "v"(voff), "s"(sbase), "n"(OFF) : "memory");
+}
+__device__ __forceinline__ void ring_landed(double2_t& d) { asm volatile("" : "+v"(d)); }
+template <int OFF>
+__device__ __forceinline__ void store_2f64_s(unsigned voff, const double2_t& v, double* sbase) {
+    asm volatile("global_store_dwordx4 %0, %1, %2 offset:%3\n\ts_nop 1" :: "v"(voff), "v"(v), "s"(sbase), "n"(OFF) : "memory");
+}
 
 __device__ __forceinline__ double swap_adjacent(double v) {
     const int lo = __builtin_amdgcn_update_dpp(0, __double2loint(v), 0xB1, 0xF, 0xF, false);
@@ -95,50 +105,7 @@
     const int wm = (wave & 1) * (TM / 2), wn = (wave >> 1) * (TN / 2);
     const int l15 = lane & 15, l4 = lane >> 4;
 
-    double4_t acc[FM][FN];
-    const double ab = g.beta / g.alpha;
-    const bool wantc = g.beta != 0.0 && !(zero_from > 0 && i0 >= zero_from);
-    constexpr int LZ = 16;
-    const bool lazyc = DMA && wantc && (g.dbg & 256) && (k1 - k0) >= (LZ + 2) * BK;
-    const bool preload = wantc && !lazyc;
-#pragma unroll
-    for (int im = 0; im < FM; ++im)
-#pragma unroll
-        for (int in = 0; in < FN; ++in) {
-            if (preload) {
-                const double* cp = Cin + (long)(i0 + wm + im * 16 + l15) + (long)(j0 + wn + in * 16 + l4) * ldcin;
-#pragma unroll
-                for (int r = 0; r < 4; ++r) acc[im][in][r] = ab * cp[(long)(4 * r) * ldcin];
-            } else {
-#pragma unroll
-                for (int r = 0; r < 4; ++r) acc[im][in][r] = 0.0;
-            }
-        }
-
-    double2_t ra[AV], rb[BV];
-    const double* pa[AV];
-    const double* pb[BV];
-    long astep, bstep;
-    if (!AKC) {
-        constexpr int VPR = TM / 2, RPP = 256 / VPR;
-#pragma unroll
-        for (int p = 0; p < AV; ++p) pa[p] = A + (long)(i0 + 2 * (t % VPR)) + (long)(k0 + t / VPR + p * RPP) * lda;
-        astep = (long)BK * lda;
-    } else {
-#pragma unroll
-        for (int p = 0; p < AV; ++p) pa[p] = A + (long)(k0 + 2 * (t & 7)) + (long)(i0 + (t >> 3) + p * 32) * lda;
-        astep = BK;
-    }
-    if (!BKC) {
-        constexpr int VPR = TN / 2, RPP = 256 / VPR;
-#pragma unroll
-        for (int p = 0; p < BV; ++p) pb[p] = B + (long)(j0 + 2 * (t % VPR)) + (long)(k0 + t / VPR + p * RPP) * g.ldb;
-        bstep = (long)BK * g.ldb;
-    } else {
-#pragma unroll
-        for (int p = 0; p < BV; ++p) pb[p] = B + (long)(k0 + 2 * (t & 7)) + (long)(j0 + (t >> 3) + p * 32) * g.ldb;
-        bstep = BK;
-    }
+    const int lean = DMA ? g.lean : 0;
     const double* da[4];
     const double* db[4];
     unsigned lds_w = 0;
@@ -199,6 +166,95 @@
         ring_piece(bufc, halfc, IC<0>{}); ring_piece(bufc, halfc, IC<1>{}); ring_piece(bufc, halfc, IC<2>{});
         if constexpr (P == 4) ring_piece(bufc, halfc, IC<3>{});
     };
+    const bool early = DMA && (lean & 4) != 0;
+    if constexpr (DMA) {
+        if (early && k0 < k1) {
+            if constexpr (RING) { ring_issue(IC<0>{}, IC<0>{}); ring_issue(IC<0>{}, IC<1>{}); }
+            else dma_stage(IC<0>{});
+            __builtin_amdgcn_sched_barrier(0);
+        }
+    }
+
+    double4_t acc[FM][FN];
+    const double ab = g.beta / g.alpha;
+    const bool wantc = g.beta != 0.0 && !(zero_from > 0 && i0 >= zero_from);
+    constexpr int LZ = 16;
+    const bool lazyc = DMA && wantc && (g.dbg & 256) && (k1 - k0) >= (LZ + 2) * BK;
+    const bool preload = wantc && !lazyc;
+    const bool odd = l15 & 1;
+    const bool c16 = DMA && (lean & 1) && wantc && !(ldcin & 1) && !((unsigned long)Cin & 15ul) && ldcin < (1L << 25);
+    const unsigned cvoff = (unsigned)(((long)(l15 & ~1) + (long)(l4 + 4 * (l15 & 1)) * ldcin) * 8L);
+    const double* const cb = uniform_ptr(Cin + (long)(i0 + wm) + (long)(j0 + wn) * ldcin);
+    auto c16_split = [&](const double2_t& v, double& c0, double& c1) __attribute__((always_inline)) {
+        const double t = swap_adjacent(odd ? v.x : v.y);
+        c0 = odd ? t : v.x;
+        c1 = odd ? v.y : t;
+    };
+    typedef const __attribute__((address_space(1))) double2_t* c16_ptr;
+    auto c16_get = [&](int im, int in, int rp) __attribute__((always_inline)) {
+        return *(c16_ptr)((unsigned long)(cb + (long)(im * 16) + (long)(in * 16 + 8 * rp) * ldcin) + cvoff);
+    };
+    if (preload && c16) {
+#pragma unroll
+        for (int im = 0; im < FM; ++im)
+#pragma unroll
+            for (int in = 0; in < FN; ++in) {
+                const double2_t lo = c16_get(im, in, 0), hi = c16_get(im, in, 1);
+                acc[im][in] = double4_t{lo.x, lo.y, hi.x, hi.y};
+            }
+#pragma unroll
+        for (int im = 0; im < FM; ++im)
+#pragma unroll
+            for (int in = 0; in < FN; ++in)
+#pragma unroll
+                for (int rp = 0; rp < 2; ++rp) {
+                    double c0, c1;
+                    c16_split(double2_t{acc[im][in][2 * rp], acc[im][in][2 * rp + 1]}, c0, c1);
+                    acc[im][in][2 * rp] = ab * c0;
+                    acc[im][in][2 * rp + 1] = ab * c1;
+                }
+    } else {
+#pragma unroll
+    for (int im = 0; im < FM; ++im)
+#pragma unroll
+        for (int in = 0; in < FN; ++in) {
+            if (preload) {
+                const double* cp = Cin + (long)(i0 + wm + im * 16 + l15) + (long)(j0 + wn + in * 16 + l4) * ldcin;
+#pragma unroll
+                for (int r = 0; r < 4; ++r) acc[im][in][r] = ab * cp[(long)(4 * r) * ldcin];
+            } else {
+#pragma unroll
+                for (int r = 0; r < 4; ++r) acc[im][in][r] = 0.0;
+            }
+        }
+    }
+
+    double2_t ra[AV], rb[BV];
+    const double* pa[AV] = {};
+    const double* pb[BV] = {};
+    long astep = 0, bstep = 0;
+    if constexpr (!DMA) {
+    if (!AKC) {
+        constexpr int VPR = TM / 2, RPP = 256 / VPR;
+#pragma unroll
+        for (int p = 0; p < AV; ++p) pa[p] = A + (long)(i0 + 2 * (t % VPR)) + (long)(k0 + t / VPR + p * RPP) * lda;
+        astep = (long)BK * lda;
+    } else {
+#pragma unroll
+        for (int p = 0; p < AV; ++p) pa[p] = A + (long)(k0 + 2 * (t & 7)) + (long)(i0 + (t >> 3) + p * 32) * lda;
+        astep = BK;
+    }
+    if (!BKC) {
+        constexpr int VPR = TN / 2, RPP = 256 / VPR;
+#pragma unroll
+        for (int p = 0; p < BV; ++p) pb[p] = B + (long)(j0 + 2 * (t % VPR)) + (long)(k0 + t / VPR + p * RPP) * g.ldb;
+        bstep = (long)BK * g.ldb;
+    } else {
+#pragma unroll
+        for (int p = 0; p < BV; ++p) pb[p] = B + (long)(k0 + 2 * (t & 7)) + (long)(j0 + (t >> 3) + p * 32) * g.ldb;
+        bstep = BK;
+    }
+    }
     auto gload = [&](int) {
 #pragma unroll
         for (int p = 0; p < AV; ++p) { ra[p] = *(const double2_t*)pa[p]; pa[p] += astep; }
@@ -252,18 +308,36 @@
             for (int r = 0; r < 4; ++r) ring_load_f64(cr[4 * q + r], cp + (long)(4 * r) * ldcin);
         }
     };
+    double2_t crv[4];
+    const double* cq[2] = {cb, cb + 8L * ldcin};
+    auto c16_load = [&](auto chunkc, auto jc) __attribute__((always_inline)) {
+        constexpr int hf = decltype(chunkc)::value % (FM / 2), j = decltype(jc)::value, q = j >> 1, rp = j & 1;
+        ring_load_2f64<(2 * hf + q) * 16 * 8>(crv[j], cvoff, cq[rp]);
+    };
+    auto c16_next = [&](auto chunkc) __attribute__((always_inline)) {
+        if constexpr (decltype(chunkc)::value % (FM / 2) == FM / 2 - 1) { cq[0] += 16L * ldcin; cq[1] += 16L * ldcin; }
+    };
+    auto c16_chunk = [&](auto chunkc) __attribute__((always_inline)) {
+        c16_load(chunkc, IC<0>{}); c16_load(chunkc, IC<1>{}); c16_load(chunkc, IC<2>{}); c16_load(chunkc, IC<3>{});
+        c16_next(chunkc);
+    };
+    const int cmode = !c16 ? 0 : (lean & 2) ? 2 : 1;
     if (k0 < k1) {
         if constexpr (RING) {
-            ring_issue(IC<0>{}, IC<0>{});
-            ring_issue(IC<0>{}, IC<1>{});
+            if (!early) {
+                ring_issue(IC<0>{}, IC<0>{});
+                ring_issue(IC<0>{}, IC<1>{});
+            }
             if (k0 + BK < k1) {
                 ring_issue(IC<1>{}, IC<0>{});
-                if (lazyc && ring_cact(1)) { ring_cload(0); ring_wait_barrier<2 * P + 8>(); }
-                else ring_wait_barrier<2 * P>();
+                if (lazyc && ring_cact(1)) {
+                    if (cmode != 0) { c16_chunk(IC<0>{}); ring_wait_barrier<2 * P + 4>(); }
+                    else { ring_cload(0); ring_wait_barrier<2 * P + 8>(); }
+                } else ring_wait_barrier<2 * P>();
             } else ring_wait_barrier<P>();
         } else {
         if constexpr (DMA) {
-            dma_stage(IC<0>{});
+            if (!early) dma_stage(IC<0>{});
             asm volatile("s_waitcnt vmcnt(0)" ::: "memory");
         } else {
             gload(k0);
@@ -324,10 +398,16 @@
             constexpr int i = decltype(ic)::value, in = i / FM, im = i % FM;
             acc[im][in] = __builtin_amdgcn_mfma_f64_16x16x4f64(fb[slot][in], fa[slot][im], acc[im][in], 0, 0, 0);
         };
-        auto mfmas_p = [&](int slot, bool go, auto bufc, auto halfc) __attribute__((always_inline)) {
+        auto mfmas_p = [&](int slot, bool go, auto bufc, auto halfc, bool cgo, auto cchunkc) __attribute__((always_inline)) {
+            constexpr int cch = decltype(cchunkc)::value;
             auto one = [&](auto ic) __attribute__((always_inline)) {
                 constexpr int i = decltype(ic)::value;
                 mfma1(slot, ic);
+                if constexpr (cch >= 0 && i % 2 == 0 && i / 2 < 4) {
+                    __builtin_amdgcn_sched_barrier(0);
+                    if (cgo) c16_load(cchunkc, IC<i / 2>{});
+                    __builtin_amdgcn_sched_barrier(0);
+                }
                 if constexpr (i % 2 == 1 && i / 2 < P) {
                     __builtin_amdgcn_sched_barrier(0);
                     if (go) ring_piece(bufc, halfc, IC<i / 2>{});
@@ -338,30 +418,40 @@
             if constexpr (FM * FN == 16) {
                 one(IC<8>{}); one(IC<9>{}); one(IC<10>{}); one(IC<11>{}); one(IC<12>{}); one(IC<13>{}); one(IC<14>{}); one(IC<15>{});
             }
+            if constexpr (cch >= 0) { if (cgo) c16_next(cchunkc); }
         };
-        auto rstep = [&](int kt, auto bufc, auto pollc, int cp, int cmchunk, bool cmact) __attribute__((always_inline)) {
+        auto rstep = [&](int kt, auto bufc, auto pollc, int cp, auto cmc, bool cmact) __attribute__((always_inline)) {
             constexpr int buf = decltype(bufc)::value;
+            constexpr int cmchunk = decltype(cmc)::value;
             constexpr bool POLL = YIELD && decltype(pollc)::value != 0;
             constexpr int Y = POLL ? 1 : 0;
             const bool more = kt + BK < k1, more2 = kt + 2 * BK < k1;
             unsigned yv = 0u;
             if constexpr (POLL) asm volatile("global_load_dword %0, %1, %2 sc1" : "=v"(yv) : "v"(0u), "s"(yf) : "memory");
             ldfrag(buf, 1, 1);
-            mfmas_p(0, more, IC<(buf ^ 1)>{}, IC<1>{});
+            mfmas_p(0, more, IC<(buf ^ 1)>{}, IC<1>{}, false, IC<-1>{});
             if (more) {
-                if (cp != 0) ring_wait_barrier<2 * P + Y + 8>();
+                if (cp == 8) ring_wait_barrier<2 * P + Y + 8>();
+                else if (cp == 4) ring_wait_barrier<2 * P + Y + 4>();
                 else ring_wait_barrier<2 * P + Y>();
             } else ring_wait_barrier<0>();
             const bool cm = cmchunk >= 0 && cmact;
-            if (cm) ring_cload(cmchunk);
+            if constexpr (cmchunk >= 0) {
+                if (cm) {
+                    if (cmode == 0) ring_cload(cmchunk);
+                    else if (cmode == 1) c16_chunk(cmc);
+                }
+            }
             ldfrag(buf, 2, 0);
             __builtin_amdgcn_sched_barrier(0);
-            mfmas_p(1, more2, IC<buf>{}, IC<0>{});
+            if constexpr (cmchunk >= 0) mfmas_p(1, more2, IC<buf>{}, IC<0>{}, cm && cmode == 2, cmc);
+            else mfmas_p(1, more2, IC<buf>{}, IC<0>{}, false, IC<-1>{});
             ldfrag(buf, 3, 1);
             mfmas(0);
             if (more2) {
-                if (cm) ring_wait_barrier<2 * P + 8>();
-                else ring_wait_barrier<2 * P>();
+                if (!cm) ring_wait_barrier<2 * P>();
+                else if (cmode != 0) ring_wait_barrier<2 * P + 4>();
+                else ring_wait_barrier<2 * P + 8>();
             } else if (more) ring_wait_barrier<P>();
             else ring_wait_barrier<0>();
             if constexpr (POLL) { ring_landed(yv); if (__builtin_amdgcn_readfirstlane(yv) != 0u) gemm_yield_wait(yf); }
@@ -378,18 +468,33 @@
                     constexpr int chunk = (BH ? (st & 7) : st) >> 1, in = chunk / (FM / 2), hf = chunk % (FM / 2);
                     if constexpr ((st & 1) != 0) {
                         if (ring_cact(st)) {
-#pragma unroll
-                            for (int i = 0; i < 8; ++i) ring_landed(cr[i]);
-#pragma unroll
-                            for (int q = 0; q < 2; ++q)
-#pragma unroll
-                                for (int r = 0; r < 4; ++r) acc[2 * hf + q][in][r] = fma(ab, cr[4 * q + r], acc[2 * hf + q][in][r]);
+                            if (cmode == 0) {
+#pragma unroll
+                                for (int i = 0; i < 8; ++i) ring_landed(cr[i]);
+#pragma unroll
+                                for (int q = 0; q < 2; ++q)
+#pragma unroll
+                                    for (int r = 0; r < 4; ++r) acc[2 * hf + q][in][r] = fma(ab, cr[4 * q + r], acc[2 * hf + q][in][r]);
+                            } else {
+#pragma unroll
+                                for (int i = 0; i < 4; ++i) ring_landed(crv[i]);
+#pragma unroll
+                                for (int q = 0; q < 2; ++q)
+#pragma unroll
+                                    for (int rp = 0; rp < 2; ++rp) {
+                                        double c0, c1;
+                                        c16_split(crv[2 * q + rp], c0, c1);
+                                        acc[2 * hf + q][in][2 * rp] = fma(ab, c0, acc[2 * hf + q][in][2 * rp]);
+                                        acc[2 * hf + q][in][2 * rp + 1] = fma(ab, c1, acc[2 * hf + q][in][2 * rp + 1]);
+                                    }
+                            }
                         }
-                        rstep(kt, IC<1>{}, IC<0>{}, 0, st + 2 < LZ ? (BH ? ((st + 2) & 7) : (st + 2)) >> 1 : -1, ring_cact(st + 2));
+                        constexpr int nxt = st + 2 < LZ ? (BH ? ((st + 2) & 7) : (st + 2)) >> 1 : -1;
+                        rstep(kt, IC<1>{}, IC<0>{}, 0, IC<nxt>{}, ring_cact(st + 2));
                     } else {
-                        const int cp = ring_cact(st + 1) ? 8 : 0;
-                        if constexpr ((st & 3) == 0) rstep(kt, IC<0>{}, IC<1>{}, cp, -1, false);
-                        else rstep(kt, IC<0>{}, IC<0>{}, cp, -1, false);
+                        const int cp = ring_cact(st + 1) ? (cmode != 0 ? 4 : 8) : 0;
+                        if constexpr ((st & 3) == 0) rstep(kt, IC<0>{}, IC<1>{}, cp, IC<-1>{}, false);
+                        else rstep(kt, IC<0>{}, IC<0>{}, cp, IC<-1>{}, false);
                     }
                     kt += BK;
                 };
@@ -399,17 +504,17 @@
                 if (g.trace) smem[2 * STAGE] = __longlong_as_double((long long)wall_clock64());
             }
             while (kt < k1) {
-                rstep(kt, IC<0>{}, IC<1>{}, 0, -1, false);
+                rstep(kt, IC<0>{}, IC<1>{}, 0, IC<-1>{}, false);
                 kt += BK;
                 if (kt >= k1) break;
-                rstep(kt, IC<1>{}, IC<0>{}, 0, -1, false);
+                rstep(kt, IC<1>{}, IC<0>{}, 0, IC<-1>{}, false);
                 kt += BK;
                 if constexpr (YIELD) {
                     if (kt >= k1) break;
-                    rstep(kt, IC<0>{}, IC<0>{}, 0, -1, false);
+                    rstep(kt, IC<0>{}, IC<0>{}, 0, IC<-1>{}, false);
                     kt += BK;
                     if (kt >= k1) break;
-                    rstep(kt, IC<1>{}, IC<0>{}, 0, -1, false);
+                    rstep(kt, IC<1>{}, IC<0>{}, 0, IC<-1>{}, false);
                     kt += BK;
                 }
             }
@@ -469,7 +574,30 @@
         trc[2] = (long long)wall_clock64();
         if constexpr (DMA) trc[1] = lazyc ? __double_as_longlong(smem[2 * STAGE]) : 0ll;
     }
-    if (!diag && (g.dbg & 512) && !(ldc & 1) && !((unsigned long)C & 15ul)) {
+    if (DMA && (lean & 1) && !diag && (g.dbg & 512) && !(ldc & 1) && !((unsigned long)C & 15ul) && ldc < (1L << 25)) {
+        if constexpr (DMA) {
+        const bool oddl = l15 & 1;
+        const unsigned evoff = (unsigned)(((long)(l15 & ~1) + (long)(l4 + 4 * (l15 & 1)) * ldc) * 8L);
+        double* const eb = (double*)uniform_ptr(C + (long)(i0 + wm) + (long)(j0 + wn) * ldc);
+        double* ecol = eb;
+        const long ecstep = 8L * ldc;
+        static_assert(FM == 4, "four 16-row fragments per wave");
+#pragma unroll
+        for (int in = 0; in < FN; ++in)
+#pragma unroll
+            for (int r = 0; r < 4; r += 2) {
+                auto put = [&](auto imc) __attribute__((always_inline)) {
+                    constexpr int im = decltype(imc)::value;
+                    const double x = g.alpha * acc[im][in][r], yv = g.alpha * acc[im][in][r + 1];
+                    const double nx = swap_adjacent(x), ny = swap_adjacent(yv);
+                    const double2_t val = oddl ? double2_t{ny, yv} : double2_t{x, nx};
+                    store_2f64_s<im * 16 * 8>(evoff, val, ecol);
+                };
+                put(IC<0>{}); put(IC<1>{}); put(IC<2>{}); put(IC<3>{});
+                ecol += ecstep;
+            }
+        }
+    } else if (!diag && (g.dbg & 512) && !(ldc & 1) && !((unsigned long)C & 15ul)) {
         const bool odd = l15 & 1;
 #pragma unroll
         for (int im = 0; im < FM; ++im)
diff --git a/pygps_amd/csrc/testhooks.hip b/pygps_amd/csrc/testhooks.hip
--- a/pygps_amd/csrc/testhooks.hip
+++ b/pygps_amd/csrc/testhooks.hip
@@ -382,15 +382,17 @@
     if (poll && !c->yield_flags) return -2;
     HIP_TRY(hipSetDevice(c->device));
     const size_t an = (size_t)lda * (a_kc ? M : K), bn = (size_t)ldb * (b_kc ? N : K), cn = (size_t)ldc * N;
-    double *Ad, *Bd, *Cd;
-    HIP_TRY(hipMalloc((void**)&Ad, an * 8)); HIP_TRY(hipMalloc((void**)&Bd, bn * 8)); HIP_TRY(hipMalloc((void**)&Cd, cn * 8));
+    double *Ad, *Bd, *Cd0;
+    const size_t coff = getenv("PGP_TEST_GEMM_COFF") ? 1 : 0;
+    HIP_TRY(hipMalloc((void**)&Ad, an * 8)); HIP_TRY(hipMalloc((void**)&Bd, bn * 8)); HIP_TRY(hipMalloc((void**)&Cd0, (cn + coff) * 8));
+    double* const Cd = Cd0 + coff;
     HIP_TRY(hipMemcpy(Ad, A, an * 8, hipMemcpyHostToDevice));
     HIP_TRY(hipMemcpy(Bd, B, bn * 8, hipMemcpyHostToDevice));
     HIP_TRY(hipMemcpy(Cd, C, cn * 8, hipMemcpyHostToDevice));
     GemmArgs g{};
     g.A = Ad; g.lda = lda; g.a_kc = a_kc; g.B = Bd; g.ldb = ldb; g.b_kc = b_kc; g.C = Cd; g.ldc = ldc;
     g.M = M; g.N = N; g.K = K; g.alpha = alpha; g.beta = beta; g.tri = tri; g.tri_off = 0; g.mask_diag = mask_diag;
-    g.kmode = kmode; g.koff = koff; g.batch = 1; g.tile = tile; g.dbg = c->gemm_dbg; g.ring = c->tile_ring != 0;
+    g.kmode = kmode; g.koff = koff; g.batch = 1; g.tile = tile; g.dbg = c->gemm_dbg; g.ring = c->tile_ring != 0; g.lean = c->tile_lean;
     if (getenv("PGP_TEST_GEMM_FOLD")) g.fold_rows = 1;
     if (poll && gemm_f64_uses_dma(g)) { g.yield_flags = c->yield_flags; g.yield_role = 1; }
     hipStream_t ts = c->st;
@@ -419,7 +421,7 @@
         *ms_out = ms / iters;
         (void)hipEventDestroy(e0); (void)hipEventDestroy(e1);
     }
-    (void)hipFree(Ad); (void)hipFree(Bd); (void)hipFree(Cd);
+    (void)hipFree(Ad); (void)hipFree(Bd); (void)hipFree(Cd0);
     return rc;
 }
 
@@ -440,7 +442,7 @@
     HIP_TRY(hipMemset(Cd, 0, (size_t)M * M * 8)); HIP_TRY(hipMemset(C2, 0, (size_t)M * M * 8));
     GemmArgs g{};
     g.A = A; g.lda = M; g.B = A; g.ldb = M; g.C = Cd; g.ldc = M; g.M = M; g.N = M; g.K = K; g.alpha = -1.0; g.beta = 1.0;
-    g.tri = tri ? 2 : 0; g.mask_diag = tri ? 1 : 0; g.batch = 1; g.tile = 128; g.dbg = c->gemm_dbg; g.ring = c->tile_ring != 0;
+    g.tri = tri ? 2 : 0; g.mask_diag = tri ? 1 : 0; g.batch = 1; g.tile = 128; g.dbg = c->gemm_dbg; g.ring = c->tile_ring != 0; g.lean = c->tile_lean;
     int rc = PGP_OK;
     for (int i = 0; i < warm && rc == PGP_OK; ++i) rc = gemm_f64_launch(g, c->st);
     HIP_TRY(hipStreamSynchronize(c->st));
@@ -484,7 +486,7 @@
     HIP_TRY(hipMemset(fl, 0, 16));
     GemmArgs g{};
     g.A = Ad; g.lda = n; g.B = Bd; g.ldb = n; g.C = Cd; g.ldc = n; g.M = n; g.N = n; g.K = K; g.alpha = -1.0; g.beta = 1.0;
-    g.tri = 2; g.mask_diag = 1; g.batch = 1; g.tile = tile; g.dbg = c->gemm_dbg; g.ring = c->tile_ring != 0; g.skip_lo = skip_lo; g.skip_hi = skip_hi;
+    g.tri = 2; g.mask_diag = 1; g.batch = 1; g.tile = tile; g.dbg = c->gemm_dbg; g.ring = c->tile_ring != 0; g.lean = c->tile_lean; g.skip_lo = skip_lo; g.skip_hi = skip_hi;
     if (wait_ms > 0) { g.wait_flag = fl; g.wait_target = 7u; g.wait_err = fl + 1; }
     int rc = gemm_f64_launch(g, c->st);
     if (rc == PGP_OK && wait_ms > 0) {
@@ -542,7 +544,7 @@
     GemmArgs g{};
     g.A = Ad; g.lda = lda; g.B = Bd; g.ldb = ldb; g.C = Cd; g.ldc = ldc; g.M = M; g.N = N; g.K = K; g.alpha = alpha; g.beta = beta;
     if (Ci) { g.Cin = Ci; g.ldcin = ldc; }
-    g.tri = tri; g.mask_diag = mask_diag; g.kmode = KM_FULL; g.batch = 1; g.tile = tile; g.dbg = c->gemm_dbg; g.ring = c->tile_ring != 0;
+    g.tri = tri; g.mask_diag = mask_diag; g.kmode = KM_FULL; g.batch = 1; g.tile = tile; g.dbg = c->gemm_dbg; g.ring = c->tile_ring != 0; g.lean = c->tile_lean;
     g.zero_from = zero_from; g.zf_upper = zf_upper;
     const int rc = gemm_f64_launch(g, c->st);
     HIP_TRY(hipStreamSynchronize(c->st));
@@ -567,7 +569,7 @@
     HIP_TRY(hipMemcpy(Cbd, Cb, cn, hipMemcpyHostToDevice));
     GemmArgs g{};
     g.A = Ad; g.lda = lda; g.B = Bd; g.ldb = ldb; g.C = Cad; g.ldc = ldc; g.M = M; g.N = N; g.K = Ka; g.alpha = alpha; g.beta = beta;
-    g.kmode = KM_FULL; g.batch = 1; g.tile = 128; g.dbg = c->gemm_dbg; g.ring = c->tile_ring != 0;
+    g.kmode = KM_FULL; g.batch = 1; g.tile = 128; g.dbg = c->gemm_dbg; g.ring = c->tile_ring != 0; g.lean = c->tile_lean;
     GemmArgs h = g;
     h.C = Cbd; h.K = Kb;
     const int rc = gemm_f64_launch_pair(g, h, c->st);
@@ -668,7 +670,7 @@
     HIP_TRY(hipMemset(A, 0, (size_t)M * K * 8)); HIP_TRY(hipMemset(Cm, 0, (size_t)M * M * 8));
     GemmArgs g{};
     g.A = A; g.lda = M; g.B = A; g.ldb = M; g.C = Cm; g.ldc = M; g.M = M; g.N = M; g.K = K;
-    g.alpha = -1.0; g.beta = 1.0; g.tile = 128; g.batch = 1; g.dbg = c->gemm_dbg; g.ring = c->tile_ring != 0;
+    g.alpha = -1.0; g.beta = 1.0; g.tile = 128; g.batch = 1; g.dbg = c->gemm_dbg; g.ring = c->tile_ring != 0; g.lean = c->tile_lean;
     hipEvent_t e0, e1;
     HIP_TRY(hipEventCreate(&e0)); HIP_TRY(hipEventCreate(&e1));
     hipStream_t sts[2] = {ms, c->st};
```
